# Gardlin/PCR-CG

Measured on AMD Instinct MI355X. Metric: fragment-pairs/s KPFCNN+GCN fwd, 30k-pt pairs, higher is better.
Workload: dtype f32

## Files before the change

include/pcrcg.h:

```cpp
#ifndef PCRCG_H
#define PCRCG_H

#include <stddef.h>
#include <stdint.h>

#ifdef __cplusplus
extern "C" {
#endif

#define PCRCG_OK 0
#define PCRCG_EBADARG (-1)
#define PCRCG_EWORKSPACE (-2)
#define PCRCG_ELAUNCH (-3)
#define PCRCG_ECAPACITY (-4)

#define PCRCG_KPOINTS 15

const char* pcrcg_last_error(void);
#define PCRCG_ABI_VERSION 4
int pcrcg_abi_version(void);

int pcrcg_debug_set(const char* spec);
int pcrcg_debug_release(void);

// ... 111 lines not shown
                             float* const* out, int count, int c, int ld_x, int ld_out, void* stream);
size_t pcrcg_instnorm_ws_bytes(int c);
int pcrcg_instnorm_stats_from_partials(const void* partials, int chunks, int c, double count, float eps,
                                       float* stats, void* stream);
int pcrcg_instnorm_stats(const float* x, int n, int c, int ldx, float eps, float* stats, void* ws,
                         size_t ws_bytes, void* stream);
int pcrcg_instnorm_apply(const float* x, int n, int c, int ldx, const float* stats, const float* res,
                         int ldr, const float* res_stats, float slope, float* y, int ldy, void* stream);
int pcrcg_instnorm_colsums(const float* x, int n, int c, int ldx, void* sums, void* stream);
int pcrcg_instnorm_apply_sums(const float* x, int n, int c, int ldx, const void* sums, double count, float eps,
                              const float* res, int ldr, const void* res_sums, float slope, float* y, int ldy,
                              void* stream);

int pcrcg_fill2d(float* dst, int ld, int rows, int cols, float value, void* stream);
int pcrcg_inject_image_features(const float* fmap, int c, int h, int w, const float* valid, const int64_t* inds2d,
                                const int64_t* inds3d, int n, long row_offset, long n_rows, float* x, int ldx,
                                void* stream);

typedef struct pcrcg_image_frame {
    const float* fmap;
    const float* depth;
    const float* valid;
    float world2camera[16];
    float intrinsics[16];
    float thresh;
    int h, w;
    int depth_h, depth_w;
    int target;
} pcrcg_image_frame;

size_t pcrcg_project_depth_ws_bytes(int n);
int pcrcg_project_depth(const float* points, int n, const float* depth, int h, int w, const float* h_world2camera,
                        const float* h_intrinsics, float thresh, int64_t* inds2d, int64_t* inds3d, int* k, void* ws,
                        size_t ws_bytes, void* stream);
int pcrcg_inject_frames(const float* points, long n_points, long len_src, const pcrcg_image_frame* h_frames, int n_frames,
                        int c, float* x, int ldx, void* stream);
int pcrcg_superglue_valid_maps(const float* keypoints0, int n0, const float* keypoints1, int n1, const int64_t* matches,
                               const float* confidence, int window, int map_w, int map_h, float* src_valid, float* tgt_valid,
                               void* stream);

int pcrcg_knn(const float* coords, int n, int k, int* idx, void* stream);
size_t pcrcg_edgeconv_ws_bytes(int c);
int pcrcg_edgeconv_reduce(const float* ctr, int ld_ctr, const float* nbr, int ld_nbr, const int* idx,
                          int n, int k, int c, float eps, float* emax, int ld_emax, float* stats,
                          void* ws, size_t ws_bytes, void* stream);
int pcrcg_edgeconv_reduce_sums(const float* ctr, int ld_ctr, const float* nbr, int ld_nbr, const int* idx, int n, int k,
                               int c, float* emax, int ld_emax, void* sums, void* stream);
int pcrcg_softmax_rows(float* x, int rows, int cols, int ld, float scale, void* stream);
int pcrcg_attention_supported(int d);
int pcrcg_attention(const float* q, int ldq, const float* k, int ldk, const float* v, int ldv, float* out, int ldo, int n,
                    int ms, int heads, int d, float scale, void* stream);
int pcrcg_softmax_matvec(const float* x, int rows, int cols, int ld, float scale, const float* vec, int ldv, float* y,
                         int ldy, void* stream);

int pcrcg_check_status(const int* status, void* stream);

int pcrcg_copy2d(const float* src, int ld_src, float* dst, int ld_dst, int rows, int cols, void* stream);
int pcrcg_add(const float* a, const float* b, float* dst, long n, void* stream);
int pcrcg_l2norm_rows(const float* src, int ld_src, float* dst, int ld_dst, int rows, int cols, void* stream);
int pcrcg_sigmoid_scores(const float* src, int ld_src, float* dst, int rows, void* stream);

#define PCRCG_MAX_LEVELS 8
#define PCRCG_MAX_BLOCKS 32
#define PCRCG_MAX_GNN 8

enum { PCRCG_BLK_SIMPLE = 0, PCRCG_BLK_RESNETB = 1, PCRCG_BLK_UNARY = 2, PCRCG_BLK_LAST_UNARY = 3,
       PCRCG_BLK_UPSAMPLE = 4 };

typedef struct pcrcg_block {
    int type;
    int layer;
    int strided;
    int in_dim, out_dim;
    int mid_dim;
    float extent;
    const float* kp;
    const float* kp_w;
    const float* kp_wt;
    const float* kp_w_pad;
    int cin_pad;
    const float* unary1;
    const float* unary2;
    const float* shortcut;
    const float* mlp;
    int mlp_ld;
    const float* mlp_skip;
    int mlp_skip_ld, skip_dim;
} pcrcg_block;

typedef struct pcrcg_gnn_layer {
    int cross;
    const float* edge1;
    const float* edge2;
    const float* conv3;
    const float *wq, *bq, *wk, *bk, *wv, *bv;
    const float *wm, *bm;
    const float *w0, *b0;
    const float *w3, *b3;
} pcrcg_gnn_layer;

typedef struct pcrcg_model {
    int n_enc, n_dec, n_gnn;
    pcrcg_block enc[PCRCG_MAX_BLOCKS];
    pcrcg_block dec[PCRCG_MAX_BLOCKS];
    pcrcg_gnn_layer gnn[PCRCG_MAX_GNN];
    int enc_skip[PCRCG_MAX_BLOCKS];
    int dec_concat[PCRCG_MAX_BLOCKS];
    int enc_out_dim, gnn_dim, heads, knn_k, final_dim;
    const float *bottle_w, *bottle_b;
    const float *proj_gnn_w, *proj_gnn_b;
    const float *proj_score_w, *proj_score_b;
    float temperature;
    int feature_bf16;
// ... 143 lines not shown
```

pcrcg_amd/_lib.py:

```python
import ctypes
import os

_HERE = os.path.dirname(os.path.abspath(__file__))
LIB_PATH = os.path.join(_HERE, "libpcrcg_hip.so")


def lib_identity():
    import hashlib
    with open(LIB_PATH, "rb") as f:
        return LIB_PATH, hashlib.sha256(f.read()).hexdigest()[:16]

ABI_VERSION = 4

c_int, c_float, c_void_p, c_size_t = ctypes.c_int, ctypes.c_float, ctypes.c_void_p, ctypes.c_size_t

SIGNATURES = {
    "pcrcg_last_error": (ctypes.c_char_p, []),
    "pcrcg_abi_version": (c_int, []),
    "pcrcg_debug_set": (c_int, [ctypes.c_char_p]),
    "pcrcg_check_status": (c_int, [c_void_p, c_void_p]),
    "pcrcg_grid_subsample_ws_bytes": (c_size_t, [c_int, c_int]),
    "pcrcg_grid_subsample_batch": (c_int, [c_void_p, c_int, c_void_p, c_int, c_float, c_int, c_void_p, c_void_p,
                                           c_void_p, c_void_p, c_size_t, c_void_p]),
    "pcrcg_grid_subsample_ex_ws_bytes": (c_size_t, [c_int, c_int, c_int, c_int]),
# ... 36 lines not shown
    "pcrcg_kpconv_aggregate_walk": (c_int, [c_void_p, c_int, c_void_p, c_int, c_void_p, c_int, c_int, c_void_p, c_int,
                                            c_void_p, c_float, c_void_p, c_void_p, c_void_p, c_size_t, c_void_p, c_void_p]),
    "pcrcg_kpconv_aggregate_bf16_walk": (c_int, [c_void_p, c_int, c_void_p, c_int, c_void_p, c_int, c_int, c_void_p, c_int,
                                                 c_void_p, c_float, c_void_p, c_void_p, c_void_p, c_void_p, c_size_t,
                                                 c_void_p, c_void_p]),
    "pcrcg_gather_max_walk": (c_int, [c_void_p, c_int, c_int, c_void_p, c_int, c_int, c_int, c_void_p, c_void_p, c_void_p]),
    "pcrcg_profile_kpconv": (None, [c_int]),
    "pcrcg_profile_kpconv_read": (c_int, [c_void_p, c_void_p, c_void_p, c_void_p, c_void_p, c_void_p, c_int]),
    "pcrcg_gemm_f32": (c_int, [c_void_p, c_int, c_void_p, c_int, c_int, c_void_p, c_int, c_int, c_int, c_int,
                               c_void_p, c_void_p, c_void_p]),
    "pcrcg_gemm_colstats_bytes": (c_size_t, [c_int, c_int]),
    "pcrcg_gemm_f32_colstats": (c_int, [c_void_p, c_int, c_void_p, c_int, c_int, c_void_p, c_int, c_int, c_int, c_int,
                                        c_void_p, c_void_p, c_void_p, c_size_t, c_void_p, c_void_p]),
    "pcrcg_gemm_bf16a_f32_colstats": (c_int, [c_void_p, c_int, c_void_p, c_int, c_void_p, c_int, c_int, c_int, c_int,
                                              c_void_p, c_void_p, c_void_p, c_size_t, c_void_p, c_void_p]),
    "pcrcg_gemm_f32_fused": (c_int, [c_void_p, c_int, c_void_p, c_int, c_int, c_void_p, c_void_p, ctypes.c_double, c_float,
                                     c_float, c_void_p, c_int, c_void_p, c_void_p, c_int, c_int, c_int, c_int, c_int, c_void_p]),
    "pcrcg_gemm_set_mode": (None, [c_int]),
    "pcrcg_gemm_get_mode": (c_int, []),
    "pcrcg_gemm_redo_counts": (c_int, [c_void_p, c_int]),
    "pcrcg_instnorm_stats_from_partials": (c_int, [c_void_p, c_int, c_int, ctypes.c_double, c_float, c_void_p,
                                                   c_void_p]),
    "pcrcg_gather_max": (c_int, [c_void_p, c_int, c_int, c_void_p, c_int, c_int, c_int, c_void_p, c_void_p]),
    "pcrcg_gather_first": (c_int, [c_void_p, c_int, c_int, c_void_p, c_int, c_int, c_void_p, c_int, c_void_p]),
    "pcrcg_gather_first_multi": (c_int, [c_void_p, c_void_p, c_void_p, c_void_p, c_void_p, c_void_p, c_int, c_int, c_int, c_int,
                                         c_void_p]),
    "pcrcg_instnorm_ws_bytes": (c_size_t, [c_int]),
    "pcrcg_instnorm_stats": (c_int, [c_void_p, c_int, c_int, c_int, c_float, c_void_p, c_void_p, c_size_t, c_void_p]),
    "pcrcg_instnorm_apply": (c_int, [c_void_p, c_int, c_int, c_int, c_void_p, c_void_p, c_int, c_void_p, c_float,
                                     c_void_p, c_int, c_void_p]),
    "pcrcg_instnorm_colsums": (c_int, [c_void_p, c_int, c_int, c_int, c_void_p, c_void_p]),
    "pcrcg_instnorm_apply_sums": (c_int, [c_void_p, c_int, c_int, c_int, c_void_p, ctypes.c_double, c_float, c_void_p, c_int,
                                          c_void_p, c_float, c_void_p, c_int, c_void_p]),
    "pcrcg_fill2d": (c_int, [c_void_p, c_int, c_int, c_int, c_float, c_void_p]),
    "pcrcg_inject_image_features": (c_int, [c_void_p, c_int, c_int, c_int, c_void_p, c_void_p, c_void_p, c_int, ctypes.c_long,
                                            ctypes.c_long, c_void_p, c_int, c_void_p]),
    "pcrcg_project_depth_ws_bytes": (c_size_t, [c_int]),
    "pcrcg_project_depth": (c_int, [c_void_p, c_int, c_void_p, c_int, c_int, c_void_p, c_void_p, c_float, c_void_p, c_void_p,
                                    c_void_p, c_void_p, c_size_t, c_void_p]),
    "pcrcg_inject_frames": (c_int, [c_void_p, ctypes.c_long, ctypes.c_long, c_void_p, c_int, c_int, c_void_p, c_int, c_void_p]),
    "pcrcg_superglue_valid_maps": (c_int, [c_void_p, c_int, c_void_p, c_int, c_void_p, c_void_p, c_int, c_int, c_int, c_void_p,
                                           c_void_p, c_void_p]),
    "pcrcg_knn": (c_int, [c_void_p, c_int, c_int, c_void_p, c_void_p]),
    "pcrcg_edgeconv_ws_bytes": (c_size_t, [c_int]),
    "pcrcg_edgeconv_reduce": (c_int, [c_void_p, c_int, c_void_p, c_int, c_void_p, c_int, c_int, c_int, c_float,
                                      c_void_p, c_int, c_void_p, c_void_p, c_size_t, c_void_p]),
    "pcrcg_edgeconv_reduce_sums": (c_int, [c_void_p, c_int, c_void_p, c_int, c_void_p, c_int, c_int, c_int, c_void_p, c_int,
                                           c_void_p, c_void_p]),
    "pcrcg_softmax_rows": (c_int, [c_void_p, c_int, c_int, c_int, c_float, c_void_p]),
    "pcrcg_attention_supported": (c_int, [c_int]),
    "pcrcg_attention": (c_int, [c_void_p, c_int, c_void_p, c_int, c_void_p, c_int, c_void_p, c_int, c_int, c_int, c_int,
                                c_int, c_float, c_void_p]),
    "pcrcg_softmax_matvec": (c_int, [c_void_p, c_int, c_int, c_int, c_float, c_void_p, c_int, c_void_p, c_int, c_void_p]),
    "pcrcg_copy2d": (c_int, [c_void_p, c_int, c_void_p, c_int, c_int, c_int, c_void_p]),
    "pcrcg_add": (c_int, [c_void_p, c_void_p, c_void_p, ctypes.c_long, c_void_p]),
    "pcrcg_l2norm_rows": (c_int, [c_void_p, c_int, c_void_p, c_int, c_int, c_int, c_void_p]),
    "pcrcg_sigmoid_scores": (c_int, [c_void_p, c_int, c_void_p, c_int, c_void_p]),
    "pcrcg_kpfcnn_ws_bytes": (c_size_t, [c_void_p, c_void_p]),
    "pcrcg_kpfcnn_group_ws_bytes": (c_size_t, [c_void_p, c_void_p, c_int]),
    "pcrcg_kpfcnn_forward_group": (c_int, [c_void_p, c_void_p, c_void_p, c_int, c_void_p, c_size_t, c_void_p]),
    "pcrcg_kpfcnn_forward": (c_int, [c_void_p, c_void_p, c_void_p, c_void_p, c_size_t, c_void_p]),
    "pcrcg_pyramid_ws_bytes": (c_size_t, [c_int, c_int, c_void_p]),
    "pcrcg_pyramid_build": (c_int, [c_void_p, c_int, c_void_p, c_int, c_void_p, c_void_p, c_size_t, c_void_p, c_void_p,
                                    c_void_p, c_void_p, c_void_p, c_void_p]),
    "pcrcg_pyramid_build_parts": (c_int, [c_void_p, c_void_p, c_void_p, c_void_p, c_int, c_void_p, c_void_p, c_size_t, c_void_p,
                                          c_void_p, c_void_p, c_void_p, c_void_p, c_void_p]),
    "pcrcg_pyramid_restore_run": (c_int, [c_void_p, c_void_p, c_void_p]),
    "pcrcg_debug_release": (c_int, []),
    "pcrcg_stream_pipe_classes": (c_int, [c_void_p, c_int, c_void_p, c_void_p]),
    "pcrcg_thread_shares_gpu": (None, [c_int]),
    "pcrcg_stream_create": (c_int, [c_void_p, c_int]),
    "pcrcg_stream_destroy": (c_int, [c_void_p]),
    "pcrcg_ransac_ws_bytes": (c_size_t, [c_int, c_int, c_int, c_int]),
    "pcrcg_feature_match": (c_int, [c_void_p, c_int, c_int, c_void_p, c_int, c_int, c_int, c_int, c_void_p, c_void_p,
                                    c_void_p, c_size_t, c_void_p]),
    "pcrcg_ransac": (c_int, [c_void_p, c_int, c_void_p, c_int, c_void_p, c_void_p, c_int, c_void_p, c_int, ctypes.c_double,
                             ctypes.c_double, c_int, c_int, c_int, ctypes.c_uint64, c_void_p, c_void_p, c_void_p, c_void_p,
                             c_size_t, c_void_p]),
    "pcrcg_ransac_batch_ws_bytes": (c_size_t, [c_int, c_int, c_int, c_int, c_int]),
    "pcrcg_feature_match_batch": (c_int, [c_void_p, c_int, c_void_p, c_int, c_int, c_void_p, c_int, c_void_p, c_int, c_int,
                                          c_int, c_int, c_void_p, c_void_p, c_void_p, c_size_t, c_void_p]),
    "pcrcg_ransac_batch": (c_int, [c_void_p, c_void_p, c_void_p, c_void_p, c_int, c_void_p, c_void_p, c_void_p, c_int, c_int,
                                   ctypes.c_double, ctypes.c_double, c_int, c_int, c_int, c_void_p, c_void_p, c_void_p,
                                   c_void_p, c_size_t, c_void_p]),
    "pcrcg_inlier_stats_batch_ws_bytes": (c_size_t, [c_int, c_int, c_int]),
    "pcrcg_inlier_stats_batch": (c_int, [c_void_p, c_void_p, c_int, c_void_p, c_int, c_int, c_void_p, c_void_p, c_int, c_void_p,
                                         c_int, c_int, c_int, c_int, c_void_p, c_void_p, c_int, c_void_p, c_void_p, c_void_p,
                                         c_void_p, c_void_p, c_void_p, c_void_p, c_size_t, c_void_p]),
    "pcrcg_icp_batch_ws_bytes": (c_size_t, [c_int, c_int, c_int, c_int]),
    "pcrcg_icp_batch": (c_int, [c_void_p, c_void_p, c_int, c_int, c_void_p, c_int, c_void_p, c_void_p, c_int, ctypes.c_double,
                                c_int, ctypes.c_double, ctypes.c_double, c_void_p, c_void_p, c_void_p, c_void_p, c_size_t,
                                c_void_p]),
    "pcrcg_voxel_down_sample_ws_bytes": (c_size_t, [c_int, c_int]),
    "pcrcg_voxel_down_sample_batch": (c_int, [c_void_p, c_void_p, c_int, c_int, ctypes.c_double, c_void_p, c_void_p, c_void_p,
                                              c_void_p, c_void_p, c_size_t, c_void_p]),
    "pcrcg_weighted_sample_ws_bytes": (c_size_t, [c_int, c_int]),
    "pcrcg_weighted_sample_batch": (c_int, [c_void_p, c_void_p, c_int, c_int, c_void_p, c_void_p, c_void_p, c_void_p, c_size_t,
                                            c_void_p]),
    "pcrcg_chamfer_batch_ws_bytes": (c_size_t, [c_int, c_int, c_int, c_int]),
    "pcrcg_chamfer_batch": (c_int, [c_void_p, c_void_p, c_int, c_void_p, c_void_p, c_int, c_void_p, c_void_p, c_int, c_int,
                                    c_void_p, c_void_p, c_void_p, c_void_p, c_void_p, c_void_p, c_void_p, c_void_p, c_void_p,
                                    c_void_p, c_size_t, c_void_p]),
    "pcrcg_res50unet_arena_bytes": (c_size_t, [c_int]),
    "pcrcg_res50unet_pack": (c_int, [c_void_p, c_int, c_int, c_void_p, c_void_p]),
    "pcrcg_res50unet_ws_bytes": (c_size_t, [c_int, c_int, c_int]),
    "pcrcg_res50unet_forward": (c_int, [c_void_p, c_void_p, c_int, c_int, c_void_p, c_int, c_int, c_int, c_int, c_int,
# ... 112 lines not shown
```

pcrcg_amd/csrc/common.h:

```cpp
#pragma once
#include <hip/hip_runtime.h>

#include <cstdarg>
#include <cstdint>
#include <cstdio>
#include <map>
#include <mutex>

#include "pcrcg.h"

namespace pcrcg {

void set_error(const char* fmt, ...);

inline hipStream_t as_stream(void* s) { return reinterpret_cast<hipStream_t>(s); }

struct Carver {
    char* base;
    size_t cap;
    size_t off = 0;
    Carver(void* ws, size_t bytes) : base(static_cast<char*>(ws)), cap(bytes) {}
    template <typename T>
    T* take(size_t count) {
        size_t bytes = (count * sizeof(T) + 255) & ~size_t(255);
        T* p = reinterpret_cast<T*>(base + off);
        off += bytes;
        return p;
    }
    bool ok() const { return off <= cap; }
};
inline size_t carve_bytes(size_t count, size_t elem) { return (count * elem + 255) & ~size_t(255); }

size_t scan_ws_bytes(int n);
int exclusive_scan_i32(const int* in, int* out, int n, int* total, void* ws, hipStream_t stream);

constexpr int kWave = 64;

bool instnorm_pack_ok(int c, int ldx, int ldy);
int instnorm_apply_pack(const float* x, int n, int c, int ldx, const float* stats, const double* sums, double count, float eps,
                        float slope, float* y, int ldy, const float* s_pts, float4* pk, hipStream_t st);
size_t colstats_ws_bytes(int c);
int colstats_finalize(const double* partial, int nchunks, int c, double count, float eps, float* stats,
                      hipStream_t st);
int colstats_chunks();

class StreamScratch {
public:
    explicit StreamScratch(bool cleared = false);
    void* get(hipStream_t st, size_t bytes, size_t slack = 0);
    void release();
private:
    struct Buf { void* p = nullptr; size_t bytes = 0; };
    const bool cleared_;
    std::mutex mu_;
    std::map<hipStream_t, Buf> bufs_;
};

int query_walk_multi(const float* const* pts, const int* n, int* const* walk, int* const* key, int count, hipStream_t st);

struct NormJob {
    const float* x; const double* sums; const float* res; const double* res_sums; float* y;
    const float* s_pts; float4* pk;
    int n; double count;
    float* stats_out = nullptr;
};
int instnorm_apply_sums_multi(const NormJob* jobs, int count, int c, int ldx, float eps, int ldr, float slope, int ldy, bool pack,
                              hipStream_t st);
bool instnorm_sums_ok(int c, int ldx, int ldy, int ldr = 0);

struct GatherJob { const float* x; const int64_t* idx; float* out; int ns, nq, h, ld_idx; const int* walk = nullptr; };
int gather_max_multi(const GatherJob* jobs, int count, int c, hipStream_t st);
struct FirstJob { const float* x; const int64_t* idx; float* out; int ns, nq, ld_idx; };
int gather_first_multi(const FirstJob* jobs, int count, int c, int ld_x, int ld_out, hipStream_t st);
int heads_multi(const float* const* x, const int* rows, int count, int ld, int fd, float* const* feats, float* const* s_ov,
                float* const* s_sal, hipStream_t st);
int copy2d_multi(const float* const* src, float* const* dst, const int* rows, int count, int ld_src, int ld_dst, int cols,
                 hipStream_t st);
int instnorm_colsums_multi(const float* const* x, double* const* sums, const int* n, int count, int c, int ldx, hipStream_t st);

struct EdgeCloud {
    const float* ctr; const float* nbr; const int* idx; float* emax; double* sums; int n, k;
};
bool edgeconv_rows_ok(const EdgeCloud* cl, int count, int ld_ctr, int ld_nbr, int ld_emax, int c);
int edgeconv_rows_multi(const EdgeCloud* cl, int count, int ld_ctr, int ld_nbr, int ld_emax, int c, bool atomic, int* nchunks_out,
                        hipStream_t st);

struct AttnCloud { const float* q; const float* k; const float* v; float* out; int n, ms; };
bool attention_mfma_ok(const AttnCloud* cl, int count, int ldq, int ldk, int ldv, int d);
int attention_mfma_multi(const AttnCloud* cl, int count, int ldq, int ldk, int ldv, int ldo, int heads, int d, float scale,
                         hipStream_t st);
bool attention_bwd_mfma_ok(int n, int ms, int d, int ldq, int ldk, int ldv, int ld_do);
int attention_bwd_mfma(const float* q, int ldq, const float* k, int ldk, const float* v, int ldv, const float* o, int ldo,
                       const float* d_o, int ld_do, float* dq, int ld_dq, float* dk, int ld_dk, float* dv, int ld_dv, int n, int ms,
                       int heads, int d, float scale, hipStream_t st);

struct DebugOpts {
    int stat_sums = 1;
    int stat_sums_rows = 1 << 30;
    int att_mfma = 1;
    int radius_blocks = 0;
    int kd_blocks = 0;
    int att_tq = 16;
    int kd_spin_limit = 0;
    int gemm_log = 0;
    int x6_tile = -1, x6_splitk = 0, x6_t1 = 1, x6_t2 = 1, x6_order = -1, x6_big = 0, x6_h2 = 1;
    int train_side_stream = 1;
    int gemm_tile = -1, gemm_splitk = 0, gemm_split_target = 768;
    int deterministic = 0;
    int bwd_mfma = 1;
    int walk = 1;
};
const DebugOpts& debug_opts();

struct KpProfScope {
    hipStream_t st;
    hipEvent_t a, b;
    int nq, h, cin, cout, kind;
    bool on;
    KpProfScope(hipStream_t s, int nq, int h, int cin, int cout, int kind);
    ~KpProfScope();
};

}

#define PCRCG_CHECK_ARG(cond)                                                        \
    do {                                                                             \
        if (!(cond)) {                                                               \
            pcrcg::set_error("%s: bad argument: %s", __func__, #cond);               \
            return PCRCG_EBADARG;                                                    \
        }                                                                            \
    } while (0)
// ... 44 lines not shown
```

pcrcg_amd/csrc/elementwise.hip:

```cpp
#include "common.h"
#include "pcrcg_train.h"

namespace pcrcg {
namespace {

struct CopyMulti { const float* src[4]; float* dst[4]; int rows[4]; };
__global__ void __launch_bounds__(256) k_copy2d(CopyMulti mm, int ld_src, int ld_dst, int cols) {
    const float* __restrict__ src = mm.src[blockIdx.y];
    float* __restrict__ dst = mm.dst[blockIdx.y];
    const int rows = mm.rows[blockIdx.y];
    const long e = (long)blockIdx.x * blockDim.x + threadIdx.x;
    if (e >= (long)rows * cols) return;
    const long r = e / cols;
    const int c = (int)(e - r * cols);
    dst[r * ld_dst + c] = src[r * ld_src + c];
}

__global__ void __launch_bounds__(256) k_add(const float* __restrict__ a, const float* __restrict__ b,
                                              float* __restrict__ dst, long n) {
    const long e = (long)blockIdx.x * blockDim.x + threadIdx.x;
    if (e < n) dst[e] = a[e] + b[e];
}

__global__ void __launch_bounds__(256) k_l2norm_rows(const float* __restrict__ src, int ld_src, float* __restrict__ dst,
                                                      int ld_dst, int rows, int cols) {
    const int lane = threadIdx.x & 63;
    const int r = blockIdx.x * 4 + (threadIdx.x >> 6);
    if (r >= rows) return;
    float s = 0.f;
    for (int c = lane; c < cols; c += 64) {
        const float v = src[(long)r * ld_src + c];
        s += v * v;
    }
#pragma unroll
    for (int d = 32; d >= 1; d >>= 1) s += __shfl_xor(s, d, 64);
    const float inv = 1.0f / fmaxf(sqrtf(s), 1e-12f);
    for (int c = lane; c < cols; c += 64) dst[(long)r * ld_dst + c] = src[(long)r * ld_src + c] * inv;
}

__global__ void __launch_bounds__(256) k_sigmoid_scores(const float* __restrict__ src, int ld_src,
                                                         float* __restrict__ dst, int rows) {
    const int r = blockIdx.x * blockDim.x + threadIdx.x;
    if (r >= rows) return;
    float v = 1.0f / (1.0f + expf(-src[(long)r * ld_src]));
    v = fminf(fmaxf(v, 0.0f), 1.0f);
    if (isnan(v) || isinf(v)) v = 0.0f;
    dst[r] = v;
}

struct HeadsMulti { const float* x[4]; float* feats[4]; float* s_ov[4]; float* s_sal[4]; int rows[4]; };
__global__ void __launch_bounds__(256) k_heads(HeadsMulti mm, int ld, int fd) {
    const int g = blockIdx.y, lane = threadIdx.x & 63;
    const int r = blockIdx.x * 4 + (threadIdx.x >> 6);
    if (r >= mm.rows[g]) return;
    const float* src = mm.x[g] + (long)r * ld;
    float s = 0.f;
    for (int c = lane; c < fd; c += 64) {
        const float v = src[c];
        s += v * v;
    }
#pragma unroll
    for (int d = 32; d >= 1; d >>= 1) s += __shfl_xor(s, d, 64);
    const float inv = 1.0f / fmaxf(sqrtf(s), 1e-12f);
    float* dst = mm.feats[g] + (long)r * fd;
    for (int c = lane; c < fd; c += 64) dst[c] = src[c] * inv;
    if (lane < 2) {
        float v = 1.0f / (1.0f + expf(-src[fd + lane]));
        v = fminf(fmaxf(v, 0.0f), 1.0f);
        if (isnan(v) || isinf(v)) v = 0.0f;
        (lane == 0 ? mm.s_ov[g] : mm.s_sal[g])[r] = v;
    }
}

__global__ void __launch_bounds__(256) k_fill2d(float* __restrict__ dst, int ld, int rows, int cols, float v) {
    const long e = (long)blockIdx.x * blockDim.x + threadIdx.x;
    if (e >= (long)rows * cols) return;
    const long r = e / cols;
    dst[r * ld + (int)(e - r * cols)] = v;
}

__global__ void __launch_bounds__(256) k_inject_image(const float* __restrict__ fmap, int c, int h, int w,
                                                       const float* __restrict__ valid, const long long* __restrict__ inds2d,
                                                       const long long* __restrict__ inds3d, int n, long row_offset,
                                                       long n_rows, float* __restrict__ x, int ldx) {
    const int lane = threadIdx.x & 63;
    const int j = blockIdx.x * 4 + (threadIdx.x >> 6);
    if (j >= n) return;
    const long px = inds2d[2 * (long)j], py = inds2d[2 * (long)j + 1], row = inds3d[j] + row_offset;
    if (px < 0 || px >= w || py < 0 || py >= h || row < 0 || row >= n_rows) return;
    const float m = valid ? valid[px * h + py] : 1.0f;
    float* dst = x + row * ldx;
    for (int ch = lane; ch < c; ch += 64) dst[ch] = fmap[((long)ch * h + py) * w + px] * m;
    if (lane == 0) dst[c] = 1.0f;
}

}

int heads_multi(const float* const* x, const int* rows, int count, int ld, int fd, float* const* feats, float* const* s_ov,
                float* const* s_sal, hipStream_t st) {
    PCRCG_CHECK_ARG(count >= 1 && count <= 4 && fd >= 1 && ld >= fd + 2);
    HeadsMulti mm;
    int rmax = 0;
    for (int g = 0; g < 4; ++g) {
        const int k = g < count ? g : 0;
        PCRCG_CHECK_ARG(x[k] && feats[k] && s_ov[k] && s_sal[k] && rows[k] >= 0);
        mm.x[g] = x[k]; mm.feats[g] = feats[k]; mm.s_ov[g] = s_ov[k]; mm.s_sal[g] = s_sal[k]; mm.rows[g] = g < count ? rows[k] : 0;
        if (g < count) rmax = rows[k] > rmax ? rows[k] : rmax;
    }
    if (rmax == 0) return PCRCG_OK;
    hipLaunchKernelGGL(k_heads, dim3((rmax + 3) / 4, count), dim3(256), 0, st, mm, ld, fd);
    PCRCG_CHECK_LAUNCH();
    return PCRCG_OK;
}

int copy2d_multi(const float* const* src, float* const* dst, const int* rows, int count, int ld_src, int ld_dst, int cols,
                 hipStream_t st) {
    PCRCG_CHECK_ARG(count >= 1 && count <= 4 && cols >= 0 && ld_src >= cols && ld_dst >= cols);
    CopyMulti mm;
    int rmax = 0;
    for (int g = 0; g < 4; ++g) {
        const int k = g < count ? g : 0;
        mm.src[g] = src[k]; mm.dst[g] = dst[k]; mm.rows[g] = g < count ? rows[k] : 0;
        if (g < count) {
            PCRCG_CHECK_ARG(rows[k] >= 0 && (rows[k] == 0 || (src[k] && dst[k])));
            rmax = rows[k] > rmax ? rows[k] : rmax;
        }
    }
    if (rmax == 0 || cols == 0) return PCRCG_OK;
    const long total = (long)rmax * cols;
    hipLaunchKernelGGL(k_copy2d, dim3((unsigned)((total + 255) / 256), count), dim3(256), 0, st, mm, ld_src, ld_dst, cols);
    PCRCG_CHECK_LAUNCH();
    return PCRCG_OK;
}
struct GatherJobs { const float* src; float* dst; const int* m1; const int* m2; int n; float s2; int accumulate; int cols; };
__global__ void __launch_bounds__(256) k_gather_jobs(const GatherJobs* __restrict__ jobs) {
    const GatherJobs jb = jobs[blockIdx.y];
    if (!jb.m1) {
        __shared__ float tile[32][33];
        const int cols = jb.cols, rows = jb.n / cols;
        const int tx = (cols + 31) / 32, ty = (rows + 31) / 32;
        const int lx = threadIdx.x & 31, ly = threadIdx.x >> 5;
        for (int t = blockIdx.x; t < tx * ty; t += gridDim.x) {
            const int r0 = (t / tx) * 32, c0 = (t % tx) * 32;
            __syncthreads();
#pragma unroll
            for (int u = 0; u < 4; ++u) {
                const int r = r0 + ly + 8 * u, c = c0 + lx;
                tile[ly + 8 * u][lx] = (r < rows && c < cols) ? jb.src[(long)r * cols + c] : 0.f;
            }
            __syncthreads();
#pragma unroll
            for (int u = 0; u < 4; ++u) {
                const int c = c0 + ly + 8 * u, r = r0 + lx;
                if (c < cols && r < rows) {
                    float* d = jb.dst + (long)c * rows + r;
                    *d = jb.accumulate ? *d + tile[lx][ly + 8 * u] : tile[lx][ly + 8 * u];
                }
            }
        }
        return;
    }
    auto one = [&](long i) {
        const int a = jb.m1[i];
        float v = a >= 0 ? jb.src[a] : 0.f;
        if (jb.m2) {
            const int b = jb.m2[i];
            if (b >= 0) v += jb.s2 * jb.src[b];
        }
        jb.dst[i] = jb.accumulate ? jb.dst[i] + v : v;
    };
    const bool vec = ((reinterpret_cast<uintptr_t>(jb.dst) | reinterpret_cast<uintptr_t>(jb.m1) | reinterpret_cast<uintptr_t>(jb.m2)) & 15) == 0;
    if (!vec) {
        for (long i = (long)blockIdx.x * 256 + threadIdx.x; i < jb.n; i += (long)gridDim.x * 256) one(i);
        return;
    }
    const long n4 = jb.n & ~3;
    for (long i = ((long)blockIdx.x * 256 + threadIdx.x) * 4; i < n4; i += (long)gridDim.x * 1024) {
        const int4 a = *reinterpret_cast<const int4*>(jb.m1 + i);
        int4 b = make_int4(-1, -1, -1, -1);
        if (jb.m2) b = *reinterpret_cast<const int4*>(jb.m2 + i);
        float4 v = make_float4(a.x >= 0 ? jb.src[a.x] : 0.f, a.y >= 0 ? jb.src[a.y] : 0.f, a.z >= 0 ? jb.src[a.z] : 0.f,
                               a.w >= 0 ? jb.src[a.w] : 0.f);
        if (b.x >= 0) v.x += jb.s2 * jb.src[b.x];
// ... 8 lines not shown
}
}

using namespace pcrcg;

extern "C" {

int pcrcg_fill2d(float* dst, int ld, int rows, int cols, float value, void* stream) {
    PCRCG_CHECK_ARG(rows >= 0 && cols >= 0 && ld >= cols);
    if (rows == 0 || cols == 0) return PCRCG_OK;
    PCRCG_CHECK_ARG(dst != nullptr);
    const long total = (long)rows * cols;
    hipLaunchKernelGGL(k_fill2d, dim3((unsigned)((total + 255) / 256)), dim3(256), 0, as_stream(stream), dst, ld, rows,
                       cols, value);
    PCRCG_CHECK_LAUNCH();
    return PCRCG_OK;
}

int pcrcg_inject_image_features(const float* fmap, int c, int h, int w, const float* valid, const int64_t* inds2d,
                                const int64_t* inds3d, int n, long row_offset, long n_rows, float* x, int ldx,
                                void* stream) {
    PCRCG_CHECK_ARG(c >= 1 && h >= 1 && w >= 1 && n >= 0 && n_rows >= 0 && ldx >= c + 1);
    if (n == 0) return PCRCG_OK;
    PCRCG_CHECK_ARG(fmap && inds2d && inds3d && x);
    hipLaunchKernelGGL(k_inject_image, dim3((n + 3) / 4), dim3(256), 0, as_stream(stream), fmap, c, h, w, valid,
                       reinterpret_cast<const long long*>(inds2d), reinterpret_cast<const long long*>(inds3d), n, row_offset,
                       n_rows, x, ldx);
    PCRCG_CHECK_LAUNCH();
    return PCRCG_OK;
}

int pcrcg_copy2d(const float* src, int ld_src, float* dst, int ld_dst, int rows, int cols, void* stream) {
    PCRCG_CHECK_ARG(rows >= 0 && cols >= 0 && ld_src >= cols && ld_dst >= cols);
    if (rows == 0 || cols == 0) return PCRCG_OK;
    PCRCG_CHECK_ARG(src && dst);
    return pcrcg::copy2d_multi(&src, &dst, &rows, 1, ld_src, ld_dst, cols, as_stream(stream));
}

int pcrcg_gather_jobs(const void* jobs, int n_jobs, int max_n, void* stream) {
    static_assert(sizeof(GatherJobs) == sizeof(pcrcg_gather_job), "pcrcg_gather_job layout");
    PCRCG_CHECK_ARG(n_jobs >= 0 && max_n >= 0);
    if (n_jobs == 0 || max_n == 0) return PCRCG_OK;
    PCRCG_CHECK_ARG(jobs != nullptr);
    const int gx = (max_n + 1023) / 1024 < 1024 ? (max_n + 1023) / 1024 : 1024;
    hipLaunchKernelGGL(k_gather_jobs, dim3(gx, n_jobs), dim3(256), 0, as_stream(stream), static_cast<const GatherJobs*>(jobs));
    PCRCG_CHECK_LAUNCH();
    return PCRCG_OK;
}

int pcrcg_add(const float* a, const float* b, float* dst, long n, void* stream) {
    PCRCG_CHECK_ARG(n >= 0);
    if (n == 0) return PCRCG_OK;
    PCRCG_CHECK_ARG(a && b && dst);
    hipLaunchKernelGGL(k_add, dim3((unsigned)((n + 255) / 256)), dim3(256), 0, as_stream(stream), a, b, dst, n);
    PCRCG_CHECK_LAUNCH();
    return PCRCG_OK;
}

int pcrcg_l2norm_rows(const float* src, int ld_src, float* dst, int ld_dst, int rows, int cols, void* stream) {
    PCRCG_CHECK_ARG(rows >= 0 && cols >= 1 && ld_src >= cols && ld_dst >= cols);
    if (rows == 0) return PCRCG_OK;
    PCRCG_CHECK_ARG(src && dst);
    hipLaunchKernelGGL(k_l2norm_rows, dim3((rows + 3) / 4), dim3(256), 0, as_stream(stream), src, ld_src, dst, ld_dst,
                       rows, cols);
    PCRCG_CHECK_LAUNCH();
    return PCRCG_OK;
}

int pcrcg_sigmoid_scores(const float* src, int ld_src, float* dst, int rows, void* stream) {
    PCRCG_CHECK_ARG(rows >= 0 && ld_src >= 1);
    if (rows == 0) return PCRCG_OK;
    PCRCG_CHECK_ARG(src && dst);
    hipLaunchKernelGGL(k_sigmoid_scores, dim3((rows + 255) / 256), dim3(256), 0, as_stream(stream), src, ld_src, dst,
                       rows);
    PCRCG_CHECK_LAUNCH();
    return PCRCG_OK;
}
}
```

pcrcg_amd/csrc/gnn.hip:

```cpp
#include "common.h"
#include "pcrcg_train.h"

namespace pcrcg {
namespace {

typedef unsigned long long u64;

__device__ __forceinline__ float knn_sq(float x, float y, float z) {
#pragma clang fp contract(off)
    return (x * x + y * y) + z * z;
}
__device__ __forceinline__ float knn_dist(float ax, float ay, float az, float sa, float bx, float by, float bz) {
#pragma clang fp contract(off)
    const float dot = __builtin_fmaf(az, bz, __builtin_fmaf(ay, by, ax * bx));
    const float sb = (bx * bx + by * by) + bz * bz;
    const float d = (-2.0f * dot + sa) + sb;
    return fmaxf(d, 1e-12f);
}

#define KNN_RB_MAX 704
#define KNN_K_MAX 10
__device__ __forceinline__ bool kless(u64 x, u64 y) { return (x >> 32) < (y >> 32); }

__device__ void rp_adjust_heap(u64* a, int hole, int len, u64 value) {
// ... 79 lines not shown
    auto key_of = [&](int j) -> u64 {
        const float d = knn_dist(ax, ay, az, sa, coords[3 * (long)j], coords[3 * (long)j + 1], coords[3 * (long)j + 2]);
        return ((u64)__float_as_uint(d) << 32) | (unsigned)j;
    };
    if (K * 64 <= n) {
        if (lane < K) a[lane] = key_of(lane);
        rp_make_heap(a, K);
        for (int base = K; base < n; base += 64) {
            const int j = base + lane;
            const u64 kj = j < n ? key_of(j) : ~0ull;
            u64 m = __ballot(kless(kj, a[0]));
            while (m) {
                const int l = __ffsll((long long)m) - 1;
                const u64 value = __shfl(kj, l, 64);
                rp_adjust_heap(a, 0, K, value);
                m = __ballot(kless(kj, a[0])) & ~((2ull << l) - 1ull);
            }
        }
        rp_sort_heap(a, K);
    } else {
        for (int j = lane; j < n; j += 64) a[j] = key_of(j);
        int first = 0, last = n;
        const int nth = K - 1;
        int depth = 2 * (31 - __clz(n));
        bool done = false;
        while (last - first > 3) {
            if (depth == 0) {
                u64* h = a + first;
                const int hl = nth + 1 - first;
                rp_make_heap(h, hl);
                for (int j = nth + 1; j < last; ++j)
                    if (kless(a[j], h[0])) {
                        const u64 value = a[j];
                        a[j] = h[0];
                        rp_adjust_heap(h, 0, hl, value);
                    }
                const u64 t = a[first];
                a[first] = a[nth];
                a[nth] = t;
                done = true;
                break;
            }
            --depth;
            const int cut = rp_partition_pivot(a, first, last);
            if (cut <= nth) first = cut;
            else last = cut;
        }
        if (!done) rp_insertion_sort(a, first, last);
        rp_insertion_sort(a, 0, K - 1);
    }
    if (lane >= 1 && lane < K) out[lane - 1] = (int)(a[lane] & 0xFFFFFFFFull);
}

__global__ void __launch_bounds__(256) k_knn(const float* __restrict__ coords, int n, int k, int* __restrict__ idx) {
    const int lane = threadIdx.x & 63;
    const int i = blockIdx.x * 4 + (threadIdx.x >> 6);
    if (i >= n) return;
    const float ax = coords[3 * (long)i], ay = coords[3 * (long)i + 1], az = coords[3 * (long)i + 2];
    const float sa = knn_sq(ax, ay, az);
    __shared__ u64 s_q[4][KNN_RB_MAX];
    u64 last = 0;
    bool have_last = false;
    bool tie = false;
    for (int round = 0; round <= k + 1; ++round) {
        u64 best = ~0ull;
        for (int j = lane; j < n; j += 64) {
            const float bx = coords[3 * (long)j], by = coords[3 * (long)j + 1], bz = coords[3 * (long)j + 2];
            float d = knn_dist(ax, ay, az, sa, bx, by, bz);
            const u64 key = ((u64)__float_as_uint(d) << 32) | (unsigned)j;
            if ((!have_last || key > last) && key < best) best = key;
        }
#pragma unroll
        for (int s = 32; s >= 1; s >>= 1) {
            const u64 o = __shfl_xor(best, s, 64);
            best = o < best ? o : best;
        }
        tie |= have_last && best != ~0ull && (best >> 32) == (last >> 32);
        last = best;
        have_last = true;
        if (round >= 1 && round <= k && lane == 0)
            idx[(long)i * k + (round - 1)] = best == ~0ull ? i : (int)(best & 0xFFFFFFFFull);
    }
    if (tie && n > k && k <= KNN_K_MAX) knn_replay_row(coords, n, i, k, s_q[threadIdx.x >> 6], idx + (long)i * k);
}

template <int PER>
__global__ void __launch_bounds__(256) k_knn_reg(const float* __restrict__ coords, int n, int k, int* __restrict__ idx) {
    const int lane = threadIdx.x & 63;
    const int i = blockIdx.x * 4 + (threadIdx.x >> 6);
    if (i >= n) return;
    const float ax = coords[3 * (long)i], ay = coords[3 * (long)i + 1], az = coords[3 * (long)i + 2];
    const float sa = knn_sq(ax, ay, az);
    u64 key[PER];
#pragma unroll
    for (int t = 0; t < PER; ++t) {
        const int j = lane + 64 * t;
        const int jc = j < n ? j : n - 1;
        const float bx = coords[3 * (long)jc], by = coords[3 * (long)jc + 1], bz = coords[3 * (long)jc + 2];
        float d = knn_dist(ax, ay, az, sa, bx, by, bz);
        key[t] = j < n ? (((u64)__float_as_uint(d) << 32) | (unsigned)j) : ~0ull;
    }
    __shared__ u64 s_q[4][KNN_RB_MAX];
    u64 last = 0;
    bool tie = false;
    for (int round = 0; round <= k + 1; ++round) {
        u64 best = ~0ull;
#pragma unroll
        for (int t = 0; t < PER; ++t)
            if ((round == 0 || key[t] > last) && key[t] < best) best = key[t];
#pragma unroll
        for (int s = 32; s >= 1; s >>= 1) {
            const u64 o = __shfl_xor(best, s, 64);
            best = o < best ? o : best;
        }
        tie |= round > 0 && best != ~0ull && (best >> 32) == (last >> 32);
        last = best;
        if (round >= 1 && round <= k && lane == 0)
            idx[(long)i * k + (round - 1)] = best == ~0ull ? i : (int)(best & 0xFFFFFFFFull);
    }
    if (tie && n > k && k <= KNN_K_MAX) knn_replay_row(coords, n, i, k, s_q[threadIdx.x >> 6], idx + (long)i * k);
}

struct AttCloud { const float* q; const float* k; const float* v; float* out; int n, ms; };
struct AttMulti { AttCloud cl[4]; int ldq, ldk, ldv, ldo; float scale; int chunk_blocks; };

typedef float attf16 __attribute__((ext_vector_type(16)));

template <int D>
__global__ void __launch_bounds__(256) k_attention_mfma(AttMulti a) {
    constexpr int DH = D / 2, NT = D / 32;
    extern __shared__ __attribute__((aligned(16))) float att2_lds[];
    const AttCloud cl = a.cl[blockIdx.z];
    const int n = cl.n, ms = cl.ms;
    const int q0 = blockIdx.x * 32;
    if (q0 >= n) return;
    const int head = blockIdx.y;
    const int lane = threadIdx.x & 63, wave = __builtin_amdgcn_readfirstlane((int)(threadIdx.x >> 6));
    const int l31 = lane & 31, half = lane >> 5;
    const int sld = a.chunk_blocks * 32 + 1;
    float* const S = att2_lds;
    float* const m_run = S + 32 * sld;
    float* const l_run = m_run + 32;
    float* const alpha = l_run + 32;
    float* const red = alpha + 32;
    const int nkb = (ms + 31) / 32;
    if (threadIdx.x < 32) { m_run[threadIdx.x] = -INFINITY; l_run[threadIdx.x] = 0.f; }
    float qr[DH];
    {
        const float* qrow = cl.q + (long)min(q0 + l31, n - 1) * a.ldq + head * D + half * DH;
#pragma unroll
        for (int c = 0; c < DH / 4; ++c) {
            const float4 t = *reinterpret_cast<const float4*>(qrow + 4 * c);
            qr[4 * c] = t.x; qr[4 * c + 1] = t.y; qr[4 * c + 2] = t.z; qr[4 * c + 3] = t.w;
        }
    }
    attf16 o[NT];
#pragma unroll
    for (int t = 0; t < NT; ++t)
#pragma unroll
        for (int r = 0; r < 16; ++r) o[t][r] = 0.f;
    for (int kb_lo = 0; kb_lo < nkb; kb_lo += a.chunk_blocks) {
        const int kb_hi = min(nkb, kb_lo + a.chunk_blocks), cb = kb_hi - kb_lo;
        __syncthreads();
        for (int kb = kb_lo + wave; kb < kb_hi; kb += 4) {
            const int key = kb * 32 + l31;
            const float* krow = cl.k + (long)min(key, ms - 1) * a.ldk + head * D + half * DH;
            float kr[DH];
#pragma unroll
            for (int c = 0; c < DH / 4; ++c) {
                const float4 t = *reinterpret_cast<const float4*>(krow + 4 * c);
                kr[4 * c] = t.x; kr[4 * c + 1] = t.y; kr[4 * c + 2] = t.z; kr[4 * c + 3] = t.w;
            }
            attf16 acc;
#pragma unroll
            for (int r = 0; r < 16; ++r) acc[r] = 0.f;
#pragma unroll
            for (int kk = 0; kk < DH; ++kk) acc = __builtin_amdgcn_mfma_f32_32x32x2f32(qr[kk], kr[kk], acc, 0, 0, 0);
// ... 217 lines not shown
            attf16 acc;
#pragma unroll
            for (int r = 0; r < 16; ++r) acc[r] = 0.f;
#pragma unroll
            for (int s = 0; s < 16; ++s) {
                const int qi = 2 * s + half;
                const long ro = (long)min(q0 + qi, n - 1);
                const float av = dS[qi * sld + key_lo + l31];
                const float bv = a.q[ro * a.ldq + head * D + 32 * t + l31];
                acc = __builtin_amdgcn_mfma_f32_32x32x2f32(av, bv, acc, 0, 0, 0);
            }
#pragma unroll
            for (int r = 0; r < 16; ++r) {
                const int key = key_lo + (r & 3) + 8 * (r >> 2) + 4 * half;
                if (key < ms) atomicAdd(a.dk + (long)key * a.ld_dk + head * D + 32 * t + l31, acc[r]);
            }
        }
    }
    {
        attf16 o[NT];
#pragma unroll
        for (int t = 0; t < NT; ++t)
#pragma unroll
            for (int r = 0; r < 16; ++r) o[t][r] = 0.f;
        const int per = (nkb + NW - 1) / NW;
        const int b0 = min(wave * per, nkb), b1 = min(b0 + per, nkb);
        for (int bi = b0; bi < b1; ++bi) {
            float pv[16], kv[NT][16];
#pragma unroll
            for (int j = 0; j < 16; ++j) {
                const int key = bi * 32 + 16 * half + j;
                pv[j] = dS[l31 * sld + key];
                const float* krow = a.k + (long)min(key, ms - 1) * a.ldk + head * D;
#pragma unroll
                for (int t = 0; t < NT; ++t) kv[t][j] = key < ms ? krow[t * 32 + l31] : 0.f;
            }
#pragma unroll
            for (int j = 0; j < 16; ++j)
#pragma unroll
                for (int t = 0; t < NT; ++t) o[t] = __builtin_amdgcn_mfma_f32_32x32x2f32(pv[j], kv[t][j], o[t], 0, 0, 0);
        }
        if (b1 > b0) {
#pragma unroll
            for (int t = 0; t < NT; ++t)
#pragma unroll
                for (int r = 0; r < 16; ++r) {
                    const int row = (r & 3) + 8 * (r >> 2) + 4 * half;
                    if (q0 + row < n) atomicAdd(a.dq + (long)(q0 + row) * a.ld_dq + head * D + t * 32 + l31, o[t][r]);
                }
        }
    }
}

struct EdgeMulti { EdgeCloud cl[4]; int ld_ctr, ld_nbr, ld_emax, c, rows_per_block, nchunks; };

template <bool ATOMIC>
__global__ void __launch_bounds__(256) k_edgeconv_rows(EdgeMulti a) {
    __shared__ double s_sum[4][256], s_sq[4][256];
    const EdgeCloud cl = a.cl[blockIdx.z];
    const int lane = threadIdx.x & 63, wave = __builtin_amdgcn_readfirstlane((int)(threadIdx.x >> 6));
    const int c0 = blockIdx.y * 256 + lane * 4;
    const bool cok = c0 < a.c;
    const int r0 = blockIdx.x * a.rows_per_block, r1 = min(cl.n, r0 + a.rows_per_block);
    double s[4] = {0.0, 0.0, 0.0, 0.0}, sq[4] = {0.0, 0.0, 0.0, 0.0};
    for (int r = r0 + wave; r < r1; r += 4) {
        const int mine = lane < cl.k ? cl.idx[(long)r * cl.k + lane] : 0;
        float4 q = make_float4(0.f, 0.f, 0.f, 0.f), m = q;
        if (cok) q = *reinterpret_cast<const float4*>(cl.ctr + (long)r * a.ld_ctr + c0);
        for (int j0 = 0; j0 < cl.k; j0 += 8) {
            float4 v[8];
#pragma unroll
            for (int u = 0; u < 8; ++u) {
                const int nb = __builtin_amdgcn_readlane(mine, min(j0 + u, cl.k - 1));
                v[u] = cok ? *reinterpret_cast<const float4*>(cl.nbr + (long)nb * a.ld_nbr + c0) : make_float4(0.f, 0.f, 0.f, 0.f);
            }
#pragma unroll
            for (int u = 0; u < 8; ++u) {
                if (j0 + u >= cl.k) continue;
                const float e[4] = {q.x + v[u].x, q.y + v[u].y, q.z + v[u].z, q.w + v[u].w};
                if (j0 + u == 0) m = make_float4(e[0], e[1], e[2], e[3]);
                else { m.x = fmaxf(m.x, e[0]); m.y = fmaxf(m.y, e[1]); m.z = fmaxf(m.z, e[2]); m.w = fmaxf(m.w, e[3]); }
#pragma unroll
                for (int t = 0; t < 4; ++t) { s[t] += (double)e[t]; sq[t] += (double)e[t] * (double)e[t]; }
            }
        }
        if (cok) *reinterpret_cast<float4*>(cl.emax + (long)r * a.ld_emax + c0) = m;
    }
#pragma unroll
    for (int t = 0; t < 4; ++t) { s_sum[wave][lane * 4 + t] = s[t]; s_sq[wave][lane * 4 + t] = sq[t]; }
    __syncthreads();
    const int ch = blockIdx.y * 256 + threadIdx.x;
    if (ch < a.c && r0 < r1) {
        const int t = threadIdx.x;
        const double ss = (s_sum[0][t] + s_sum[1][t]) + (s_sum[2][t] + s_sum[3][t]);
        const double qq = (s_sq[0][t] + s_sq[1][t]) + (s_sq[2][t] + s_sq[3][t]);
        if (ATOMIC) {
            unsafeAtomicAdd(&cl.sums[ch], ss);
            unsafeAtomicAdd(&cl.sums[(long)a.c + ch], qq);
        } else {
            cl.sums[(long)ch * a.nchunks + blockIdx.x] = ss;
            cl.sums[((long)a.c + ch) * a.nchunks + blockIdx.x] = qq;
        }
    } else if (!ATOMIC && ch < a.c) {
        cl.sums[(long)ch * a.nchunks + blockIdx.x] = 0.0;
        cl.sums[((long)a.c + ch) * a.nchunks + blockIdx.x] = 0.0;
    }
}
// ... 100 lines not shown
        for (int t = 0; t < KT; ++t) {
            const int key = j + G * t;
            const float* kr = Ks + key * KS;
            float acc = 0.f;
#pragma unroll
            for (int c = 0; c < D4; ++c) {
                const float4 kv = *reinterpret_cast<const float4*>(kr + 4 * c);
                acc = fmaf(qr[c].x, kv.x, acc);
                acc = fmaf(qr[c].y, kv.y, acc);
                acc = fmaf(qr[c].z, kv.z, acc);
                acc = fmaf(qr[c].w, kv.w, acc);
            }
            sc[t] = kc0 + key < ms ? acc * scale : -INFINITY;
            mx = fmaxf(mx, sc[t]);
        }
#pragma unroll
        for (int s = G / 2; s >= 1; s >>= 1) mx = fmaxf(mx, __shfl_xor(mx, s, 64));
        const float m_new = fmaxf(m, mx);
        const float alpha = expf(m - m_new);
        float psum = 0.f;
#pragma unroll
        for (int t = 0; t < KT; ++t) {
            const float pe = expf(sc[t] - m_new);
            Ps[qi * KC + j + G * t] = pe;
            psum += pe;
        }
#pragma unroll
        for (int s = G / 2; s >= 1; s >>= 1) psum += __shfl_xor(psum, s, 64);
        l = l * alpha + psum;
        m = m_new;
        __syncthreads();
#pragma unroll
        for (int i = 0; i < DV; ++i) o[i] *= alpha;
#pragma unroll 4
        for (int k4 = 0; k4 < KC / 4; ++k4) {
            const float4 pp = *reinterpret_cast<const float4*>(Ps + qi * KC + 4 * k4);
            const float pv[4] = {pp.x, pp.y, pp.z, pp.w};
#pragma unroll
            for (int u = 0; u < 4; ++u) {
                const float* vr = Vs + (4 * k4 + u) * D + j * DV;
#pragma unroll
                for (int i = 0; i < DV; ++i) o[i] = fmaf(pv[u], vr[i], o[i]);
            }
        }
    }
    if (row < n) {
        const float inv = 1.0f / l;
        float* orow = out + (long)row * ldo + head * D + j * DV;
#pragma unroll
        for (int i = 0; i < DV; ++i) orow[i] = o[i] * inv;
    }
}

__global__ void __launch_bounds__(256) k_softmax_matvec(const float* __restrict__ x, int rows, int cols, int ld, float scale,
                                                        const float* __restrict__ vec, int ldv, float* __restrict__ y,
                                                        int ldy) {
    const int lane = threadIdx.x & 63;
    const int r = blockIdx.x * 4 + (threadIdx.x >> 6);
    if (r >= rows) return;
    const float* row = x + (long)r * ld;
    float m = -INFINITY;
    for (int j = lane; j < cols; j += 64) m = fmaxf(m, row[j] * scale);
#pragma unroll
    for (int s = 32; s >= 1; s >>= 1) m = fmaxf(m, __shfl_xor(m, s, 64));
    float sum = 0.f, dot = 0.f;
    for (int j = lane; j < cols; j += 64) {
        const float e = expf(row[j] * scale - m);
        sum += e;
        dot = fmaf(e, vec[(long)j * ldv], dot);
    }
#pragma unroll
    for (int s = 32; s >= 1; s >>= 1) {
        sum += __shfl_xor(sum, s, 64);
        dot += __shfl_xor(dot, s, 64);
    }
    if (lane == 0) y[(long)r * ldy] = dot / sum;
}

}

bool edgeconv_rows_ok(const EdgeCloud* cl, int count, int ld_ctr, int ld_nbr, int ld_emax, int c) {
    if (count < 1 || count > 4 || c % 4 != 0 || ld_ctr % 4 != 0 || ld_nbr % 4 != 0 || ld_emax % 4 != 0) return false;
    for (int i = 0; i < count; ++i) {
        if (cl[i].k < 1 || cl[i].k > 64 || cl[i].n < 1) return false;
        if ((reinterpret_cast<uintptr_t>(cl[i].ctr) | reinterpret_cast<uintptr_t>(cl[i].nbr) | reinterpret_cast<uintptr_t>(cl[i].emax)) & 15)
            return false;
    }
    return true;
}
int edgeconv_rows_multi(const EdgeCloud* cl, int count, int ld_ctr, int ld_nbr, int ld_emax, int c, bool atomic, int* nchunks_out,
                        hipStream_t st) {
    EdgeMulti a;
    int nmax = 0;
    for (int i = 0; i < count; ++i) { a.cl[i] = cl[i]; nmax = cl[i].n > nmax ? cl[i].n : nmax; }
    for (int i = count; i < 4; ++i) a.cl[i] = cl[0];
    a.ld_ctr = ld_ctr; a.ld_nbr = ld_nbr; a.ld_emax = ld_emax; a.c = c;
    int rpb = 8;
    while ((nmax + rpb - 1) / rpb > colstats_chunks()) rpb += 4;
    a.rows_per_block = rpb;
    a.nchunks = (nmax + rpb - 1) / rpb;
    if (nchunks_out) *nchunks_out = a.nchunks;
    const dim3 grid(a.nchunks, (c + 255) / 256, count);
    if (atomic) hipLaunchKernelGGL(k_edgeconv_rows<true>, grid, dim3(256), 0, st, a);
    else hipLaunchKernelGGL(k_edgeconv_rows<false>, grid, dim3(256), 0, st, a);
    PCRCG_CHECK_LAUNCH();
    return PCRCG_OK;
}
static int attention_chunk_blocks(int d) {
    const size_t fixed = sizeof(float) * (96 + (size_t)96 * d);
    const size_t budget = 156 * 1024 - fixed;
    return (int)((budget / (32 * sizeof(float)) - 1) / 32);
}
bool attention_mfma_ok(const AttnCloud* cl, int count, int ldq, int ldk, int ldv, int d) {
    if (!debug_opts().att_mfma || count < 1 || count > 4 || (d != 32 && d != 64 && d != 128)) return false;
    if (ldq % 4 != 0 || ldk % 4 != 0 || ldv % 4 != 0) return false;
    for (int i = 0; i < count; ++i) {
        if (cl[i].n < 1 || cl[i].ms < 1) return false;
        if ((reinterpret_cast<uintptr_t>(cl[i].q) | reinterpret_cast<uintptr_t>(cl[i].k)) & 15) return false;
    }
    return true;
}
int attention_mfma_multi(const AttnCloud* cl, int count, int ldq, int ldk, int ldv, int ldo, int heads, int d, float scale,
                         hipStream_t st) {
    AttMulti a;
    int nmax = 0, msmax = 0;
    for (int i = 0; i < 4; ++i) {
        const AttnCloud& c = cl[i < count ? i : 0];
        a.cl[i] = AttCloud{c.q, c.k, c.v, c.out, c.n, c.ms};
        if (i < count) { nmax = c.n > nmax ? c.n : nmax; msmax = c.ms > msmax ? c.ms : msmax; }
    }
    a.ldq = ldq; a.ldk = ldk; a.ldv = ldv; a.ldo = ldo; a.scale = scale;
    const int nkb = (msmax + 31) / 32, cap = attention_chunk_blocks(d);
    a.chunk_blocks = nkb < cap ? nkb : cap;
    const size_t sld = (size_t)a.chunk_blocks * 32 + 1;
    const size_t lds = sizeof(float) * (32 * sld + 96 + (size_t)3 * 32 * d);
    const dim3 grid((nmax + 31) / 32, heads, count);
#define ATT2(DD)                                                                                                          \
    do {                                                                                                                  \
        PCRCG_GRANT_LDS((k_attention_mfma<DD>));                                                            \
        hipLaunchKernelGGL((k_attention_mfma<DD>), grid, dim3(256), lds, st, a);                                          \
    } while (0)
    if (d == 128) ATT2(128);
    else if (d == 64) ATT2(64);
    else ATT2(32);
#undef ATT2
    PCRCG_CHECK_LAUNCH();
    return PCRCG_OK;
}
bool attention_bwd_mfma_ok(int n, int ms, int d, int ldq, int ldk, int ldv, int ld_do) {
    if (!debug_opts().att_mfma || debug_opts().deterministic || n < 1 || ms < 1 || (d != 32 && d != 64 && d != 128)) return false;
    if (ldq % 4 != 0 || ldk % 4 != 0 || ldv % 4 != 0 || ld_do % 4 != 0) return false;
    const size_t sld = (size_t)((ms + 31) / 32) * 32 + 1;
    return sizeof(float) * (32 * sld + 32) <= 156 * 1024;
}
int attention_bwd_mfma(const float* q, int ldq, const float* k, int ldk, const float* v, int ldv, const float* o, int ldo,
                       const float* d_o, int ld_do, float* dq, int ld_dq, float* dk, int ld_dk, float* dv, int ld_dv, int n, int ms,
                       int heads, int d, float scale, hipStream_t st) {
    PCRCG_CHECK_ARG(attention_bwd_mfma_ok(n, ms, d, ldq, ldk, ldv, ld_do) && q && k && v && o && d_o && dq && dk && dv);
    PCRCG_CHECK_ARG(((reinterpret_cast<uintptr_t>(q) | reinterpret_cast<uintptr_t>(k) | reinterpret_cast<uintptr_t>(v) |
                      reinterpret_cast<uintptr_t>(d_o)) & 15) == 0);
    AttBwd a{q, k, v, o, d_o, dq, dk, dv, n, ms, ldq, ldk, ldv, ldo, ld_do, ld_dq, ld_dk, ld_dv, scale};
    const size_t sld = (size_t)((ms + 31) / 32) * 32 + 1;
    const size_t lds = sizeof(float) * (32 * sld + 32);
    const dim3 grid((n + 31) / 32, heads);
#define ATTB(DD)                                                                                                          \
    do {                                                                                                                  \
        PCRCG_GRANT_LDS((k_attention_bwd_mfma<DD>));                                                            \
        hipLaunchKernelGGL((k_attention_bwd_mfma<DD>), grid, dim3(512), lds, st, a);                                      \
    } while (0)
    if (d == 128) ATTB(128);
    else if (d == 64) ATTB(64);
    else ATTB(32);
#undef ATTB
    PCRCG_CHECK_LAUNCH();
    return PCRCG_OK;
}
}

using namespace pcrcg;

extern "C" {

int pcrcg_knn(const float* coords, int n, int k, int* idx, void* stream) {
    PCRCG_CHECK_ARG(n >= 0 && k >= 1);
    if (n == 0) return PCRCG_OK;
    PCRCG_CHECK_ARG(coords && idx);
    if (n <= 64 * 8)
        hipLaunchKernelGGL(k_knn_reg<8>, dim3((n + 3) / 4), dim3(256), 0, as_stream(stream), coords, n, k, idx);
    else if (n <= 64 * 16)
        hipLaunchKernelGGL(k_knn_reg<16>, dim3((n + 3) / 4), dim3(256), 0, as_stream(stream), coords, n, k, idx);
    else
        hipLaunchKernelGGL(k_knn, dim3((n + 3) / 4), dim3(256), 0, as_stream(stream), coords, n, k, idx);
    PCRCG_CHECK_LAUNCH();
    return PCRCG_OK;
}

size_t pcrcg_edgeconv_ws_bytes(int c) { return colstats_ws_bytes(c); }

int pcrcg_edgeconv_reduce(const float* ctr, int ld_ctr, const float* nbr, int ld_nbr, const int* idx,
                          int n, int k, int c, float eps, float* emax, int ld_emax, float* stats,
                          void* ws, size_t ws_bytes, void* stream) {
    PCRCG_CHECK_ARG(n >= 1 && k >= 1 && c >= 1 && ld_ctr >= c && ld_nbr >= c && ld_emax >= c);
    PCRCG_CHECK_ARG(ctr && nbr && idx && emax && stats && ws);
    const int chunks = colstats_chunks();
    Carver cv(ws, ws_bytes);
    double* partial = cv.take<double>((size_t)chunks * 2 * c);
    PCRCG_CHECK_WS(cv);
    hipStream_t st = as_stream(stream);
    {
        const EdgeCloud one = {ctr, nbr, idx, emax, partial, n, k};
        if (edgeconv_rows_ok(&one, 1, ld_ctr, ld_nbr, ld_emax, c)) {
            int nchunks = 0;
            PCRCG_PROPAGATE(edgeconv_rows_multi(&one, 1, ld_ctr, ld_nbr, ld_emax, c, false, &nchunks, st));
            return colstats_finalize(partial, nchunks, c, (double)n * (double)k, eps, stats, st);
        }
    }
    hipLaunchKernelGGL(k_edgeconv_reduce<false>, dim3(chunks, (c + 63) / 64), dim3(256), 0, st, ctr, ld_ctr, nbr, ld_nbr,
                       idx, n, k, c, emax, ld_emax, partial);
    return colstats_finalize(partial, chunks, c, (double)n * (double)k, eps, stats, st);
}

int pcrcg_edgeconv_reduce_sums(const float* ctr, int ld_ctr, const float* nbr, int ld_nbr, const int* idx, int n, int k,
                               int c, float* emax, int ld_emax, void* sums, void* stream) {
    PCRCG_CHECK_ARG(n >= 1 && k >= 1 && c >= 1 && ld_ctr >= c && ld_nbr >= c && ld_emax >= c);
    PCRCG_CHECK_ARG(ctr && nbr && idx && emax && sums);
    {
        const EdgeCloud one = {ctr, nbr, idx, emax, static_cast<double*>(sums), n, k};
        if (edgeconv_rows_ok(&one, 1, ld_ctr, ld_nbr, ld_emax, c))
            return edgeconv_rows_multi(&one, 1, ld_ctr, ld_nbr, ld_emax, c, true, nullptr, as_stream(stream));
    }
    int chunks = (n + 15) / 16;
    if (chunks > colstats_chunks()) chunks = colstats_chunks();
    hipLaunchKernelGGL(k_edgeconv_reduce<true>, dim3(chunks, (c + 63) / 64), dim3(256), 0, as_stream(stream), ctr, ld_ctr,
                       nbr, ld_nbr, idx, n, k, c, emax, ld_emax, static_cast<double*>(sums));
    PCRCG_CHECK_LAUNCH();
    return PCRCG_OK;
}

int pcrcg_attention_backward_supported(int n, int ms, int d, int ldq, int ldk, int ldv, int ld_do) {
    return attention_bwd_mfma_ok(n, ms, d, ldq, ldk, ldv, ld_do) ? 1 : 0;
}
int pcrcg_attention_backward(const float* q, int ldq, const float* k, int ldk, const float* v, int ldv, const float* out, int ldo,
                             const float* d_out, int ld_do, float* dq, int ld_dq, float* dk, int ld_dk, float* dv, int ld_dv,
                             int n, int ms, int heads, int d, float scale, void* stream) {
    PCRCG_CHECK_ARG(n >= 0 && ms >= 1 && heads >= 1);
    if (n == 0) return PCRCG_OK;
    PCRCG_CHECK_ARG(ldq >= heads * d && ldk >= heads * d && ldv >= heads * d && ldo >= heads * d && ld_do >= heads * d &&
                    ld_dq >= heads * d && ld_dk >= heads * d && ld_dv >= heads * d);
    return attention_bwd_mfma(q, ldq, k, ldk, v, ldv, out, ldo, d_out, ld_do, dq, ld_dq, dk, ld_dk, dv, ld_dv, n, ms, heads, d, scale,
                              as_stream(stream));
}

int pcrcg_attention_supported(int d) { return d == 16 || d == 32 || d == 48 || d == 64 || d == 128; }

int pcrcg_attention(const float* q, int ldq, const float* k, int ldk, const float* v, int ldv, float* out, int ldo, int n,
                    int ms, int heads, int d, float scale, void* stream) {
    PCRCG_CHECK_ARG(n >= 0 && ms >= 1 && heads >= 1 && pcrcg_attention_supported(d));
    PCRCG_CHECK_ARG(ldq >= heads * d && ldk >= heads * d && ldv >= heads * d && ldo >= heads * d);
    PCRCG_CHECK_ARG(ldq % 4 == 0 && ldk % 4 == 0 && ldv % 4 == 0);
    if (n == 0) return PCRCG_OK;
    PCRCG_CHECK_ARG(q && k && v && out);
    PCRCG_CHECK_ARG(((reinterpret_cast<uintptr_t>(q) | reinterpret_cast<uintptr_t>(k) | reinterpret_cast<uintptr_t>(v)) & 15) == 0);
    hipStream_t st = as_stream(stream);
    {
        const AttnCloud one = {q, k, v, out, n, ms};
        if (attention_mfma_ok(&one, 1, ldq, ldk, ldv, d)) return attention_mfma_multi(&one, 1, ldq, ldk, ldv, ldo, heads, d, scale, st);
    }
#define ATT(DD, TQ)                                                                                                  \
    do {                                                                                                             \
        constexpr size_t lds = sizeof(float) * (64 * (DD + 4) + 64 * DD + TQ * 64);                                  \
        if (lds > 64 * 1024) PCRCG_GRANT_LDS((k_attention<DD, TQ>));                              \
        hipLaunchKernelGGL((k_attention<DD, TQ>), dim3((n + TQ - 1) / TQ, heads), dim3(256), lds, st, q, ldq, k, ldk, v, \
                           ldv, out, ldo, n, ms, scale);                                                             \
    } while (0)
    const int att_tq = debug_opts().att_tq;
    if (d == 128 && att_tq == 8) ATT(128, 8);
    else if (d == 128) ATT(128, 16);
    else if (d == 64) ATT(64, 8);
    else if (d == 48) ATT(48, 16);
    else if (d == 32) ATT(32, 16);
    else ATT(16, 16);
#undef ATT
    PCRCG_CHECK_LAUNCH();
    return PCRCG_OK;
}

int pcrcg_softmax_matvec(const float* x, int rows, int cols, int ld, float scale, const float* vec, int ldv, float* y,
                         int ldy, void* stream) {
    PCRCG_CHECK_ARG(rows >= 0 && cols >= 1 && ld >= cols && ldv >= 1 && ldy >= 1);
    if (rows == 0) return PCRCG_OK;
    PCRCG_CHECK_ARG(x && vec && y);
    hipLaunchKernelGGL(k_softmax_matvec, dim3((rows + 3) / 4), dim3(256), 0, as_stream(stream), x, rows, cols, ld, scale, vec,
                       ldv, y, ldy);
    PCRCG_CHECK_LAUNCH();
    return PCRCG_OK;
}

int pcrcg_softmax_rows(float* x, int rows, int cols, int ld, float scale, void* stream) {
    PCRCG_CHECK_ARG(rows >= 0 && cols >= 1 && ld >= cols);
    if (rows == 0) return PCRCG_OK;
    PCRCG_CHECK_ARG(x != nullptr);
    hipLaunchKernelGGL(k_softmax_rows, dim3((rows + 3) / 4), dim3(256), 0, as_stream(stream), x, rows, cols, ld, scale);
    PCRCG_CHECK_LAUNCH();
    return PCRCG_OK;
}
}
```

pcrcg_amd/csrc/pointops.hip:

```cpp
#include "common.h"

namespace pcrcg {
namespace {

constexpr int kWavesPerBlock = 4;

struct GatherMulti { const float* x[4]; const long long* idx[4]; float* out[4]; int ns[4], nq[4], h[4], ld_idx[4]; const int* walk[4]; };
template <bool VEC4>
__global__ void __launch_bounds__(kWavesPerBlock * 64) k_gather_max(GatherMulti mm, int c, int nchunk) {
    const int g = blockIdx.y;
    const float* __restrict__ x = mm.x[g];
    const long long* __restrict__ idx = mm.idx[g];
    float* __restrict__ out = mm.out[g];
    const int ns = mm.ns[g], nq = mm.nq[g], h = mm.h[g], ld_idx = mm.ld_idx[g];
    const int lane = threadIdx.x & 63;
    const int* __restrict__ walk = mm.walk[g];
    const int wave = __builtin_amdgcn_readfirstlane((int)(threadIdx.x >> 6));
    long item = (long)blockIdx.x * kWavesPerBlock + wave, items = (long)nq * nchunk;
    int pos0 = 0;
    if (walk) {
        const int xcd = blockIdx.x & 7, slot = blockIdx.x >> 3;
        const int xq = nq >> 3, xr = nq & 7;
        pos0 = xcd < xr ? xcd * (xq + 1) : xr * (xq + 1) + (xcd - xr) * xq;
        item = (long)slot * kWavesPerBlock + wave;
// ... 21 lines not shown
            else { m.x = fmaxf(m.x, v.x); m.y = fmaxf(m.y, v.y); m.z = fmaxf(m.z, v.z); m.w = fmaxf(m.w, v.w); }
        }
        reinterpret_cast<float4*>(out + (long)q * c)[cb] = m;
    } else {
        const int cc = chunk * 64 + lane;
        if (cc >= c) return;
        float m = 0.f;
        bool any = false;
#pragma unroll 4
        for (int j = 0; j < h; ++j) {
            const long long i = row[j];
            const float v = (i >= 0 && i < ns) ? x[i * c + cc] : 0.f;
            m = any ? fmaxf(m, v) : v;
            any = true;
        }
        out[(long)q * c + cc] = m;
    }
}

__global__ void __launch_bounds__(256) k_gather_first(const float* __restrict__ x, int ns, int c,
                                                       const long long* __restrict__ idx, int nq, int ld_idx,
                                                       float* __restrict__ out, int ld_out) {
    const int lane = threadIdx.x & 63;
    const int q = blockIdx.x * 4 + __builtin_amdgcn_readfirstlane((int)(threadIdx.x >> 6));
    if (q >= nq) return;
    const long long i = idx[(long)q * ld_idx];
    const bool real = i >= 0 && i < ns;
    for (int cc = lane; cc < c; cc += 64) out[(long)q * ld_out + cc] = real ? x[i * c + cc] : 0.f;
}

struct FirstMulti { const float* x[4]; const long long* idx[4]; float* out[4]; int ns[4], nq[4], ld_idx[4]; };
template <bool VEC>
__global__ void __launch_bounds__(256) k_gather_first_multi(FirstMulti mm, int c, int ld_x, int ld_out) {
    const int g = blockIdx.y;
    const int segs = (c + 3) >> 2;
    const long t = (long)blockIdx.x * 256 + threadIdx.x;
    const long q = t / segs;
    if (q >= mm.nq[g]) return;
    const int c0 = (int)(t - q * segs) * 4;
    const long long i = mm.idx[g][q * mm.ld_idx[g]];
    const bool real = i >= 0 && i < mm.ns[g];
    const float* __restrict__ src = mm.x[g] + (real ? i : 0) * ld_x + c0;
    float* __restrict__ dst = mm.out[g] + q * ld_out + c0;
    if (VEC && c0 + 4 <= c) {
        *reinterpret_cast<float4*>(dst) = real ? *reinterpret_cast<const float4*>(src) : make_float4(0.f, 0.f, 0.f, 0.f);
    } else {
        const int n = c - c0 < 4 ? c - c0 : 4;
        for (int k = 0; k < n; ++k) dst[k] = real ? src[k] : 0.f;
    }
}

constexpr int kStatChunks = 128;

struct ColsMulti { const float* x[4]; double* partial[4]; int n[4]; };
template <bool ATOMIC>
__global__ void __launch_bounds__(256) k_colstats_partial(ColsMulti mm, int c, int ldx) {
    const float* __restrict__ x = mm.x[blockIdx.z];
    double* __restrict__ partial = mm.partial[blockIdx.z];
    const int n = mm.n[blockIdx.z];
    __shared__ double s_sum[4][64], s_sq[4][64];
    const int lane = threadIdx.x & 63, rl = threadIdx.x >> 6;
    const int ch = blockIdx.y * 64 + lane;
    const int chunk = blockIdx.x, nchunks = gridDim.x;
    const long rows_per = ((long)n + nchunks - 1) / nchunks;
    const long r0 = chunk * rows_per, r1 = min((long)n, r0 + rows_per);
    double s = 0.0, sq = 0.0;
    if (ch < c) {
        long r = r0 + rl;
        for (; r + 12 < r1; r += 16) {
            const float v0 = x[r * ldx + ch], v1 = x[(r + 4) * ldx + ch], v2 = x[(r + 8) * ldx + ch],
                        v3 = x[(r + 12) * ldx + ch];
            s += ((double)v0 + (double)v1) + ((double)v2 + (double)v3);
            sq += ((double)v0 * v0 + (double)v1 * v1) + ((double)v2 * v2 + (double)v3 * v3);
        }
        for (; r < r1; r += 4) {
            const double v = (double)x[r * ldx + ch];
            s += v;
            sq += v * v;
        }
    }
    s_sum[rl][lane] = s;
    s_sq[rl][lane] = sq;
    __syncthreads();
    if (rl == 0 && ch < c) {
        s = (s_sum[0][lane] + s_sum[1][lane]) + (s_sum[2][lane] + s_sum[3][lane]);
        sq = (s_sq[0][lane] + s_sq[1][lane]) + (s_sq[2][lane] + s_sq[3][lane]);
        if (ATOMIC) {
            if (r0 < r1) {
                unsafeAtomicAdd(&partial[ch], s);
                unsafeAtomicAdd(&partial[(long)c + ch], sq);
            }
        } else {
            partial[(long)ch * nchunks + chunk] = s;
            partial[((long)c + ch) * nchunks + chunk] = sq;
        }
    }
}

__global__ void __launch_bounds__(256) k_colstats_final(const double* __restrict__ partial, int nchunks, int c,
                                                         double count, float eps, float* __restrict__ stats) {
    const int lane = threadIdx.x & 63;
    const int ch = blockIdx.x * (blockDim.x >> 6) + (threadIdx.x >> 6);
    if (ch >= c) return;
    double s = 0.0, sq = 0.0;
    for (int k = lane; k < nchunks; k += 64) {
        s += partial[(long)ch * nchunks + k];
        sq += partial[((long)c + ch) * nchunks + k];
// ... 21 lines not shown
    const int ch = (int)(e - r * c);
    float v = (x[r * ldx + ch] - stats[2 * ch]) * stats[2 * ch + 1];
    if (res) {
        float rv = res[r * ldr + ch];
        if (res_stats) rv = (rv - res_stats[2 * ch]) * res_stats[2 * ch + 1];
        v += rv;
    }
    y[r * ldy + ch] = v >= 0.f ? v : v * slope;
}

__global__ void __launch_bounds__(256) k_instnorm_apply4(const float* __restrict__ x, int n, int c4, int ldx,
                                                          const float* __restrict__ stats, const float* __restrict__ res,
                                                          int ldr, const float* __restrict__ res_stats, float slope,
                                                          float* __restrict__ y, int ldy) {
    const long e = (long)blockIdx.x * blockDim.x + threadIdx.x;
    if (e >= (long)n * c4) return;
    const long r = e / c4;
    const int q = (int)(e - r * c4);
    const float4 xv = *reinterpret_cast<const float4*>(x + r * ldx + 4 * q);
    const float4 s0 = *reinterpret_cast<const float4*>(stats + 8 * q), s1 = *reinterpret_cast<const float4*>(stats + 8 * q + 4);
    float4 v = make_float4((xv.x - s0.x) * s0.y, (xv.y - s0.z) * s0.w, (xv.z - s1.x) * s1.y, (xv.w - s1.z) * s1.w);
    if (res) {
        float4 rv = *reinterpret_cast<const float4*>(res + r * ldr + 4 * q);
        if (res_stats) {
            const float4 t0 = *reinterpret_cast<const float4*>(res_stats + 8 * q),
                         t1 = *reinterpret_cast<const float4*>(res_stats + 8 * q + 4);
            rv = make_float4((rv.x - t0.x) * t0.y, (rv.y - t0.z) * t0.w, (rv.z - t1.x) * t1.y, (rv.w - t1.z) * t1.w);
        }
        v.x += rv.x; v.y += rv.y; v.z += rv.z; v.w += rv.w;
    }
    v.x = v.x >= 0.f ? v.x : v.x * slope;
    v.y = v.y >= 0.f ? v.y : v.y * slope;
    v.z = v.z >= 0.f ? v.z : v.z * slope;
    v.w = v.w >= 0.f ? v.w : v.w * slope;
    *reinterpret_cast<float4*>(y + r * ldy + 4 * q) = v;
}

__device__ __forceinline__ void stats4_from_sums(const double* __restrict__ sums, int c, int ch, double count, float eps,
                                                 float4& mean, float4& rstd) {
    float m[4], r[4];
#pragma unroll
    for (int i = 0; i < 4; ++i) {
        const double mu = sums[ch + i] / count;
        double var = sums[c + ch + i] / count - mu * mu;
        if (var < 0.0) var = 0.0;
        m[i] = (float)mu;
        r[i] = (float)(1.0 / sqrt(var + (double)eps));
    }
    mean = make_float4(m[0], m[1], m[2], m[3]);
    rstd = make_float4(r[0], r[1], r[2], r[3]);
}

struct NormMulti {
    const float* x[4]; const double* sums[4]; const float* res[4]; const double* res_sums[4]; float* y[4];
    const float* s_pts[4]; float4* pk[4];
    int n[4]; double count[4];
    float* stats_out[4];
};
template <int RES>
__global__ void __launch_bounds__(256) k_instnorm_apply4_sums(NormMulti mm, int c4, int ldx, float eps, int ldr, float slope, int ldy,
                                                               int rows_per_block) {
    const int g = blockIdx.y;
    const float* __restrict__ x = mm.x[g];
    const double* __restrict__ sums = mm.sums[g];
    const float* __restrict__ res = mm.res[g];
    const double* __restrict__ res_sums = mm.res_sums[g];
    float* __restrict__ y = mm.y[g];
    const int n = mm.n[g];
    const double count = mm.count[g];
    if ((long)blockIdx.x * rows_per_block >= n) return;
    const int cb = c4 < 256 ? c4 : 256;
    const int rp = 256 / cb;
    const int r_lo = blockIdx.x * rows_per_block, r_hi = min(n, r_lo + rows_per_block);
    for (int qb = 0; qb < c4; qb += cb) {
        const int q = qb + (int)(threadIdx.x % cb);
        float4 m0, s0, m1 = make_float4(0.f, 0.f, 0.f, 0.f), s1 = make_float4(1.f, 1.f, 1.f, 1.f);
        stats4_from_sums(sums, 4 * c4, 4 * q, count, eps, m0, s0);
        if (RES == 2) stats4_from_sums(res_sums, 4 * c4, 4 * q, count, eps, m1, s1);
        if (blockIdx.x == 0 && threadIdx.x < cb && mm.stats_out[g]) {
            float4* so = reinterpret_cast<float4*>(mm.stats_out[g] + 8 * q);
            so[0] = make_float4(m0.x, s0.x, m0.y, s0.y);
            so[1] = make_float4(m0.z, s0.z, m0.w, s0.w);
        }
        auto finish = [&](const float4& xv, float4 rv, long r) {
            float4 v = make_float4((xv.x - m0.x) * s0.x, (xv.y - m0.y) * s0.y, (xv.z - m0.z) * s0.z, (xv.w - m0.w) * s0.w);
            if (RES) {
                if (RES == 2) rv = make_float4((rv.x - m1.x) * s1.x, (rv.y - m1.y) * s1.y, (rv.z - m1.z) * s1.z, (rv.w - m1.w) * s1.w);
                v.x += rv.x; v.y += rv.y; v.z += rv.z; v.w += rv.w;
            }
            v.x = v.x >= 0.f ? v.x : v.x * slope;
            v.y = v.y >= 0.f ? v.y : v.y * slope;
            v.z = v.z >= 0.f ? v.z : v.z * slope;
            v.w = v.w >= 0.f ? v.w : v.w * slope;
            *reinterpret_cast<float4*>(y + r * ldy + 4 * q) = v;
        };
        long r = r_lo + (int)(threadIdx.x / cb);
        for (; r + 3 * rp < r_hi; r += 4 * rp) {
            float4 xv[4], rv[4];
#pragma unroll
            for (int u = 0; u < 4; ++u) {
                xv[u] = *reinterpret_cast<const float4*>(x + (r + u * rp) * ldx + 4 * q);
                rv[u] = RES ? *reinterpret_cast<const float4*>(res + (r + u * rp) * ldr + 4 * q) : make_float4(0.f, 0.f, 0.f, 0.f);
            }
#pragma unroll
            for (int u = 0; u < 4; ++u) finish(xv[u], rv[u], r + u * rp);
        }
        for (; r < r_hi; r += rp) {
            const float4 xv = *reinterpret_cast<const float4*>(x + r * ldx + 4 * q);
            const float4 rv = RES ? *reinterpret_cast<const float4*>(res + r * ldr + 4 * q) : make_float4(0.f, 0.f, 0.f, 0.f);
            finish(xv, rv, r);
// ... 32 lines not shown
    float4* __restrict__ pk = mm.pk[g];
    const int n = mm.n[g];
    const double count = mm.count[g];
    if ((long)blockIdx.x * rows_per_block >= n) return;
    const int rp = 256 / c4;
    const int r_lo = blockIdx.x * rows_per_block, r_hi = min(n, r_lo + rows_per_block);
    const int q = (int)(threadIdx.x % c4);
    float4 m0, s0;
    stats4_from_sums(sums, 4 * c4, 4 * q, count, eps, m0, s0);
    for (long r = r_lo + (int)(threadIdx.x / c4); r < r_hi; r += rp) {
        const float4 xv = *reinterpret_cast<const float4*>(x + r * ldx + 4 * q);
        float4 v = make_float4((xv.x - m0.x) * s0.x, (xv.y - m0.y) * s0.y, (xv.z - m0.z) * s0.z, (xv.w - m0.w) * s0.w);
        v.x = v.x >= 0.f ? v.x : v.x * slope;
        v.y = v.y >= 0.f ? v.y : v.y * slope;
        v.z = v.z >= 0.f ? v.z : v.z * slope;
        v.w = v.w >= 0.f ? v.w : v.w * slope;
        *reinterpret_cast<float4*>(y + r * ldy + 4 * q) = v;
        float part = (v.x + v.y) + (v.z + v.w);
        for (int sh = c4 >> 1; sh >= 1; sh >>= 1) part += __shfl_xor(part, sh, 64);
        if (q == 0) pk[r] = make_float4(s_pts[3 * r], s_pts[3 * r + 1], s_pts[3 * r + 2], part > 0.0f ? 1.f : 0.f);
    }
}

}

bool instnorm_pack_ok(int c, int ldx, int ldy) {
    const int c4 = c / 4;
    return c % 4 == 0 && c4 >= 1 && c4 <= 64 && (c4 & (c4 - 1)) == 0 && ldx % 4 == 0 && ldy % 4 == 0;
}
int instnorm_apply_pack(const float* x, int n, int c, int ldx, const float* stats, const double* sums, double count, float eps,
                        float slope, float* y, int ldy, const float* s_pts, float4* pk, hipStream_t st) {
    PCRCG_CHECK_ARG(n >= 0 && instnorm_pack_ok(c, ldx, ldy) && ldx >= c && ldy >= c && (stats != nullptr) != (sums != nullptr));
    if (n == 0) return PCRCG_OK;
    PCRCG_CHECK_ARG(x && y && s_pts && pk && ((reinterpret_cast<uintptr_t>(x) | reinterpret_cast<uintptr_t>(y)) & 15) == 0);
    const int c4 = c / 4;
    if (stats) {
        const long total = (long)n * c4;
        hipLaunchKernelGGL(k_instnorm_apply4_pack, dim3((unsigned)((total + 255) / 256)), dim3(256), 0, st, x, n, c4, ldx, stats,
                           slope, y, ldy, s_pts, pk);
    } else {
        NormJob one{x, sums, nullptr, nullptr, y, s_pts, pk, n, count};
        return instnorm_apply_sums_multi(&one, 1, c, ldx, eps, 0, slope, ldy, true, st);
    }
    PCRCG_CHECK_LAUNCH();
    return PCRCG_OK;
}

bool instnorm_sums_ok(int c, int ldx, int ldy, int ldr) {
    const int c4 = c / 4;
    return c >= 4 && c % 4 == 0 && (c4 <= 256 ? 256 % c4 == 0 : c4 % 256 == 0) && ldx % 4 == 0 && ldy % 4 == 0 && ldr % 4 == 0;
}
int instnorm_apply_sums_multi(const NormJob* jobs, int count, int c, int ldx, float eps, int ldr, float slope, int ldy, bool pack,
                              hipStream_t st) {
    PCRCG_CHECK_ARG(jobs && count >= 1 && count <= 4 && c >= 4 && c % 4 == 0);
    const int c4 = c / 4;
    NormMulti mm;
    int nmax = 0;
    for (int g = 0; g < 4; ++g) {
        const NormJob& j = jobs[g < count ? g : 0];
        mm.x[g] = j.x; mm.sums[g] = j.sums; mm.res[g] = j.res; mm.res_sums[g] = j.res_sums; mm.y[g] = j.y;
        mm.s_pts[g] = j.s_pts; mm.pk[g] = j.pk; mm.n[g] = g < count ? j.n : 0; mm.count[g] = j.count;
        mm.stats_out[g] = g < count ? j.stats_out : nullptr;
        if (g < count) {
            PCRCG_CHECK_ARG(j.n >= 0 && j.x && j.sums && j.y && j.count >= 1.0);
            PCRCG_CHECK_ARG((j.res != nullptr) == (jobs[0].res != nullptr) && (j.res_sums != nullptr) == (jobs[0].res_sums != nullptr));
            nmax = j.n > nmax ? j.n : nmax;
        }
    }
    if (nmax == 0) return PCRCG_OK;
    const int rp = 256 / (c4 < 256 ? c4 : 256);
    int rows_per_block = rp * 8;
    while (rows_per_block > rp && (long)(nmax + rows_per_block - 1) / rows_per_block * count < 256) rows_per_block -= rp;
    const dim3 grid((unsigned)((nmax + rows_per_block - 1) / rows_per_block), count);
    if (pack)
        hipLaunchKernelGGL(k_instnorm_apply4_sums_pack, grid, dim3(256), 0, st, mm, c4, ldx, eps, slope, ldy, rows_per_block);
    else if (!jobs[0].res)
        hipLaunchKernelGGL(k_instnorm_apply4_sums<0>, grid, dim3(256), 0, st, mm, c4, ldx, eps, ldr, slope, ldy, rows_per_block);
    else if (!jobs[0].res_sums)
        hipLaunchKernelGGL(k_instnorm_apply4_sums<1>, grid, dim3(256), 0, st, mm, c4, ldx, eps, ldr, slope, ldy, rows_per_block);
    else
        hipLaunchKernelGGL(k_instnorm_apply4_sums<2>, grid, dim3(256), 0, st, mm, c4, ldx, eps, ldr, slope, ldy, rows_per_block);
    PCRCG_CHECK_LAUNCH();
    return PCRCG_OK;
}

size_t colstats_ws_bytes(int c) { return carve_bytes((size_t)kStatChunks * 2 * (size_t)(c > 0 ? c : 1), sizeof(double)); }

int colstats_finalize(const double* partial, int nchunks, int c, double count, float eps, float* stats,
                      hipStream_t st) {
    hipLaunchKernelGGL(k_colstats_final, dim3((c + 3) / 4), dim3(256), 0, st, partial, nchunks, c, count, eps, stats);
    PCRCG_CHECK_LAUNCH();
    return PCRCG_OK;
}
int colstats_chunks() { return kStatChunks; }

int gather_max_multi(const GatherJob* jobs, int count, int c, hipStream_t st) {
    PCRCG_CHECK_ARG(jobs && count >= 1 && count <= 4 && c >= 1);
    GatherMulti mm;
    bool vec = c % 4 == 0;
    int nq_max = 0;
    for (int g = 0; g < 4; ++g) {
        const GatherJob& j = jobs[g < count ? g : 0];
        mm.x[g] = j.x; mm.idx[g] = reinterpret_cast<const long long*>(j.idx); mm.out[g] = j.out;
        mm.ns[g] = j.ns; mm.nq[g] = g < count ? j.nq : 0; mm.h[g] = j.h; mm.ld_idx[g] = j.ld_idx;
        mm.walk[g] = j.walk;
        if (g < count) {
            PCRCG_CHECK_ARG((j.walk != nullptr) == (jobs[0].walk != nullptr));
            PCRCG_CHECK_ARG(j.ns >= 0 && j.nq >= 0 && j.h >= 1 && j.ld_idx >= j.h && (j.nq == 0 || (j.x && j.idx && j.out)));
            vec = vec && ((reinterpret_cast<uintptr_t>(j.x) | reinterpret_cast<uintptr_t>(j.out)) & 15) == 0;
            nq_max = j.nq > nq_max ? j.nq : nq_max;
        }
    }
    if (nq_max == 0) return PCRCG_OK;
    const int per_wave = vec ? 256 : 64;
    const int nchunk = (c + per_wave - 1) / per_wave;
    const long items = jobs[0].walk ? (long)((nq_max + 7) / 8) * nchunk : (long)nq_max * nchunk;
    const dim3 grid((unsigned)((items + kWavesPerBlock - 1) / kWavesPerBlock) * (jobs[0].walk ? 8 : 1), count);
    if (vec) hipLaunchKernelGGL(k_gather_max<true>, grid, dim3(kWavesPerBlock * 64), 0, st, mm, c, nchunk);
    else hipLaunchKernelGGL(k_gather_max<false>, grid, dim3(kWavesPerBlock * 64), 0, st, mm, c, nchunk);
    PCRCG_CHECK_LAUNCH();
    return PCRCG_OK;
}

int gather_first_multi(const FirstJob* jobs, int count, int c, int ld_x, int ld_out, hipStream_t st) {
    PCRCG_CHECK_ARG(jobs && count >= 1 && count <= 4 && c >= 1 && ld_x >= c && ld_out >= c);
    FirstMulti mm;
    bool vec = ld_x % 4 == 0 && ld_out % 4 == 0;
    int nq_max = 0;
    for (int g = 0; g < 4; ++g) {
        const FirstJob& j = jobs[g < count ? g : 0];
        mm.x[g] = j.x; mm.idx[g] = reinterpret_cast<const long long*>(j.idx); mm.out[g] = j.out;
        mm.ns[g] = j.ns; mm.nq[g] = g < count ? j.nq : 0; mm.ld_idx[g] = j.ld_idx;
        if (g < count) {
            PCRCG_CHECK_ARG(j.ns >= 0 && j.nq >= 0 && j.ld_idx >= 1 && (j.nq == 0 || (j.idx && j.out && (j.x || j.ns == 0))));
            if (j.nq > 0) vec = vec && ((reinterpret_cast<uintptr_t>(j.x) | reinterpret_cast<uintptr_t>(j.out)) & 15) == 0;
            nq_max = j.nq > nq_max ? j.nq : nq_max;
        }
    }
    if (nq_max == 0) return PCRCG_OK;
    const long threads = (long)nq_max * ((c + 3) / 4);
    const dim3 grid((unsigned)((threads + 255) / 256), count);
    if (vec) hipLaunchKernelGGL(k_gather_first_multi<true>, grid, dim3(256), 0, st, mm, c, ld_x, ld_out);
    else hipLaunchKernelGGL(k_gather_first_multi<false>, grid, dim3(256), 0, st, mm, c, ld_x, ld_out);
    PCRCG_CHECK_LAUNCH();
    return PCRCG_OK;
}

int instnorm_colsums_multi(const float* const* x, double* const* sums, const int* n, int count, int c, int ldx, hipStream_t st) {
    PCRCG_CHECK_ARG(count >= 1 && count <= 4 && c >= 1 && ldx >= c);
    ColsMulti mm;
    int nmax = 0;
    for (int g = 0; g < 4; ++g) {
        const int k = g < count ? g : 0;
        PCRCG_CHECK_ARG(n[k] >= 1 && x[k] && sums[k]);
        mm.x[g] = x[k]; mm.partial[g] = sums[k]; mm.n[g] = n[k];
        if (g < count) nmax = n[k] > nmax ? n[k] : nmax;
    }
    int chunks = (nmax + 63) / 64;
    if (chunks > kStatChunks) chunks = kStatChunks;
    if (debug_opts().deterministic) chunks = 1;
    hipLaunchKernelGGL(k_colstats_partial<true>, dim3(chunks, (c + 63) / 64, count), dim3(256), 0, st, mm, c, ldx);
    PCRCG_CHECK_LAUNCH();
    return PCRCG_OK;
}

}

using namespace pcrcg;

extern "C" {

int pcrcg_gather_max(const float* x, int ns, int c, const int64_t* idx, int nq, int h, int ld_idx,
                     float* out, void* stream) {
    PCRCG_CHECK_ARG(ns >= 0 && c >= 1 && nq >= 0 && h >= 1 && ld_idx >= h);
    if (nq == 0) return PCRCG_OK;
    PCRCG_CHECK_ARG(x && idx && out);
    const GatherJob one{x, idx, out, ns, nq, h, ld_idx};
    return gather_max_multi(&one, 1, c, as_stream(stream));
}

int pcrcg_gather_first(const float* x, int ns, int c, const int64_t* idx, int nq, int ld_idx, float* out,
                       int ld_out, void* stream) {
    PCRCG_CHECK_ARG(ns >= 0 && c >= 1 && nq >= 0 && ld_idx >= 1 && ld_out >= c);
    if (nq == 0) return PCRCG_OK;
    PCRCG_CHECK_ARG(x && idx && out);
    hipLaunchKernelGGL(k_gather_first, dim3((nq + 3) / 4), dim3(256), 0, as_stream(stream), x, ns, c,
                       reinterpret_cast<const long long*>(idx), nq, ld_idx, out, ld_out);
    PCRCG_CHECK_LAUNCH();
    return PCRCG_OK;
}

int pcrcg_gather_first_multi(const float* const* x, const int* ns, const int64_t* const* idx, const int* nq, const int* ld_idx,
                             float* const* out, int count, int c, int ld_x, int ld_out, void* stream) {
    PCRCG_CHECK_ARG(x && ns && idx && nq && ld_idx && out && count >= 1 && count <= 4);
    FirstJob jobs[4];
    for (int g = 0; g < count; ++g) jobs[g] = FirstJob{x[g], idx[g], out[g], ns[g], nq[g], ld_idx[g]};
    return gather_first_multi(jobs, count, c, ld_x, ld_out, as_stream(stream));
}

size_t pcrcg_instnorm_ws_bytes(int c) { return colstats_ws_bytes(c); }

int pcrcg_instnorm_stats_from_partials(const void* partials, int chunks, int c, double count, float eps,
                                       float* stats, void* stream) {
    PCRCG_CHECK_ARG(partials && stats && chunks >= 1 && c >= 1 && count >= 1.0);
    return colstats_finalize(static_cast<const double*>(partials), chunks, c, count, eps, stats, as_stream(stream));
// ... 59 lines not shown
```

pcrcg_amd/csrc/runner.hip:

```cpp
#include <vector>

#include <cstdlib>

#include "gemm.h"
#include "kpconv.h"

namespace pcrcg {
namespace {

constexpr int GMAX = 4;
static_assert(GMAX <= 4, "instnorm_apply_sums_multi, instnorm_colsums_multi, gather_max_multi, gather_first_multi, copy2d_multi, heads_multi, "
                         "edgeconv_rows_multi and attention_mfma_multi (common.h) take up to four clouds");

struct Mat {
    float* p[GMAX] = {};
    int rows[GMAX] = {};
    int cols = 0, ld = 0;
    bool zeroed = false;
};

struct Ctx {
    char* base = nullptr;
    size_t cap = 0, off = 0, peak = 0;
    hipStream_t st = nullptr;
    bool dry = false;
    bool bf16 = false;
    int G = 1;
    int rc = PCRCG_OK;

    void* raw(size_t bytes) {
        bytes = (bytes + 255) & ~size_t(255);
        void* p = base ? base + off : nullptr;
        off += bytes;
        if (off > peak) peak = off;
        if (!dry && off > cap && rc == PCRCG_OK) {
            set_error("pcrcg_kpfcnn_forward: workspace too small (%zu needed so far, %zu given)", off, cap);
            rc = PCRCG_EWORKSPACE;
        }
        return p;
    }
    Mat mat(const int* rows, int cols, int ld = 0) {
        Mat m;
        m.cols = cols; m.ld = ld ? ld : cols;
        for (int g = 0; g < G; ++g) {
            m.rows[g] = rows[g];
            m.p[g] = static_cast<float*>(raw((size_t)(rows[g] > 0 ? rows[g] : 1) * m.ld * sizeof(float)));
        }
        return m;
    }
    char* zbase = nullptr;
    size_t zcap = 0, zoff = 0;
    void* zraw(size_t bytes) {
        bytes = (bytes + 255) & ~size_t(255);
        void* p = zbase ? zbase + zoff : nullptr;
        zoff += bytes;
        if (!dry && zoff > zcap && rc == PCRCG_OK) {
            set_error("pcrcg_kpfcnn_forward: zero arena too small (%zu needed so far, %zu reserved)", zoff, zcap);
            rc = PCRCG_EWORKSPACE;
        }
        return p;
    }
    int max_rows(const int* rows) const { int m = rows[0]; for (int g = 1; g < G; ++g) m = rows[g] > m ? rows[g] : m; return m; }
    Mat gemm_out(const int* rows, int cols, int k, int ld = 0) {
        long total = 0;
        for (int g = 0; g < G; ++g) total += rows[g];
        if (!gemm_bt_accumulates(max_rows(rows), cols, k, total)) return mat(rows, cols, ld);
        Mat m;
        m.cols = cols; m.ld = ld ? ld : cols;
        for (int g = 0; g < G; ++g) {
            m.rows[g] = rows[g];
            m.p[g] = static_cast<float*>(zraw((size_t)(rows[g] > 0 ? rows[g] : 1) * m.ld * sizeof(float)));
        }
        m.zeroed = true;
        return m;
    }
    size_t mark() const { return off; }
    void release(size_t m) { off = m; }
    bool live() const { return !dry && rc == PCRCG_OK; }
    void check(int r) { if (r != PCRCG_OK && rc == PCRCG_OK) rc = r; }
    bool paired() const { return G >= 2 && gemm_split_terms_on(); }
    template <class F> Mat twice(F&& f) { G *= 2; const Mat r = f(); G /= 2; return r; }
};

inline int pad4(int v) { return (v + 3) & ~3; }
inline Mat cols(const Mat& m, int c0, int n) {
    Mat r = m;
    for (int g = 0; g < GMAX; ++g) r.p[g] = m.p[g] ? m.p[g] + c0 : nullptr;
    r.cols = n;
    return r;
}
inline Mat rows(const Mat& m, const int* r0, const int* n) {
    Mat r = m;
    for (int g = 0; g < GMAX; ++g) {
        r.p[g] = m.p[g] ? m.p[g] + (long)r0[g] * m.ld : nullptr;
        r.rows[g] = n[g];
    }
    return r;
}
inline Mat stacked(const Mat& a, const Mat& b, int G0) {
    Mat m = a;
    for (int g = 0; g < G0; ++g) { m.p[G0 + g] = b.p[g]; m.rows[G0 + g] = b.rows[g]; }
    return m;
}
inline Mat half(const Mat& m, int which, int G0) {
    Mat r = m;
    for (int g = 0; g < GMAX; ++g) {
        r.p[g] = g < G0 ? m.p[which * G0 + g] : nullptr;
        r.rows[g] = g < G0 ? m.rows[which * G0 + g] : 0;
    }
    return r;
}

struct Stat {
    void* partials[GMAX] = {};
    size_t bytes = 0;
    int chunks[GMAX] = {};
    bool sums = false;
    static constexpr int SUMS = -1, NOTHING = 0;
    bool has_sums(int g) const { return chunks[g] == SUMS; }
    bool nothing(int g) const { return chunks[g] == NOTHING; }
};

Stat stat_buffer(Ctx& c, const int* rows, int cols) {
    Stat s;
    const int mr = c.max_rows(rows);
    if (debug_opts().stat_sums && mr <= debug_opts().stat_sums_rows && gemm_split_terms_on()) {
        s.sums = true;
        s.bytes = 2 * sizeof(double) * (size_t)cols;
        for (int g = 0; g < c.G; ++g) s.partials[g] = c.zraw(s.bytes);
        return s;
    }
    s.bytes = pcrcg_gemm_colstats_bytes(mr, cols);
    for (int g = 0; g < c.G; ++g) s.partials[g] = c.raw(s.bytes);
    return s;
}

inline bool sums_apply_ok(const Mat& x, const Mat& y, const Mat* res) {
    return instnorm_sums_ok(x.cols, x.ld, y.ld, res ? res->ld : 0);
}

void col_stats(Ctx& c, const Mat& x, int g, const Stat* s, float* stats, void* ws, size_t wsb) {
    if (s && !s->nothing(g))
        c.check(pcrcg_instnorm_stats_from_partials(s->partials[g], s->has_sums(g) ? 1 : s->chunks[g], x.cols, (double)x.rows[g], 1e-5f,
                                                   stats, c.st));
    else
        c.check(pcrcg_instnorm_stats(x.p[g], x.rows[g], x.cols, x.ld, 1e-5f, stats, ws, wsb, c.st));
}

void fill_sums(Ctx& c, const Mat& x, Stat* xs) {
    if (!c.live() || !xs || !xs->sums) return;
    {
        const float* xp[GMAX]; double* sp[GMAX]; int np[GMAX]; int idx[GMAX]; int cnt = 0;
        for (int g = 0; g < c.G; ++g)
            if (xs->nothing(g) && x.rows[g] >= 1) { xp[cnt] = x.p[g]; sp[cnt] = static_cast<double*>(xs->partials[g]); np[cnt] = x.rows[g]; idx[cnt++] = g; }
        if (cnt >= 2) {
            c.check(instnorm_colsums_multi(xp, sp, np, cnt, x.cols, x.ld, c.st));
            for (int i = 0; i < cnt; ++i) xs->chunks[idx[i]] = Stat::SUMS;
        }
    }
    for (int g = 0; g < c.G; ++g)
        if (xs->nothing(g)) {
            c.check(pcrcg_instnorm_colsums(x.p[g], x.rows[g], x.cols, x.ld, xs->partials[g], c.st));
            xs->chunks[g] = Stat::SUMS;
        }
}
inline bool all_sums(const Ctx& c, const Stat* s) {
    if (!s) return false;
    for (int g = 0; g < c.G; ++g)
        if (!s->has_sums(g)) return false;
    return true;
}

struct NormJobs {
    NormJob j[GMAX];
    bool aligned = true;
};
NormJobs norm_jobs(const Ctx& c, const Mat& x, void* const* sums, const Mat& y, const Mat* res = nullptr, void* const* res_sums = nullptr) {
    NormJobs nj;
    for (int g = 0; g < c.G; ++g) {
        const float* r = res ? res->p[g] : nullptr;
        nj.j[g] = NormJob{x.p[g], static_cast<const double*>(sums[g]), r, res_sums ? static_cast<const double*>(res_sums[g]) : nullptr,
                          y.p[g], nullptr, nullptr, x.rows[g], (double)(x.rows[g] > 0 ? x.rows[g] : 1)};
        nj.aligned = nj.aligned && ((reinterpret_cast<uintptr_t>(x.p[g]) | reinterpret_cast<uintptr_t>(y.p[g]) | reinterpret_cast<uintptr_t>(r)) & 15) == 0;
    }
    return nj;
}
void apply_sums(Ctx& c, const NormJob* jobs, bool one_launch, int cols, int ldx, int ldr, float slope, int ldy) {
    if (one_launch) {
        c.check(instnorm_apply_sums_multi(jobs, c.G, cols, ldx, 1e-5f, ldr, slope, ldy, false, c.st));
        return;
    }
    for (int g = 0; g < c.G; ++g) {
        const NormJob& j = jobs[g];
        c.check(pcrcg_instnorm_apply_sums(j.x, j.n, cols, ldx, j.sums, j.count, 1e-5f, j.res, ldr, j.res_sums, slope, j.y, ldy, c.st));
    }
}

void norm_act(Ctx& c, const Mat& x, float slope, const Mat& y, Stat* xs = nullptr, const Mat* res = nullptr,
              bool norm_res = false, Stat* rs = nullptr) {
    fill_sums(c, x, xs);
    if (res && norm_res) fill_sums(c, *res, rs);
    if (c.live() && all_sums(c, xs) && (!res || !norm_res || all_sums(c, rs)) && sums_apply_ok(x, y, res)) {
        const NormJobs nj = norm_jobs(c, x, xs->partials, y, res, (res && norm_res) ? rs->partials : nullptr);
        apply_sums(c, nj.j, nj.aligned, x.cols, x.ld, res ? res->ld : 0, slope, y.ld);
        return;
    }
    const size_t m = c.mark();
    float* stats = static_cast<float*>(c.raw(sizeof(float) * 2 * x.cols));
    float* rstats = (res && norm_res) ? static_cast<float*>(c.raw(sizeof(float) * 2 * x.cols)) : nullptr;
    const size_t wsb = pcrcg_instnorm_ws_bytes(x.cols);
    void* ws = c.raw(wsb);
    if (c.live())
        for (int g = 0; g < c.G; ++g) {
            col_stats(c, x, g, xs, stats, ws, wsb);
            if (rstats) col_stats(c, *res, g, rs, rstats, ws, wsb);
            c.check(pcrcg_instnorm_apply(x.p[g], x.rows[g], x.cols, x.ld, stats, res ? res->p[g] : nullptr, res ? res->ld : 0,
                                         rstats, slope, y.p[g], y.ld, c.st));
        }
    c.release(m);
}

void stats_into(GemmCall& call, Stat* st, int g) {
    if (!st) return;
    call.colstats = st->partials[g];
    call.colstats_bytes = st->bytes;
    call.h_chunks = &st->chunks[g];
    call.colstats_sums = st->sums;
}
struct Fold {
    Stat* sums = nullptr;
    float slope = 1.0f;
    bool accumulate = false;
};
GemmExtra extra_of(const Fold& f, const Mat& x, int g) {
    GemmExtra ex;
    if (f.sums) {
        ex.a_sums = static_cast<const double*>(f.sums->partials[g]);
        ex.a_count = (double)x.rows[g];
        ex.a_slope = f.slope;
    }
    ex.accumulate = f.accumulate;
    return ex;
}
GemmGroup group_of(const Ctx& c, const Mat& x, const Mat& y, bool c_zeroed, Stat* st, const float* const* row_scale, const Fold* f) {
    GemmGroup grp;
    grp.n = c.G - 1;
    for (int g = 1; g < c.G; ++g) {
        GemmPair& p = grp.p[g - 1];
        p.a = x.p[g];
        p.c = y.p[g];
        p.m = x.rows[g];
        p.row_scale = row_scale ? row_scale[g] : nullptr;
        p.colstats = st ? st->partials[g] : nullptr;
        p.h_chunks = st ? &st->chunks[g] : nullptr;
        p.c_zeroed = c_zeroed;
        if (f && f->sums) { p.a_sums = static_cast<const double*>(f->sums->partials[g]); p.a_count = (double)x.rows[g]; }
    }
    return grp;
}

void linear(Ctx& c, const Mat& x, const float* w, int ldw, const float* bias, const Mat& y, bool c_zeroed, Stat* st = nullptr,
            const float* const* row_scale = nullptr, const Fold* f = nullptr) {
    if (!c.live()) return;
    const bool grouped = c.paired();
    for (int g = 0; g < (grouped ? 1 : c.G); ++g) {
        GemmCall call;
        call.a = x.p[g]; call.lda = x.ld;
        call.b = w; call.ldb = ldw;
        call.c = y.p[g]; call.ldc = y.ld;
        call.m = x.rows[g]; call.n = y.cols; call.k = x.cols;
        call.row_scale = row_scale ? row_scale[g] : nullptr;
        call.bias = bias;
        call.st = c.st;
        stats_into(call, st, g);
        call.c_zeroed = c_zeroed;
        const GemmExtra ex = f ? extra_of(*f, x, g) : GemmExtra();
        const GemmGroup grp = grouped ? group_of(c, x, y, c_zeroed, st, row_scale, f) : GemmGroup();
        if (f) call.ex = &ex;
        if (grouped) call.grp = &grp;
        c.check(gemm_run(call));
    }
}
void linear(Ctx& c, const Mat& x, const float* w, int ldw, const float* bias, const Mat& y, Stat* st = nullptr,
            const float* const* row_scale = nullptr) {
    linear(c, x, w, ldw, bias, y, y.zeroed, st, row_scale);
}

bool lazy_stats_ready(Ctx& c, const Mat& x, Stat* xs) {
    if (!xs || !xs->sums || x.ld % 4 != 0 || x.cols > 4096) return false;
    fill_sums(c, x, xs);
    return true;
}
bool linear_norm(Ctx& c, const Mat& x, Stat* xs, float slope, const float* w, int ldw, const float* bias, const Mat& y,
                 Stat* st = nullptr) {
    if (!gemm_split_terms_on() || !lazy_stats_ready(c, x, xs)) return false;
    Fold f;
    f.sums = xs;
    f.slope = slope;
    linear(c, x, w, ldw, bias, y, y.zeroed, st, nullptr, &f);
    return true;
}

struct Batches { const pcrcg_batch* b[GMAX]; };

struct Walks {
    int* w[PCRCG_MAX_LEVELS][GMAX] = {};
    bool built[PCRCG_MAX_LEVELS] = {};
    int mode = 0;
};

static bool walk_pays(int mode, int ns, int cin, int nq) {
    if (mode != 1) return mode == 2;
    return (size_t)ns * (size_t)cin * sizeof(float) > (size_t)8 << 20 && nq >= 2048;
}

const int* const* level_walks(Ctx& c, const Batches& B, Walks& W, int l) {
    if (c.live() && !W.built[l]) {
        const float* pts[GMAX];
        int n[GMAX];
        for (int g = 0; g < c.G; ++g) { pts[g] = B.b[g]->points[l]; n[g] = B.b[g]->n_points[l]; }
        c.check(query_walk_multi(pts, n, W.w[l], nullptr, c.G, c.st));
        W.built[l] = true;
    }
    return W.w[l];
}

int kp_cin(const pcrcg_block& blk, const Mat& x) { return (blk.kp_w_pad && blk.cin_pad > x.cols) ? blk.cin_pad : x.cols; }
const float* kp_weight(const pcrcg_block& blk, const Mat& x) {
    return (blk.kp_w_pad && blk.cin_pad > 0 && kp_cin(blk, x) == blk.cin_pad) ? blk.kp_w_pad : blk.kp_w;
}

int kp_k(const pcrcg_block& blk, const Mat& x) {
    const int cin = kp_cin(blk, x);
    return (cin == 1 && blk.kp_wt) ? 16 : PCRCG_KPOINTS * cin;
}

void kpconv(Ctx& c, const Batches& B, Walks& W, const pcrcg_block& blk, const Mat& x, const Mat& y, Stat* st = nullptr,
            void* const* packed_ws = nullptr) {
    const int l = blk.layer;
    const size_t m = c.mark();
    Mat xin = x;
    const float* const w = kp_weight(blk, x);
    const int cin = kp_cin(blk, x);
    if (cin > x.cols) {
        xin = c.mat(x.rows, cin);
        if (c.live())
            for (int g = 0; g < c.G; ++g) {
                c.check(hipMemsetAsync(xin.p[g], 0, sizeof(float) * (size_t)x.rows[g] * cin, c.st) == hipSuccess ? PCRCG_OK
                                                                                                                   : PCRCG_ELAUNCH);
                c.check(pcrcg_copy2d(x.p[g], x.ld, xin.p[g], cin, x.rows[g], x.cols, c.st));
            }
    }
    int nq[GMAX], ns[GMAX];
    const float* q[GMAX];
    const pcrcg_table* tab[GMAX];
    float* inv_n[GMAX];
    void* ws[GMAX];
    size_t wsb[GMAX];
    for (int g = 0; g < c.G; ++g) {
        const pcrcg_batch& b = *B.b[g];
        tab[g] = blk.strided ? &b.pools[l] : &b.neighbors[l];
        q[g] = blk.strided ? b.points[l + 1] : b.points[l];
        nq[g] = blk.strided ? b.n_points[l + 1] : b.n_points[l];
        ns[g] = b.n_points[l];
        inv_n[g] = static_cast<float*>(c.raw(sizeof(float) * (nq[g] > 0 ? nq[g] : 1)));
        wsb[g] = pcrcg_kpconv_ws_bytes(ns[g]);
        ws[g] = (packed_ws && packed_ws[g]) ? packed_ws[g] : c.raw(wsb[g]);
    }
    const float* const kp_wt = blk.kp_wt;
    const int kk = kp_k(blk, x);
    const int* const* walks = (cin > 1 && walk_pays(W.mode, c.max_rows(ns), cin, c.max_rows(nq))) ? level_walks(c, B, W, blk.strided ? l + 1 : l) : nullptr;
    auto gather_call = [&](int g) {
        KpconvCall k;
        k.q_pts = q[g]; k.nq = nq[g]; k.s_pts = B.b[g]->points[l]; k.ns = ns[g];
        k.idx = tab[g]->idx; k.h = tab[g]->cols; k.ld_idx = tab[g]->ld;
        k.x = xin.p[g]; k.cin = cin; k.kp = blk.kp; k.extent = blk.extent;
        k.inv_n = inv_n[g]; k.ws = ws[g]; k.ws_bytes = wsb[g]; k.st = c.st;
        k.walk = walks ? walks[g] : nullptr;
        return k;
    };
    if (c.bf16 && kp_wt && cin % 32 == 0) {
        for (int g = 0; g < c.G; ++g) {
            void* xb = c.raw(sizeof(unsigned short) * (size_t)(ns[g] > 0 ? ns[g] : 1) * cin);
            void* wfb = c.raw(sizeof(unsigned short) * (size_t)(nq[g] > 0 ? nq[g] : 1) * kk);
            if (c.live()) {
                KpconvCall gather_bf16 = gather_call(g);
                gather_bf16.form = KpForm::bf16;
                gather_bf16.x_bf16 = static_cast<unsigned short*>(xb);
                gather_bf16.wf_bf16 = static_cast<unsigned short*>(wfb);
                c.check(kpconv_run(gather_bf16));
                GemmCall call;
                call.a = wfb; call.lda = kk; call.a_form = GemmA::row_bf16;
                call.b = kp_wt; call.ldb = kk;
                call.c = y.p[g]; call.ldc = y.ld;
                call.m = nq[g]; call.n = y.cols; call.k = kk;
                call.row_scale = inv_n[g];
                call.c_zeroed = y.zeroed;
                call.st = c.st;
                stats_into(call, st, g);
                c.check(gemm_run(call));
            }
        }
        c.release(m);
        return;
    }
    if (cin == 1 && st && st->sums && kpconv_c1_fused_ok(y.cols, kp_wt)) {
        if (c.live())
            for (int g = 0; g < c.G; ++g) {
                KpconvCall layer = gather_call(g);
                layer.form = KpForm::c1_fused;
                layer.wt = kp_wt; layer.cout = y.cols; layer.y = y.p[g]; layer.ld_y = y.ld;
                layer.sums = static_cast<double*>(st->partials[g]);
                c.check(kpconv_run(layer));
                st->chunks[g] = Stat::SUMS;
            }
        c.release(m);
        return;
    }
    Mat wf = c.mat(nq, kk);
    if (c.live()) {
        for (int g = 0; g < c.G; ++g) {
            KpconvCall gather = gather_call(g);
            gather.wf = wf.p[g];
            gather.pack = !(kk != 16 && packed_ws && packed_ws[g] && xin.p[g] == x.p[g]);
            gather.c1_ld = kk == 16 ? 16 : 0;
            c.check(kpconv_run(gather));
        }
        if (kp_wt)
            linear(c, wf, kp_wt, kk, nullptr, y, st, inv_n);
        else
            for (int g = 0; g < c.G; ++g)
                c.check(pcrcg_gemm_f32_colstats(wf.p[g], wf.ld, w, y.cols, 0, y.p[g], y.ld, nq[g], y.cols, kk, inv_n[g], nullptr,
                                                (st && !st->sums) ? st->partials[g] : nullptr, (st && !st->sums) ? st->bytes : 0,
                                                (st && !st->sums) ? &st->chunks[g] : nullptr, c.st));
    }
    c.release(m);
}

void out_rows(const Ctx& c, const Batches& B, const pcrcg_block& blk, int* rows) {
    for (int g = 0; g < GMAX; ++g)
        rows[g] = g < c.G ? (blk.strided ? B.b[g]->n_points[blk.layer + 1] : B.b[g]->n_points[blk.layer]) : 0;
}

Mat simple_block(Ctx& c, const Batches& B, Walks& W, const pcrcg_block& blk, const Mat& x) {
    int nq[GMAX];
    out_rows(c, B, blk, nq);
    Mat y = c.mat(nq, blk.mid_dim);
    const size_t m = c.mark();
    Mat t = c.gemm_out(nq, y.cols, kp_k(blk, x));
    Stat ts = stat_buffer(c, nq, t.cols);
    kpconv(c, B, W, blk, x, t, &ts);
    norm_act(c, t, 0.1f, y, &ts);
    c.release(m);
    return y;
}

bool norm_act_pack(Ctx& c, const Batches& B, int layer, const Mat& t, float slope, const Mat& u, Stat* ts, void* const* kp_ws,
                   const size_t* kp_ws_bytes) {
    if (c.bf16 || !instnorm_pack_ok(t.cols, t.ld, u.ld) || u.ld != u.cols) return false;
    const size_t m = c.mark();
    float* stats = static_cast<float*>(c.raw(sizeof(float) * 2 * t.cols));
    const size_t wsb = pcrcg_instnorm_ws_bytes(t.cols);
    void* ws = c.raw(wsb);
    fill_sums(c, t, ts);
    if (c.live() && all_sums(c, ts)) {
        NormJobs nj = norm_jobs(c, t, ts->partials, u);
        bool ok = nj.aligned;
        for (int g = 0; g < c.G; ++g) {
            nj.j[g].s_pts = B.b[g]->points[layer];
            nj.j[g].pk = kpconv_pk_ptr(kp_ws[g], kp_ws_bytes[g], t.rows[g]);
            ok = ok && nj.j[g].pk != nullptr;
        }
        if (ok) {
            c.check(instnorm_apply_sums_multi(nj.j, c.G, t.cols, t.ld, 1e-5f, 0, slope, u.ld, true, c.st));
            c.release(m);
            return true;
        }
    }
    if (c.live())
        for (int g = 0; g < c.G; ++g) {
            const float* s_pts = B.b[g]->points[layer];
            float4* pk = kpconv_pk_ptr(kp_ws[g], kp_ws_bytes[g], t.rows[g]);
            if (!pk) c.check(PCRCG_EWORKSPACE);
            else if (ts && ts->has_sums(g))
                c.check(instnorm_apply_pack(t.p[g], t.rows[g], t.cols, t.ld, nullptr, static_cast<const double*>(ts->partials[g]),
                                            (double)t.rows[g], 1e-5f, slope, u.p[g], u.ld, s_pts, pk, c.st));
            else {
                col_stats(c, t, g, ts, stats, ws, wsb);
                c.check(instnorm_apply_pack(t.p[g], t.rows[g], t.cols, t.ld, stats, nullptr, 0.0, 1e-5f, slope, u.p[g], u.ld, s_pts,
                                            pk, c.st));
            }
        }
    c.release(m);
    return true;
}

Mat resnet_block(Ctx& c, const Batches& B, Walks& W, const pcrcg_block& blk, const Mat& feats) {
    int nq[GMAX];
    out_rows(c, B, blk, nq);
    Mat y = c.mat(nq, blk.out_dim);
    const size_t m = c.mark();
    Mat x = feats;
    void* kp_ws[GMAX] = {};
    size_t kp_wsb[GMAX] = {};
    bool packed = false;
    if (blk.unary1) {
        Mat t = c.gemm_out(feats.rows, blk.mid_dim, feats.cols), u = c.mat(feats.rows, blk.mid_dim);
        Stat ts = stat_buffer(c, t.rows, t.cols);
        linear(c, feats, blk.unary1, feats.cols, nullptr, t, &ts);
        if (blk.mid_dim % 4 == 0 && !(blk.kp_w_pad && blk.cin_pad > blk.mid_dim)) {
            for (int g = 0; g < c.G; ++g) {
                kp_wsb[g] = pcrcg_kpconv_ws_bytes(feats.rows[g]);
                kp_ws[g] = c.raw(kp_wsb[g]);
            }
            packed = norm_act_pack(c, B, blk.layer, t, 0.1f, u, &ts, kp_ws, kp_wsb);
        }
        if (!packed) norm_act(c, t, 0.1f, u, &ts);
        x = u;
    }
    Mat k = c.gemm_out(nq, blk.mid_dim, PCRCG_KPOINTS * kp_cin(blk, x)), kn = c.mat(nq, blk.mid_dim);
    Stat ks = stat_buffer(c, nq, blk.mid_dim);
    kpconv(c, B, W, blk, x, k, &ks, packed ? kp_ws : nullptr);
    Mat u2 = c.gemm_out(nq, blk.out_dim, blk.mid_dim);
    Stat u2s = stat_buffer(c, nq, blk.out_dim);
    if (!linear_norm(c, k, &ks, 0.1f, blk.unary2, blk.mid_dim, nullptr, u2, &u2s)) {
        norm_act(c, k, 0.1f, kn, &ks);
        linear(c, kn, blk.unary2, blk.mid_dim, nullptr, u2, &u2s);
    }
    Mat sc = feats;
    if (blk.strided) {
        sc = c.mat(nq, feats.cols);
        if (c.live()) {
            GatherJob jobs[GMAX];
            const int* const* walks = walk_pays(W.mode, c.max_rows(feats.rows), feats.cols, c.max_rows(nq)) ? level_walks(c, B, W, blk.layer + 1) : nullptr;
            for (int g = 0; g < c.G; ++g) {
                const pcrcg_table& t = B.b[g]->pools[blk.layer];
                jobs[g] = GatherJob{feats.p[g], t.idx, sc.p[g], feats.rows[g], nq[g], t.cols, t.ld, walks ? walks[g] : nullptr};
            }
            c.check(gather_max_multi(jobs, c.G, feats.cols, c.st));
        }
    }
    if (blk.shortcut) {
        Mat s2 = c.gemm_out(nq, blk.out_dim, sc.cols);
        Stat s2s = stat_buffer(c, nq, blk.out_dim);
        linear(c, sc, blk.shortcut, sc.cols, nullptr, s2, &s2s);
        norm_act(c, u2, 0.1f, y, &u2s, &s2, true, &s2s);
    } else {
        norm_act(c, u2, 0.1f, y, &u2s, &sc, false);
    }
    c.release(m);
    return y;
}

void edge_norm(Ctx& c, const float* cn, int ld_cn, int cw, const int* idx, int n, int k, float* emax, int ld_emax, float* out,
               int ld_out, void* sums, bool sums_ok, float* stats, void* ws, size_t wsb) {
    if (sums && sums_ok) {
        c.check(pcrcg_edgeconv_reduce_sums(cn, ld_cn, cn + cw, ld_cn, idx, n, k, cw, emax, ld_emax, sums, c.st));
        c.check(pcrcg_instnorm_apply_sums(emax, n, cw, ld_emax, sums, (double)n * (double)k, 1e-5f, nullptr, 0, nullptr, 0.2f, out,
                                          ld_out, c.st));
        return;
    }
    c.check(pcrcg_edgeconv_reduce(cn, ld_cn, cn + cw, ld_cn, idx, n, k, cw, 1e-5f, emax, ld_emax, stats, ws, wsb, c.st));
    c.check(pcrcg_instnorm_apply(emax, n, cw, ld_emax, stats, nullptr, 0, nullptr, 0.2f, out, ld_out, c.st));
}

void edge_norm_all(Ctx& c, const Mat& cn, int cw, int* const* idx, const int* n, const int* k, const Mat& e, const Mat& out,
                   void* const* sums, bool sums_ok, float* stats, void* ws, size_t wsb) {
    bool multi = sums_ok;
    EdgeCloud cl[GMAX];
    for (int g = 0; g < c.G; ++g) {
        multi = multi && sums[g] != nullptr;
        cl[g] = EdgeCloud{cn.p[g], cn.p[g] + cw, idx[g], e.p[g], static_cast<double*>(sums[g]), n[g], k[g]};
    }
    if (multi && edgeconv_rows_ok(cl, c.G, cn.ld, cn.ld, e.ld, cw)) {
        c.check(edgeconv_rows_multi(cl, c.G, cn.ld, cn.ld, e.ld, cw, true, nullptr, c.st));
        NormJobs nj = norm_jobs(c, e, sums, out);
        bool one = nj.aligned;
        for (int g = 0; g < c.G; ++g) {
            nj.j[g].count = (double)n[g] * (double)k[g];
            one = one && n[g] > 0 && k[g] > 0;
        }
        apply_sums(c, nj.j, one, cw, e.ld, 0, 0.2f, out.ld);
        return;
    }
    for (int g = 0; g < c.G; ++g)
        edge_norm(c, cn.p[g], cn.ld, cw, idx[g], n[g], k[g], e.p[g], e.ld, out.p[g], out.ld, sums[g], sums_ok, stats, ws, wsb);
}

Mat self_attention(Ctx& c, const pcrcg_model& mdl, const pcrcg_gnn_layer& gl, const float* const* coords, const Mat& f,
                   int* const* knn_given = nullptr) {
    const int ch = f.cols;
    Mat y = c.mat(f.rows, ch);
    const size_t m = c.mark();
    int kq[GMAX];
    int* idx[GMAX];
    for (int g = 0; g < c.G; ++g) {
        const int n = f.rows[g];
        kq[g] = mdl.knn_k < n - 1 ? mdl.knn_k : n - 1;
        idx[g] = knn_given ? knn_given[g] : static_cast<int*>(c.raw(sizeof(int) * (size_t)n * (kq[g] > 0 ? kq[g] : 1)));
    }
    Mat cat = c.mat(f.rows, 4 * ch);
    const size_t wsb = pcrcg_edgeconv_ws_bytes(2 * ch);
    void* ws = c.raw(wsb);
    float* stats = static_cast<float*>(c.raw(sizeof(float) * 4 * ch));
    Mat cn1 = c.gemm_out(f.rows, 2 * ch, ch), e1 = c.mat(f.rows, ch), cn2 = c.gemm_out(f.rows, 4 * ch, ch), e2 = c.mat(f.rows, 2 * ch);
    Mat x3 = c.gemm_out(f.rows, ch, 4 * ch);
    Stat x3s = stat_buffer(c, f.rows, ch);
    void *sums1[GMAX], *sums2[GMAX];
    for (int g = 0; g < c.G; ++g) {
        sums1[g] = gemm_split_terms_on() ? c.zraw(2 * sizeof(double) * (size_t)ch) : nullptr;
        sums2[g] = gemm_split_terms_on() ? c.zraw(2 * sizeof(double) * (size_t)(2 * ch)) : nullptr;
    }
    Mat cat1 = cols(cat, ch, ch), cat2 = cols(cat, 2 * ch, 2 * ch);
    const bool ok1 = sums_apply_ok(e1, cat1, nullptr), ok2 = sums_apply_ok(e2, cat2, nullptr);
    if (c.live()) {
        if (!knn_given)
            for (int g = 0; g < c.G; ++g) c.check(pcrcg_knn(coords[g], f.rows[g], kq[g], idx[g], c.st));
        c.check(copy2d_multi(f.p, cat.p, f.rows, c.G, f.ld, cat.ld, ch, c.st));
        linear(c, f, gl.edge1, ch, nullptr, cn1);
        edge_norm_all(c, cn1, ch, idx, f.rows, kq, e1, cat1, sums1, ok1, stats, ws, wsb);
        linear(c, cat1, gl.edge2, ch, nullptr, cn2);
        edge_norm_all(c, cn2, 2 * ch, idx, f.rows, kq, e2, cat2, sums2, ok2, stats, ws, wsb);
        linear(c, cat, gl.conv3, 4 * ch, nullptr, x3, &x3s);
    }
    norm_act(c, x3, 0.2f, y, &x3s);
    c.release(m);
    return y;
}

Mat cross_attention(Ctx& c, const pcrcg_model& mdl, const pcrcg_gnn_layer& gl, const Mat& x, const Mat& src, const Mat* q_given = nullptr) {
    const int ch = x.cols, h = mdl.heads, d = ch / h;
    Mat y = c.mat(x.rows, ch);
    const size_t m = c.mark();
    const bool kv_fused = gl.wv == gl.wk + (size_t)ch * ch && gl.bv == gl.bk + ch;
    Mat q = q_given ? *q_given : c.gemm_out(x.rows, ch, ch), kk, v, msg = c.mat(x.rows, ch);
    if (kv_fused) {
        Mat kv = c.gemm_out(src.rows, 2 * ch, ch);
        linear(c, src, gl.wk, ch, gl.bk, kv);
        kk = cols(kv, 0, ch);
        v = cols(kv, ch, ch);
        kk.zeroed = v.zeroed = false;
    } else {
        kk = c.gemm_out(src.rows, ch, ch);
        v = c.gemm_out(src.rows, ch, ch);
    }
    Mat sc = c.mat(x.rows, c.max_rows(src.rows));
    Mat cat = c.mat(x.rows, 2 * ch), h0 = c.gemm_out(x.rows, 2 * ch, 2 * ch), h1 = c.mat(x.rows, 2 * ch), delta = c.gemm_out(x.rows, ch, 2 * ch);
    if (!q_given) linear(c, x, gl.wq, ch, gl.bq, q);
    if (!kv_fused) {
        linear(c, src, gl.wk, ch, gl.bk, kk);
        linear(c, src, gl.wv, ch, gl.bv, v);
    }
    bool att_done = false;
    if (c.live()) {
        AttnCloud cl[GMAX];
        for (int g = 0; g < c.G; ++g) cl[g] = AttnCloud{q.p[g], kk.p[g], v.p[g], msg.p[g], x.rows[g], src.rows[g]};
        if (attention_mfma_ok(cl, c.G, q.ld, kk.ld, v.ld, d)) {
            c.check(attention_mfma_multi(cl, c.G, q.ld, kk.ld, v.ld, msg.ld, h, d, 1.0f / sqrtf((float)d), c.st));
            att_done = true;
        }
    }
    if (c.live())
        for (int g = 0; g < c.G; ++g) {
            const int n = x.rows[g], ms = src.rows[g];
            if (att_done) {
            } else if (pcrcg_attention_supported(d) && (long)n * ms <= 1000000) {
                c.check(pcrcg_attention(q.p[g], q.ld, kk.p[g], kk.ld, v.p[g], v.ld, msg.p[g], msg.ld, n, ms, h, d,
                                        1.0f / sqrtf((float)d), c.st));
            } else {
                for (int i = 0; i < h; ++i) {
                    c.check(pcrcg_gemm_f32(q.p[g] + i * d, q.ld, kk.p[g] + i * d, kk.ld, 1, sc.p[g], ms, n, ms, d, nullptr, nullptr,
                                           c.st));
                    c.check(pcrcg_softmax_rows(sc.p[g], n, ms, ms, 1.0f / sqrtf((float)d), c.st));
                    c.check(pcrcg_gemm_f32(sc.p[g], ms, v.p[g] + i * d, v.ld, 0, msg.p[g] + i * d, msg.ld, n, d, ms, nullptr, nullptr,
                                           c.st));
                }
            }
        }
    if (c.live()) c.check(copy2d_multi(x.p, cat.p, x.rows, c.G, x.ld, cat.ld, ch, c.st));
    linear(c, msg, gl.wm, ch, gl.bm, cols(cat, ch, ch));
    Stat h0s = stat_buffer(c, x.rows, 2 * ch);
    linear(c, cat, gl.w0, 2 * ch, gl.b0, h0, &h0s);
    if (!linear_norm(c, h0, &h0s, 0.0f, gl.w3, 2 * ch, gl.b3, delta)) {
        norm_act(c, h0, 0.0f, h1, &h0s);
        linear(c, h1, gl.w3, 2 * ch, gl.b3, delta);
    }
    if (c.live())
        for (int g = 0; g < c.G; ++g) c.check(pcrcg_add(x.p[g], delta.p[g], y.p[g], (long)x.rows[g] * ch, c.st));
    c.release(m);
    return y;
}

void forward(Ctx& c, const pcrcg_model& mdl, const Batches& B, const pcrcg_outputs* out) {
    const int L = B.b[0]->n_levels;
    c.bf16 = mdl.feature_bf16 != 0;
    Mat x;
    for (int g = 0; g < c.G; ++g) {
        x.p[g] = const_cast<float*>(B.b[g]->features);
        x.rows[g] = B.b[g]->n_points[0];
    }
    x.cols = x.ld = B.b[0]->feat_dim;
    std::vector<Mat> skips;
    Walks W;
    W.mode = debug_opts().walk;
    if (W.mode)
        for (int l = 0; l < L; ++l)
            for (int g = 0; g < c.G; ++g) {
                const int n = B.b[g]->n_points[l];
                W.w[l][g] = static_cast<int*>(c.raw(sizeof(int) * (size_t)(n > 0 ? n : 1)));
            }
    for (int i = 0; i < mdl.n_enc; ++i) {
        if (mdl.enc_skip[i]) skips.push_back(x);
        const pcrcg_block& blk = mdl.enc[i];
        x = blk.type == PCRCG_BLK_SIMPLE ? simple_block(c, B, W, blk, x) : resnet_block(c, B, W, blk, x);
    }
    const int gd = mdl.gnn_dim;
    int nc[GMAX] = {}, ns[GMAX] = {}, nt[GMAX] = {}, zero[GMAX] = {};
    const float *c0[GMAX], *c1[GMAX];
    for (int g = 0; g < c.G; ++g) {
        nc[g] = B.b[g]->n_points[L - 1];
        ns[g] = B.b[g]->len_src_c;
        nt[g] = nc[g] - ns[g];
        c0[g] = B.b[g]->points[L - 1];
        c1[g] = B.b[g]->points[L - 1] + 3 * (long)ns[g];
    }
    Mat fc = c.gemm_out(nc, gd, mdl.enc_out_dim);
    linear(c, x, mdl.bottle_w, mdl.enc_out_dim, mdl.bottle_b, fc);
    Mat d0 = rows(fc, zero, ns), d1 = rows(fc, ns, nt);
    int* knn0[GMAX] = {};
    int* knn1[GMAX] = {};
    int n_self = 0;
    for (int i = 0; i < mdl.n_gnn; ++i) n_self += mdl.gnn[i].cross ? 0 : 1;
    const bool knn_once = n_self >= 2;
    if (knn_once)
        for (int g = 0; g < c.G; ++g) {
            const int k0 = mdl.knn_k < ns[g] - 1 ? mdl.knn_k : ns[g] - 1, k1 = mdl.knn_k < nt[g] - 1 ? mdl.knn_k : nt[g] - 1;
            knn0[g] = static_cast<int*>(c.raw(sizeof(int) * (size_t)ns[g] * (k0 > 0 ? k0 : 1)));
            knn1[g] = static_cast<int*>(c.raw(sizeof(int) * (size_t)nt[g] * (k1 > 0 ? k1 : 1)));
            if (c.live()) {
                c.check(pcrcg_knn(c0[g], ns[g], k0, knn0[g], c.st));
                c.check(pcrcg_knn(c1[g], nt[g], k1, knn1[g], c.st));
            }
        }
    const int G0 = c.G;
    const bool stack = 2 * G0 <= GMAX && gemm_split_terms_on();
    const float* c01[GMAX] = {};
    int* knn01[GMAX] = {};
    for (int g = 0; g < G0 && stack; ++g) { c01[g] = c0[g]; c01[G0 + g] = c1[g]; knn01[g] = knn0[g]; knn01[G0 + g] = knn1[g]; }
    for (int i = 0; i < mdl.n_gnn; ++i) {
        const pcrcg_gnn_layer& gl = mdl.gnn[i];
        if (gl.cross) {
            Mat q0, q1;
            if (stack) {
                const int ch = d0.cols;
                const Mat x2 = stacked(d0, d1, G0);
                const Mat q2 = c.twice([&] { Mat q = c.gemm_out(x2.rows, ch, ch); linear(c, x2, gl.wq, ch, gl.bq, q); return q; });
                q0 = half(q2, 0, G0);
                q1 = half(q2, 1, G0);
            }
            d0 = cross_attention(c, mdl, gl, d0, d1, stack ? &q0 : nullptr);
            d1 = cross_attention(c, mdl, gl, d1, d0, stack ? &q1 : nullptr);
        } else if (stack) {
            const Mat f2 = stacked(d0, d1, G0);
            const Mat y2 = c.twice([&] { return self_attention(c, mdl, gl, c01, f2, knn_once ? knn01 : nullptr); });
            d0 = half(y2, 0, G0);
            d1 = half(y2, 1, G0);
        } else {
            d0 = self_attention(c, mdl, gl, c0, d0, knn_once ? knn0 : nullptr);
            d1 = self_attention(c, mdl, gl, c1, d1, knn_once ? knn1 : nullptr);
        }
    }
    const int wc = gd + 2;
    Mat xc = c.mat(nc, wc, pad4(wc));
    {
        const size_t m = c.mark();
        Mat gcat = c.mat(nc, gd), fn = c.mat(nc, gd);
        Mat pst = c.mat(ns, c.max_rows(nt)), pts = c.mat(nt, c.max_rows(ns));
        if (c.live())
            for (int g = 0; g < c.G; ++g) {
                c.check(pcrcg_copy2d(d0.p[g], d0.ld, gcat.p[g], gcat.ld, ns[g], gd, c.st));
                c.check(pcrcg_copy2d(d1.p[g], d1.ld, gcat.p[g] + (long)ns[g] * gcat.ld, gcat.ld, nt[g], gd, c.st));
            }
        Mat feats = cols(xc, 2, gd), score = cols(xc, 0, 1), sal = cols(xc, 1, 1);
        linear(c, gcat, mdl.proj_gnn_w, gd, mdl.proj_gnn_b, feats);
        linear(c, feats, mdl.proj_score_w, gd, mdl.proj_score_b, score);
        if (c.live())
            for (int g = 0; g < c.G; ++g) {
                c.check(pcrcg_l2norm_rows(feats.p[g], feats.ld, fn.p[g], fn.ld, nc[g], gd, c.st));
                const float inv_t = 1.0f / mdl.temperature;
                const float* fs = fn.p[g];
                const float* ft = fn.p[g] + (long)ns[g] * fn.ld;
                c.check(pcrcg_gemm_f32(fs, fn.ld, ft, fn.ld, 1, pst.p[g], nt[g], ns[g], nt[g], gd, nullptr, nullptr, c.st));
                c.check(pcrcg_softmax_matvec(pst.p[g], ns[g], nt[g], nt[g], inv_t, score.p[g] + (long)ns[g] * xc.ld, xc.ld, sal.p[g],
                                             xc.ld, c.st));
                c.check(pcrcg_gemm_f32(ft, fn.ld, fs, fn.ld, 1, pts.p[g], ns[g], nt[g], ns[g], gd, nullptr, nullptr, c.st));
                c.check(pcrcg_softmax_matvec(pts.p[g], nt[g], ns[g], ns[g], inv_t, score.p[g], xc.ld, sal.p[g] + (long)ns[g] * xc.ld,
                                             xc.ld, c.st));
            }
        c.release(m);
    }
    x = xc;
    Stat xs;
    bool lazy = false;
    auto materialise = [&]() {
        if (!lazy) return;
        Mat y = c.mat(x.rows, x.cols);
        norm_act(c, x, 0.1f, y, &xs);
        x = y;
        lazy = false;
    };
    for (int j = 0; j < mdl.n_dec; ++j) {
        const pcrcg_block& blk = mdl.dec[j];
        if (blk.type == PCRCG_BLK_UPSAMPLE) {
            const pcrcg_table* tabs[GMAX];
            int trows[GMAX] = {};
            for (int g = 0; g < c.G; ++g) { tabs[g] = &B.b[g]->upsamples[blk.layer - 1]; trows[g] = tabs[g]->rows; }
            const bool concat = j + 1 < mdl.n_dec && mdl.dec_concat[j + 1];
            const int cs = concat ? skips.back().cols : 0;
            const pcrcg_block* next = j + 1 < mdl.n_dec ? &mdl.dec[j + 1] : nullptr;
            if (concat && next && next->mlp_skip && next->skip_dim == cs && gemm_split_terms_on() &&
                (next->type == PCRCG_BLK_UNARY || next->type == PCRCG_BLK_LAST_UNARY) && x.ld % 4 == 0 &&
                skips.back().ld % 4 == 0) {
                const Mat& sk = skips.back();
                const bool last = next->type == PCRCG_BLK_LAST_UNARY;
                Mat tt = c.mat(trows, next->out_dim, pad4(next->out_dim));
                if (lazy && !(gemm_split_terms_on() && lazy_stats_ready(c, x, &xs))) materialise();
                Mat z = c.gemm_out(x.rows, next->out_dim, x.cols, pad4(next->out_dim));
                Fold up, add;
                up.sums = lazy ? &xs : nullptr;
                up.slope = 0.1f;
                add.accumulate = true;
                linear(c, x, next->mlp, next->mlp_ld, nullptr, z, z.zeroed, nullptr, nullptr, &up);
                if (c.live()) {
                    FirstJob jobs[GMAX];
                    for (int g = 0; g < c.G; ++g) jobs[g] = FirstJob{z.p[g], tabs[g]->idx, tt.p[g], z.rows[g], trows[g], tabs[g]->ld};
                    c.check(gather_first_multi(jobs, c.G, z.cols, z.ld, tt.ld, c.st));
                }
                linear(c, sk, next->mlp_skip, next->mlp_skip_ld, nullptr, tt, true, nullptr, nullptr, &add);
                skips.pop_back();
                lazy = false;
                x = tt;
                if (!last) {
                    xs = stat_buffer(c, tt.rows, tt.cols);
                    lazy = true;
                }
                ++j;
                continue;
            }
            materialise();
            Mat y = c.mat(trows, x.cols + cs, pad4(x.cols + cs));
            Mat xd = x;
            if (x.ld != x.cols) {
                xd = c.mat(x.rows, x.cols);
                if (c.live())
                    for (int g = 0; g < c.G; ++g) c.check(pcrcg_copy2d(x.p[g], x.ld, xd.p[g], xd.ld, x.rows[g], x.cols, c.st));
            }
            if (c.live())
                for (int g = 0; g < c.G; ++g) {
                    c.check(pcrcg_gather_first(xd.p[g], xd.rows[g], xd.cols, tabs[g]->idx, tabs[g]->rows, tabs[g]->ld, y.p[g], y.ld, c.st));
                    if (concat) {
                        const Mat& s = skips.back();
                        c.check(pcrcg_copy2d(s.p[g], s.ld, y.p[g] + x.cols, y.ld, s.rows[g], s.cols, c.st));
                    }
                }
            if (concat) skips.pop_back();
            x = y;
        } else if (blk.type == PCRCG_BLK_UNARY) {
            materialise();
// ... 102 lines not shown
```

pcrcg_amd/ops.py:

```python
import ctypes

import torch

from . import _lib

_F32, _I32, _I64 = torch.float32, torch.int32, torch.int64


def _stream():
    return torch.cuda.current_stream().cuda_stream


def _dev(t, dtype, name):
    if not isinstance(t, torch.Tensor) or not t.is_cuda:
        raise RuntimeError(f"pcrcg_amd: `{name}` must be a tensor on a HIP device (no CPU fallback exists)")
    if t.dtype != dtype:
        raise RuntimeError(f"pcrcg_amd: `{name}` must have dtype {dtype}, got {t.dtype}")
    return t


def _rows(t, dtype, name):
    _dev(t, dtype, name)
    if t.dim() != 2:
        raise RuntimeError(f"pcrcg_amd: `{name}` must be 2-D")
# ... 759 lines not shown

def edgeconv_reduce_sums(ctr, nbr, idx):
    L = _lib.lib()
    ctr, ld_ctr = _rows(ctr, _F32, "ctr")
    nbr, ld_nbr = _rows(nbr, _F32, "nbr")
    idx = _dev(idx, _I32, "idx").contiguous()
    n, c = ctr.shape
    emax = torch.empty((n, c), dtype=_F32, device=ctr.device)
    sums = torch.zeros((2, c), dtype=torch.float64, device=ctr.device)
    _lib.check(L.pcrcg_edgeconv_reduce_sums(ctr.data_ptr(), ld_ctr, nbr.data_ptr(), ld_nbr, idx.data_ptr(), n, idx.shape[1],
                                            c, emax.data_ptr(), c, sums.data_ptr(), _stream()), "pcrcg_edgeconv_reduce_sums")
    return emax, sums


def softmax_rows_(x, scale=1.0):
    L = _lib.lib()
    x_, ld = _rows(x, _F32, "x")
    if x_.data_ptr() != x.data_ptr():
        raise RuntimeError("pcrcg_amd.softmax_rows_: tensor must have unit inner stride")
    _lib.check(L.pcrcg_softmax_rows(x.data_ptr(), x.shape[0], x.shape[1], ld, float(scale), _stream()),
               "pcrcg_softmax_rows")
    return x


def attention(q, k, v, heads, scale=None):
    L = _lib.lib()
    q, ldq = _rows(q, _F32, "q")
    k, ldk = _rows(k, _F32, "k")
    v, ldv = _rows(v, _F32, "v")
    n, ch = q.shape
    ms = k.shape[0]
    d = ch // heads
    if d * heads != ch or k.shape[1] != ch or v.shape != k.shape or not L.pcrcg_attention_supported(d):
        raise RuntimeError(f"pcrcg_amd.attention: unsupported widths ({ch} channels, {heads} heads)")
    out = torch.empty((n, ch), dtype=_F32, device=q.device)
    _lib.check(L.pcrcg_attention(q.data_ptr(), ldq, k.data_ptr(), ldk, v.data_ptr(), ldv, out.data_ptr(), ch, n, ms, heads,
                                 d, float(d ** -0.5 if scale is None else scale), _stream()), "pcrcg_attention")
    return out


def softmax_matvec(x, vec, scale=1.0):
    L = _lib.lib()
    x, ld = _rows(x, _F32, "x")
    vec = _dev(vec, _F32, "vec")
    if vec.dim() != 1 or vec.shape[0] != x.shape[1]:
        raise RuntimeError("pcrcg_amd.softmax_matvec: vec must be 1-D with x.shape[1] entries")
    y = torch.empty(x.shape[0], dtype=_F32, device=x.device)
    _lib.check(L.pcrcg_softmax_matvec(x.data_ptr(), x.shape[0], x.shape[1], ld, float(scale), vec.data_ptr(),
                                      int(vec.stride(0)) if vec.shape[0] > 1 else 1, y.data_ptr(), 1, _stream()),
               "pcrcg_softmax_matvec")
    return y


def feature_argmax(a, b, want_best=False):
    L = _lib.lib()
    a, lda = _rows(a, _F32, "a")
    b, ldb = _rows(b, _F32, "b")
    n, c = a.shape
    m = b.shape[0]
    if b.shape[1] != c:
        raise RuntimeError("pcrcg_amd.feature_argmax: feature widths differ")
    if m == 0:
        raise RuntimeError("pcrcg_amd.feature_argmax: `b` has no rows")
    arg = torch.empty(n, dtype=_I64, device=a.device)
    best = torch.empty(n, dtype=_F32, device=a.device) if want_best else None
    nbytes = L.pcrcg_feature_argmax_ws_bytes(n)
    ws = _ws.get("feature_argmax", nbytes, a.device)
    _lib.check(L.pcrcg_feature_argmax(a.data_ptr(), lda, n, b.data_ptr(), ldb, m, c, arg.data_ptr(), _ptr(best),
                                      ws.data_ptr(), nbytes, _stream()), "pcrcg_feature_argmax")
    return (arg, best) if want_best else arg


POSE_HEAD_WIDTH = 1024
POSE_HEAD_ROWS = 64


def _pose_head_args(h, w_q, w_t, what):
    h, ld_h = _rows(h, _F32, "h")
    n, width = h.shape
    w_q, w_t = _dev(w_q, _F32, "w_q").contiguous(), _dev(w_t, _F32, "w_t").contiguous()
    if tuple(w_q.shape) != (4, width) or tuple(w_t.shape) != (3, width):
        raise RuntimeError(f"pcrcg_amd.{what}: w_q must be [4, {width}] and w_t [3, {width}]")
    nbytes = _lib.lib().pcrcg_pose_head_ws_bytes(n, width)
    if nbytes == 0:
        _lib.check(-1, "pcrcg_pose_head_ws_bytes")
    return h, ld_h, n, width, w_q, w_t, nbytes, _ws.get("pose_head", nbytes, h.device)


def pose_head(h, w_q, b_q, w_t, b_t, want_rows=False):
    L = _lib.lib()
    h, ld_h, n, width, w_q, w_t, nbytes, ws = _pose_head_args(h, w_q, w_t, "pose_head")
    b_q, b_t = _dev(b_q, _F32, "b_q").contiguous(), _dev(b_t, _F32, "b_t").contiguous()
    if b_q.numel() != 4 or b_t.numel() != 3:
        raise RuntimeError("pcrcg_amd.pose_head: b_q must have 4 entries and b_t 3")
    out = torch.empty(7, dtype=_F32, device=h.device)
    q_rows = torch.empty((n, 4), dtype=_F32, device=h.device) if want_rows else None
    _lib.check(L.pcrcg_pose_head(h.data_ptr(), ld_h, n, width, w_q.data_ptr(), b_q.data_ptr(), w_t.data_ptr(), b_t.data_ptr(),
                                 out.data_ptr(), _ptr(q_rows), ws.data_ptr(), nbytes, _stream()), "pcrcg_pose_head")
    return out[:4], out[4:], q_rows


def pose_head_backward(h, w_q, w_t, q_rows, g, dh=None):
    L = _lib.lib()
    h, ld_h, n, width, w_q, w_t, nbytes, ws = _pose_head_args(h, w_q, w_t, "pose_head_backward")
    q_rows = _dev(q_rows, _F32, "q_rows").contiguous()
    g = _dev(g, _F32, "g").contiguous()
# ... 15 lines not shown
```

Before: 623.6.

## Batch GNN stage kernels across clouds and fuse bidirectional softmax-matvec

Generalises several GNN-stage kernels (knn, add, l2norm, edgeconv, attention, copy) to take up to eight clouds per launch through a blockIdx.y pointer table, cutting per-cloud launch count. The saliency step replaces two GEMMs plus two row softmax-matvecs with a single GEMM and one pairs kernel that reads the score matrix both row-wise and column-wise (via a shared-memory column reduction), removing the transposed GEMM. The projection is also applied per fragment directly rather than through a concatenation copy. Column-wise strided reads of the score matrix may be less coalesced than the old transposed-matrix path.

Result: no change. 628.7, median of 6 (+0.8%).

```diff
diff --git a/include/pcrcg.h b/include/pcrcg.h
--- a/include/pcrcg.h
+++ b/include/pcrcg.h
@@ -187,6 +187,16 @@
                     int ms, int heads, int d, float scale, void* stream);
 int pcrcg_softmax_matvec(const float* x, int rows, int cols, int ld, float scale, const float* vec, int ldv, float* y,
                          int ldy, void* stream);
+int pcrcg_softmax_matvec_pairs(const float* const* s, const int* ns, const int* nt, const int* ld, const float* const* score_s,
+                               const float* const* score_t, float* const* s1, float* const* s2, int count, float scale, int ld_vec,
+                               void* stream);
+int pcrcg_knn_multi(const float* const* coords, const int* n, const int* k, int* const* idx, int count, void* stream);
+int pcrcg_edgeconv_reduce_sums_multi(const float* const* ctr, const float* const* nbr, const int* const* idx, const int* n,
+                                     const int* k, float* const* emax, void* const* sums, int count, int ld_ctr, int ld_nbr,
+                                     int ld_emax, int c, void* stream);
+int pcrcg_attention_multi(const float* const* q, const float* const* k, const float* const* v, float* const* out, const int* n,
+                          const int* ms, int count, int ldq, int ldk, int ldv, int ldo, int heads, int d, float scale,
+                          void* stream);
 
 int pcrcg_check_status(const int* status, void* stream);
 
@@ -194,6 +204,9 @@
 int pcrcg_add(const float* a, const float* b, float* dst, long n, void* stream);
 int pcrcg_l2norm_rows(const float* src, int ld_src, float* dst, int ld_dst, int rows, int cols, void* stream);
 int pcrcg_sigmoid_scores(const float* src, int ld_src, float* dst, int rows, void* stream);
+int pcrcg_add_multi(const float* const* a, const float* const* b, float* const* dst, const long* n, int count, void* stream);
+int pcrcg_l2norm_rows_multi(const float* const* src, float* const* dst, const int* rows, int count, int ld_src, int ld_dst,
+                            int cols, void* stream);
 
 #define PCRCG_MAX_LEVELS 8
 #define PCRCG_MAX_BLOCKS 32
diff --git a/pcrcg_amd/_lib.py b/pcrcg_amd/_lib.py
--- a/pcrcg_amd/_lib.py
+++ b/pcrcg_amd/_lib.py
@@ -112,6 +112,15 @@
     "pcrcg_attention": (c_int, [c_void_p, c_int, c_void_p, c_int, c_void_p, c_int, c_void_p, c_int, c_int, c_int, c_int,
                                 c_int, c_float, c_void_p]),
     "pcrcg_softmax_matvec": (c_int, [c_void_p, c_int, c_int, c_int, c_float, c_void_p, c_int, c_void_p, c_int, c_void_p]),
+    "pcrcg_softmax_matvec_pairs": (c_int, [c_void_p, c_void_p, c_void_p, c_void_p, c_void_p, c_void_p, c_void_p, c_void_p, c_int,
+                                           c_float, c_int, c_void_p]),
+    "pcrcg_knn_multi": (c_int, [c_void_p, c_void_p, c_void_p, c_void_p, c_int, c_void_p]),
+    "pcrcg_edgeconv_reduce_sums_multi": (c_int, [c_void_p, c_void_p, c_void_p, c_void_p, c_void_p, c_void_p, c_void_p, c_int, c_int,
+                                                 c_int, c_int, c_int, c_void_p]),
+    "pcrcg_attention_multi": (c_int, [c_void_p, c_void_p, c_void_p, c_void_p, c_void_p, c_void_p, c_int, c_int, c_int, c_int, c_int,
+                                      c_int, c_int, c_float, c_void_p]),
+    "pcrcg_add_multi": (c_int, [c_void_p, c_void_p, c_void_p, c_void_p, c_int, c_void_p]),
+    "pcrcg_l2norm_rows_multi": (c_int, [c_void_p, c_void_p, c_void_p, c_int, c_int, c_int, c_int, c_void_p]),
     "pcrcg_copy2d": (c_int, [c_void_p, c_int, c_void_p, c_int, c_int, c_int, c_void_p]),
     "pcrcg_add": (c_int, [c_void_p, c_void_p, c_void_p, ctypes.c_long, c_void_p]),
     "pcrcg_l2norm_rows": (c_int, [c_void_p, c_int, c_void_p, c_int, c_int, c_int, c_void_p]),
diff --git a/pcrcg_amd/csrc/common.h b/pcrcg_amd/csrc/common.h
--- a/pcrcg_amd/csrc/common.h
+++ b/pcrcg_amd/csrc/common.h
@@ -35,6 +35,9 @@
 int exclusive_scan_i32(const int* in, int* out, int n, int* total, void* ws, hipStream_t stream);
 
 constexpr int kWave = 64;
+
+constexpr int GMAX = 4;
+constexpr int CMAX = 2 * GMAX;
 
 bool instnorm_pack_ok(int c, int ldx, int ldy);
 int instnorm_apply_pack(const float* x, int n, int c, int ldx, const float* stats, const double* sums, double count, float eps,
@@ -77,6 +80,14 @@
 int copy2d_multi(const float* const* src, float* const* dst, const int* rows, int count, int ld_src, int ld_dst, int cols,
                  hipStream_t st);
 int instnorm_colsums_multi(const float* const* x, double* const* sums, const int* n, int count, int c, int ldx, hipStream_t st);
+int add_multi(const float* const* a, const float* const* b, float* const* dst, const long* n, int count, hipStream_t st);
+int l2norm_rows_multi(const float* const* src, float* const* dst, const int* rows, int count, int ld_src, int ld_dst, int cols,
+                      hipStream_t st);
+
+int knn_multi(const float* const* coords, const int* n, const int* k, int* const* idx, int count, hipStream_t st);
+
+struct SalPair { const float* s; const float* score_s; const float* score_t; float* s1; float* s2; int ns, nt, ld; };
+int softmax_matvec_pairs(const SalPair* pairs, int count, float scale, int ld_vec, hipStream_t st);
 
 struct EdgeCloud {
     const float* ctr; const float* nbr; const int* idx; float* emax; double* sums; int n, k;
diff --git a/pcrcg_amd/csrc/elementwise.hip b/pcrcg_amd/csrc/elementwise.hip
--- a/pcrcg_amd/csrc/elementwise.hip
+++ b/pcrcg_amd/csrc/elementwise.hip
@@ -4,7 +4,7 @@
 namespace pcrcg {
 namespace {
 
-struct CopyMulti { const float* src[4]; float* dst[4]; int rows[4]; };
+struct CopyMulti { const float* src[CMAX]; float* dst[CMAX]; int rows[CMAX]; };
 __global__ void __launch_bounds__(256) k_copy2d(CopyMulti mm, int ld_src, int ld_dst, int cols) {
     const float* __restrict__ src = mm.src[blockIdx.y];
     float* __restrict__ dst = mm.dst[blockIdx.y];
@@ -16,14 +16,19 @@
     dst[r * ld_dst + c] = src[r * ld_src + c];
 }
 
-__global__ void __launch_bounds__(256) k_add(const float* __restrict__ a, const float* __restrict__ b,
-                                              float* __restrict__ dst, long n) {
+struct AddMulti { const float* a[CMAX]; const float* b[CMAX]; float* dst[CMAX]; long n[CMAX]; };
+__global__ void __launch_bounds__(256) k_add(AddMulti mm) {
+    const float* __restrict__ a = mm.a[blockIdx.y];
+    const float* __restrict__ b = mm.b[blockIdx.y];
+    float* __restrict__ dst = mm.dst[blockIdx.y];
     const long e = (long)blockIdx.x * blockDim.x + threadIdx.x;
-    if (e < n) dst[e] = a[e] + b[e];
-}
-
-__global__ void __launch_bounds__(256) k_l2norm_rows(const float* __restrict__ src, int ld_src, float* __restrict__ dst,
-                                                      int ld_dst, int rows, int cols) {
+    if (e < mm.n[blockIdx.y]) dst[e] = a[e] + b[e];
+}
+
+__global__ void __launch_bounds__(256) k_l2norm_rows(CopyMulti mm, int ld_src, int ld_dst, int cols) {
+    const float* __restrict__ src = mm.src[blockIdx.y];
+    float* __restrict__ dst = mm.dst[blockIdx.y];
+    const int rows = mm.rows[blockIdx.y];
     const int lane = threadIdx.x & 63;
     const int r = blockIdx.x * 4 + (threadIdx.x >> 6);
     if (r >= rows) return;
@@ -115,10 +120,10 @@
 
 int copy2d_multi(const float* const* src, float* const* dst, const int* rows, int count, int ld_src, int ld_dst, int cols,
                  hipStream_t st) {
-    PCRCG_CHECK_ARG(count >= 1 && count <= 4 && cols >= 0 && ld_src >= cols && ld_dst >= cols);
+    PCRCG_CHECK_ARG(count >= 1 && count <= CMAX && cols >= 0 && ld_src >= cols && ld_dst >= cols);
     CopyMulti mm;
     int rmax = 0;
-    for (int g = 0; g < 4; ++g) {
+    for (int g = 0; g < CMAX; ++g) {
         const int k = g < count ? g : 0;
         mm.src[g] = src[k]; mm.dst[g] = dst[k]; mm.rows[g] = g < count ? rows[k] : 0;
         if (g < count) {
@@ -129,6 +134,41 @@
     if (rmax == 0 || cols == 0) return PCRCG_OK;
     const long total = (long)rmax * cols;
     hipLaunchKernelGGL(k_copy2d, dim3((unsigned)((total + 255) / 256), count), dim3(256), 0, st, mm, ld_src, ld_dst, cols);
+    PCRCG_CHECK_LAUNCH();
+    return PCRCG_OK;
+}
+int add_multi(const float* const* a, const float* const* b, float* const* dst, const long* n, int count, hipStream_t st) {
+    PCRCG_CHECK_ARG(count >= 1 && count <= CMAX);
+    AddMulti mm;
+    long nmax = 0;
+    for (int g = 0; g < CMAX; ++g) {
+        const int k = g < count ? g : 0;
+        mm.a[g] = a[k]; mm.b[g] = b[k]; mm.dst[g] = dst[k]; mm.n[g] = g < count ? n[k] : 0;
+        if (g < count) {
+            PCRCG_CHECK_ARG(n[k] >= 0 && (n[k] == 0 || (a[k] && b[k] && dst[k])));
+            nmax = n[k] > nmax ? n[k] : nmax;
+        }
+    }
+    if (nmax == 0) return PCRCG_OK;
+    hipLaunchKernelGGL(k_add, dim3((unsigned)((nmax + 255) / 256), count), dim3(256), 0, st, mm);
+    PCRCG_CHECK_LAUNCH();
+    return PCRCG_OK;
+}
+int l2norm_rows_multi(const float* const* src, float* const* dst, const int* rows, int count, int ld_src, int ld_dst, int cols,
+                      hipStream_t st) {
+    PCRCG_CHECK_ARG(count >= 1 && count <= CMAX && cols >= 1 && ld_src >= cols && ld_dst >= cols);
+    CopyMulti mm;
+    int rmax = 0;
+    for (int g = 0; g < CMAX; ++g) {
+        const int k = g < count ? g : 0;
+        mm.src[g] = src[k]; mm.dst[g] = dst[k]; mm.rows[g] = g < count ? rows[k] : 0;
+        if (g < count) {
+            PCRCG_CHECK_ARG(rows[k] >= 0 && (rows[k] == 0 || (src[k] && dst[k])));
+            rmax = rows[k] > rmax ? rows[k] : rmax;
+        }
+    }
+    if (rmax == 0) return PCRCG_OK;
+    hipLaunchKernelGGL(k_l2norm_rows, dim3((rmax + 3) / 4, count), dim3(256), 0, st, mm, ld_src, ld_dst, cols);
     PCRCG_CHECK_LAUNCH();
     return PCRCG_OK;
 }
@@ -243,19 +283,25 @@
     PCRCG_CHECK_ARG(n >= 0);
     if (n == 0) return PCRCG_OK;
     PCRCG_CHECK_ARG(a && b && dst);
-    hipLaunchKernelGGL(k_add, dim3((unsigned)((n + 255) / 256)), dim3(256), 0, as_stream(stream), a, b, dst, n);
-    PCRCG_CHECK_LAUNCH();
-    return PCRCG_OK;
+    return pcrcg::add_multi(&a, &b, &dst, &n, 1, as_stream(stream));
 }
 
 int pcrcg_l2norm_rows(const float* src, int ld_src, float* dst, int ld_dst, int rows, int cols, void* stream) {
     PCRCG_CHECK_ARG(rows >= 0 && cols >= 1 && ld_src >= cols && ld_dst >= cols);
     if (rows == 0) return PCRCG_OK;
     PCRCG_CHECK_ARG(src && dst);
-    hipLaunchKernelGGL(k_l2norm_rows, dim3((rows + 3) / 4), dim3(256), 0, as_stream(stream), src, ld_src, dst, ld_dst,
-                       rows, cols);
-    PCRCG_CHECK_LAUNCH();
-    return PCRCG_OK;
+    return pcrcg::l2norm_rows_multi(&src, &dst, &rows, 1, ld_src, ld_dst, cols, as_stream(stream));
+}
+
+int pcrcg_add_multi(const float* const* a, const float* const* b, float* const* dst, const long* n, int count, void* stream) {
+    PCRCG_CHECK_ARG(a && b && dst && n);
+    return pcrcg::add_multi(a, b, dst, n, count, as_stream(stream));
+}
+
+int pcrcg_l2norm_rows_multi(const float* const* src, float* const* dst, const int* rows, int count, int ld_src, int ld_dst,
+                            int cols, void* stream) {
+    PCRCG_CHECK_ARG(src && dst && rows);
+    return pcrcg::l2norm_rows_multi(src, dst, rows, count, ld_src, ld_dst, cols, as_stream(stream));
 }
 
 int pcrcg_sigmoid_scores(const float* src, int ld_src, float* dst, int rows, void* stream) {
diff --git a/pcrcg_amd/csrc/gnn.hip b/pcrcg_amd/csrc/gnn.hip
--- a/pcrcg_amd/csrc/gnn.hip
+++ b/pcrcg_amd/csrc/gnn.hip
@@ -155,7 +155,12 @@
     if (lane >= 1 && lane < K) out[lane - 1] = (int)(a[lane] & 0xFFFFFFFFull);
 }
 
-__global__ void __launch_bounds__(256) k_knn(const float* __restrict__ coords, int n, int k, int* __restrict__ idx) {
+struct KnnMulti { const float* coords[CMAX]; int* idx[CMAX]; int n[CMAX], k[CMAX]; };
+
+__global__ void __launch_bounds__(256) k_knn(KnnMulti mm) {
+    const float* __restrict__ coords = mm.coords[blockIdx.y];
+    int* __restrict__ idx = mm.idx[blockIdx.y];
+    const int n = mm.n[blockIdx.y], k = mm.k[blockIdx.y];
     const int lane = threadIdx.x & 63;
     const int i = blockIdx.x * 4 + (threadIdx.x >> 6);
     if (i >= n) return;
@@ -188,7 +193,10 @@
 }
 
 template <int PER>
-__global__ void __launch_bounds__(256) k_knn_reg(const float* __restrict__ coords, int n, int k, int* __restrict__ idx) {
+__global__ void __launch_bounds__(256) k_knn_reg(KnnMulti mm) {
+    const float* __restrict__ coords = mm.coords[blockIdx.y];
+    int* __restrict__ idx = mm.idx[blockIdx.y];
+    const int n = mm.n[blockIdx.y], k = mm.k[blockIdx.y];
     const int lane = threadIdx.x & 63;
     const int i = blockIdx.x * 4 + (threadIdx.x >> 6);
     if (i >= n) return;
@@ -225,7 +233,7 @@
 }
 
 struct AttCloud { const float* q; const float* k; const float* v; float* out; int n, ms; };
-struct AttMulti { AttCloud cl[4]; int ldq, ldk, ldv, ldo; float scale; int chunk_blocks; };
+struct AttMulti { AttCloud cl[CMAX]; int ldq, ldk, ldv, ldo; float scale; int chunk_blocks; };
 
 typedef float attf16 __attribute__((ext_vector_type(16)));
 
@@ -549,7 +557,7 @@
     }
 }
 
-struct EdgeMulti { EdgeCloud cl[4]; int ld_ctr, ld_nbr, ld_emax, c, rows_per_block, nchunks; };
+struct EdgeMulti { EdgeCloud cl[CMAX]; int ld_ctr, ld_nbr, ld_emax, c, rows_per_block, nchunks; };
 
 template <bool ATOMIC>
 __global__ void __launch_bounds__(256) k_edgeconv_rows(EdgeMulti a) {
@@ -756,35 +764,85 @@
     }
 }
 
+__device__ __forceinline__ float softmax_matvec_row(const float* __restrict__ row, int cols, float scale,
+                                                    const float* __restrict__ vec, int ldv, int lane) {
+    float m = -INFINITY;
+    for (int j = lane; j < cols; j += 64) m = fmaxf(m, row[j] * scale);
+#pragma unroll
+    for (int s = 32; s >= 1; s >>= 1) m = fmaxf(m, __shfl_xor(m, s, 64));
+    float sum = 0.f, dot = 0.f;
+    for (int j = lane; j < cols; j += 64) {
+        const float e = expf(row[j] * scale - m);
+        sum += e;
+        dot = fmaf(e, vec[(long)j * ldv], dot);
+    }
+#pragma unroll
+    for (int s = 32; s >= 1; s >>= 1) {
+        sum += __shfl_xor(sum, s, 64);
+        dot += __shfl_xor(dot, s, 64);
+    }
+    return dot / sum;
+}
 __global__ void __launch_bounds__(256) k_softmax_matvec(const float* __restrict__ x, int rows, int cols, int ld, float scale,
                                                         const float* __restrict__ vec, int ldv, float* __restrict__ y,
                                                         int ldy) {
     const int lane = threadIdx.x & 63;
     const int r = blockIdx.x * 4 + (threadIdx.x >> 6);
     if (r >= rows) return;
-    const float* row = x + (long)r * ld;
+    const float v = softmax_matvec_row(x + (long)r * ld, cols, scale, vec, ldv, lane);
+    if (lane == 0) y[(long)r * ldy] = v;
+}
+
+struct SalMulti { SalPair p[GMAX]; };
+__global__ void __launch_bounds__(256) k_softmax_matvec_pairs(SalMulti mm, float scale, int ld_vec, int row_blocks) {
+    const SalPair p = mm.p[blockIdx.y];
+    if ((int)blockIdx.x < row_blocks) {
+        const int lane = threadIdx.x & 63;
+        const int r = blockIdx.x * 4 + (threadIdx.x >> 6);
+        if (r >= p.ns) return;
+        const float v = softmax_matvec_row(p.s + (long)r * p.ld, p.nt, scale, p.score_t, ld_vec, lane);
+        if (lane == 0) p.s1[(long)r * ld_vec] = v;
+        return;
+    }
+    __shared__ float s_a[16][17], s_b[16][17];
+    const int c0 = ((int)blockIdx.x - row_blocks) * 16;
+    if (c0 >= p.nt) return;
+    const int c = threadIdx.x & 15, rl = threadIdx.x >> 4;
+    const bool ok = c0 + c < p.nt;
+    const float* __restrict__ col = p.s + (ok ? c0 + c : p.nt - 1);
     float m = -INFINITY;
-    for (int j = lane; j < cols; j += 64) m = fmaxf(m, row[j] * scale);
-#pragma unroll
-    for (int s = 32; s >= 1; s >>= 1) m = fmaxf(m, __shfl_xor(m, s, 64));
+    for (int i = rl; i < p.ns; i += 16) m = fmaxf(m, col[(long)i * p.ld] * scale);
+    s_a[rl][c] = m;
+    __syncthreads();
+    m = s_a[0][c];
+#pragma unroll
+    for (int t = 1; t < 16; ++t) m = fmaxf(m, s_a[t][c]);
+    __syncthreads();
     float sum = 0.f, dot = 0.f;
-    for (int j = lane; j < cols; j += 64) {
-        const float e = expf(row[j] * scale - m);
+    for (int i = rl; i < p.ns; i += 16) {
+        const float e = expf(col[(long)i * p.ld] * scale - m);
         sum += e;
-        dot = fmaf(e, vec[(long)j * ldv], dot);
-    }
-#pragma unroll
-    for (int s = 32; s >= 1; s >>= 1) {
-        sum += __shfl_xor(sum, s, 64);
-        dot += __shfl_xor(dot, s, 64);
-    }
-    if (lane == 0) y[(long)r * ldy] = dot / sum;
+        dot = fmaf(e, p.score_s[(long)i * ld_vec], dot);
+    }
+    s_a[rl][c] = sum;
+    s_b[rl][c] = dot;
+    __syncthreads();
+    if (rl == 0 && ok) {
+        float a[16], b[16];
+#pragma unroll
+        for (int t = 0; t < 16; ++t) { a[t] = s_a[t][c]; b[t] = s_b[t][c]; }
+#pragma unroll
+        for (int w = 8; w >= 1; w >>= 1)
+#pragma unroll
+            for (int t = 0; t < w; ++t) { a[t] += a[t + w]; b[t] += b[t + w]; }
+        p.s2[(long)(c0 + c) * ld_vec] = b[0] / a[0];
+    }
 }
 
 }
 
 bool edgeconv_rows_ok(const EdgeCloud* cl, int count, int ld_ctr, int ld_nbr, int ld_emax, int c) {
-    if (count < 1 || count > 4 || c % 4 != 0 || ld_ctr % 4 != 0 || ld_nbr % 4 != 0 || ld_emax % 4 != 0) return false;
+    if (count < 1 || count > CMAX || c % 4 != 0 || ld_ctr % 4 != 0 || ld_nbr % 4 != 0 || ld_emax % 4 != 0) return false;
     for (int i = 0; i < count; ++i) {
         if (cl[i].k < 1 || cl[i].k > 64 || cl[i].n < 1) return false;
         if ((reinterpret_cast<uintptr_t>(cl[i].ctr) | reinterpret_cast<uintptr_t>(cl[i].nbr) | reinterpret_cast<uintptr_t>(cl[i].emax)) & 15)
@@ -794,10 +852,11 @@
 }
 int edgeconv_rows_multi(const EdgeCloud* cl, int count, int ld_ctr, int ld_nbr, int ld_emax, int c, bool atomic, int* nchunks_out,
                         hipStream_t st) {
+    PCRCG_CHECK_ARG(cl && count >= 1 && count <= CMAX);
     EdgeMulti a;
     int nmax = 0;
     for (int i = 0; i < count; ++i) { a.cl[i] = cl[i]; nmax = cl[i].n > nmax ? cl[i].n : nmax; }
-    for (int i = count; i < 4; ++i) a.cl[i] = cl[0];
+    for (int i = count; i < CMAX; ++i) a.cl[i] = cl[0];
     a.ld_ctr = ld_ctr; a.ld_nbr = ld_nbr; a.ld_emax = ld_emax; a.c = c;
     int rpb = 8;
     while ((nmax + rpb - 1) / rpb > colstats_chunks()) rpb += 4;
@@ -816,7 +875,7 @@
     return (int)((budget / (32 * sizeof(float)) - 1) / 32);
 }
 bool attention_mfma_ok(const AttnCloud* cl, int count, int ldq, int ldk, int ldv, int d) {
-    if (!debug_opts().att_mfma || count < 1 || count > 4 || (d != 32 && d != 64 && d != 128)) return false;
+    if (!debug_opts().att_mfma || count < 1 || count > CMAX || (d != 32 && d != 64 && d != 128)) return false;
     if (ldq % 4 != 0 || ldk % 4 != 0 || ldv % 4 != 0) return false;
     for (int i = 0; i < count; ++i) {
         if (cl[i].n < 1 || cl[i].ms < 1) return false;
@@ -826,9 +885,10 @@
 }
 int attention_mfma_multi(const AttnCloud* cl, int count, int ldq, int ldk, int ldv, int ldo, int heads, int d, float scale,
                          hipStream_t st) {
+    PCRCG_CHECK_ARG(cl && count >= 1 && count <= CMAX);
     AttMulti a;
     int nmax = 0, msmax = 0;
-    for (int i = 0; i < 4; ++i) {
+    for (int i = 0; i < CMAX; ++i) {
         const AttnCloud& c = cl[i < count ? i : 0];
         a.cl[i] = AttCloud{c.q, c.k, c.v, c.out, c.n, c.ms};
         if (i < count) { nmax = c.n > nmax ? c.n : nmax; msmax = c.ms > msmax ? c.ms : msmax; }
@@ -848,6 +908,44 @@
     else if (d == 64) ATT2(64);
     else ATT2(32);
 #undef ATT2
+    PCRCG_CHECK_LAUNCH();
+    return PCRCG_OK;
+}
+int knn_multi(const float* const* coords, const int* n, const int* k, int* const* idx, int count, hipStream_t st) {
+    PCRCG_CHECK_ARG(coords && n && k && idx && count >= 1 && count <= CMAX);
+    KnnMulti mm;
+    int nmax = 0;
+    for (int g = 0; g < CMAX; ++g) {
+        const int i = g < count ? g : 0;
+        mm.coords[g] = coords[i]; mm.idx[g] = idx[i]; mm.n[g] = g < count ? n[i] : 0; mm.k[g] = k[i];
+        if (g < count) {
+            PCRCG_CHECK_ARG(n[i] >= 0 && (n[i] == 0 || (k[i] >= 1 && coords[i] && idx[i])));
+            nmax = n[i] > nmax ? n[i] : nmax;
+        }
+    }
+    if (nmax == 0) return PCRCG_OK;
+    const dim3 grid((nmax + 3) / 4, count);
+    if (nmax <= 64 * 8) hipLaunchKernelGGL(k_knn_reg<8>, grid, dim3(256), 0, st, mm);
+    else if (nmax <= 64 * 16) hipLaunchKernelGGL(k_knn_reg<16>, grid, dim3(256), 0, st, mm);
+    else hipLaunchKernelGGL(k_knn, grid, dim3(256), 0, st, mm);
+    PCRCG_CHECK_LAUNCH();
+    return PCRCG_OK;
+}
+int softmax_matvec_pairs(const SalPair* pairs, int count, float scale, int ld_vec, hipStream_t st) {
+    PCRCG_CHECK_ARG(pairs && count >= 1 && count <= GMAX && ld_vec >= 1);
+    SalMulti mm;
+    int ns_max = 0, nt_max = 0;
+    for (int g = 0; g < GMAX; ++g) {
+        mm.p[g] = pairs[g < count ? g : 0];
+        if (g >= count) { mm.p[g].ns = 0; mm.p[g].nt = 0; continue; }
+        const SalPair& p = pairs[g];
+        PCRCG_CHECK_ARG(p.ns >= 1 && p.nt >= 1 && p.ld >= p.nt && p.s && p.score_s && p.score_t && p.s1 && p.s2);
+        ns_max = p.ns > ns_max ? p.ns : ns_max;
+        nt_max = p.nt > nt_max ? p.nt : nt_max;
+    }
+    const int row_blocks = (ns_max + 3) / 4;
+    hipLaunchKernelGGL(k_softmax_matvec_pairs, dim3(row_blocks + (nt_max + 15) / 16, count), dim3(256), 0, st, mm, scale, ld_vec,
+                       row_blocks);
     PCRCG_CHECK_LAUNCH();
     return PCRCG_OK;
 }
@@ -889,14 +987,7 @@
     PCRCG_CHECK_ARG(n >= 0 && k >= 1);
     if (n == 0) return PCRCG_OK;
     PCRCG_CHECK_ARG(coords && idx);
-    if (n <= 64 * 8)
-        hipLaunchKernelGGL(k_knn_reg<8>, dim3((n + 3) / 4), dim3(256), 0, as_stream(stream), coords, n, k, idx);
-    else if (n <= 64 * 16)
-        hipLaunchKernelGGL(k_knn_reg<16>, dim3((n + 3) / 4), dim3(256), 0, as_stream(stream), coords, n, k, idx);
-    else
-        hipLaunchKernelGGL(k_knn, dim3((n + 3) / 4), dim3(256), 0, as_stream(stream), coords, n, k, idx);
-    PCRCG_CHECK_LAUNCH();
-    return PCRCG_OK;
+    return knn_multi(&coords, &n, &k, &idx, 1, as_stream(stream));
 }
 
 size_t pcrcg_edgeconv_ws_bytes(int c) { return colstats_ws_bytes(c); }
@@ -1000,6 +1091,47 @@
     return PCRCG_OK;
 }
 
+int pcrcg_softmax_matvec_pairs(const float* const* s, const int* ns, const int* nt, const int* ld, const float* const* score_s,
+                               const float* const* score_t, float* const* s1, float* const* s2, int count, float scale, int ld_vec,
+                               void* stream) {
+    PCRCG_CHECK_ARG(s && ns && nt && ld && score_s && score_t && s1 && s2 && count >= 1 && count <= GMAX);
+    SalPair p[GMAX];
+    for (int g = 0; g < count; ++g) p[g] = SalPair{s[g], score_s[g], score_t[g], s1[g], s2[g], ns[g], nt[g], ld[g]};
+    return softmax_matvec_pairs(p, count, scale, ld_vec, as_stream(stream));
+}
+
+int pcrcg_knn_multi(const float* const* coords, const int* n, const int* k, int* const* idx, int count, void* stream) {
+    return knn_multi(coords, n, k, idx, count, as_stream(stream));
+}
+
+int pcrcg_edgeconv_reduce_sums_multi(const float* const* ctr, const float* const* nbr, const int* const* idx, const int* n,
+                                     const int* k, float* const* emax, void* const* sums, int count, int ld_ctr, int ld_nbr,
+                                     int ld_emax, int c, void* stream) {
+    PCRCG_CHECK_ARG(ctr && nbr && idx && n && k && emax && sums && count >= 1 && count <= CMAX);
+    PCRCG_CHECK_ARG(c >= 1 && ld_ctr >= c && ld_nbr >= c && ld_emax >= c);
+    EdgeCloud cl[CMAX];
+    for (int g = 0; g < count; ++g) {
+        PCRCG_CHECK_ARG(ctr[g] && nbr[g] && idx[g] && emax[g] && sums[g]);
+        cl[g] = EdgeCloud{ctr[g], nbr[g], idx[g], emax[g], static_cast<double*>(sums[g]), n[g], k[g]};
+    }
+    PCRCG_CHECK_ARG(edgeconv_rows_ok(cl, count, ld_ctr, ld_nbr, ld_emax, c));
+    return edgeconv_rows_multi(cl, count, ld_ctr, ld_nbr, ld_emax, c, true, nullptr, as_stream(stream));
+}
+
+int pcrcg_attention_multi(const float* const* q, const float* const* k, const float* const* v, float* const* out, const int* n,
+                          const int* ms, int count, int ldq, int ldk, int ldv, int ldo, int heads, int d, float scale,
+                          void* stream) {
+    PCRCG_CHECK_ARG(q && k && v && out && n && ms && count >= 1 && count <= CMAX && heads >= 1);
+    PCRCG_CHECK_ARG(ldq >= heads * d && ldk >= heads * d && ldv >= heads * d && ldo >= heads * d);
+    AttnCloud cl[CMAX];
+    for (int g = 0; g < count; ++g) {
+        PCRCG_CHECK_ARG(q[g] && k[g] && v[g] && out[g] && (reinterpret_cast<uintptr_t>(v[g]) & 15) == 0);
+        cl[g] = AttnCloud{q[g], k[g], v[g], out[g], n[g], ms[g]};
+    }
+    PCRCG_CHECK_ARG(attention_mfma_ok(cl, count, ldq, ldk, ldv, d));
+    return attention_mfma_multi(cl, count, ldq, ldk, ldv, ldo, heads, d, scale, as_stream(stream));
+}
+
 int pcrcg_softmax_rows(float* x, int rows, int cols, int ld, float scale, void* stream) {
     PCRCG_CHECK_ARG(rows >= 0 && cols >= 1 && ld >= cols);
     if (rows == 0) return PCRCG_OK;
diff --git a/pcrcg_amd/csrc/pointops.hip b/pcrcg_amd/csrc/pointops.hip
--- a/pcrcg_amd/csrc/pointops.hip
+++ b/pcrcg_amd/csrc/pointops.hip
@@ -97,7 +97,7 @@
 
 constexpr int kStatChunks = 128;
 
-struct ColsMulti { const float* x[4]; double* partial[4]; int n[4]; };
+struct ColsMulti { const float* x[CMAX]; double* partial[CMAX]; int n[CMAX]; };
 template <bool ATOMIC>
 __global__ void __launch_bounds__(256) k_colstats_partial(ColsMulti mm, int c, int ldx) {
     const float* __restrict__ x = mm.x[blockIdx.z];
@@ -225,10 +225,10 @@
 }
 
 struct NormMulti {
-    const float* x[4]; const double* sums[4]; const float* res[4]; const double* res_sums[4]; float* y[4];
-    const float* s_pts[4]; float4* pk[4];
-    int n[4]; double count[4];
-    float* stats_out[4];
+    const float* x[CMAX]; const double* sums[CMAX]; const float* res[CMAX]; const double* res_sums[CMAX]; float* y[CMAX];
+    const float* s_pts[CMAX]; float4* pk[CMAX];
+    int n[CMAX]; double count[CMAX];
+    float* stats_out[CMAX];
 };
 template <int RES>
 __global__ void __launch_bounds__(256) k_instnorm_apply4_sums(NormMulti mm, int c4, int ldx, float eps, int ldr, float slope, int ldy,
@@ -367,11 +367,11 @@
 }
 int instnorm_apply_sums_multi(const NormJob* jobs, int count, int c, int ldx, float eps, int ldr, float slope, int ldy, bool pack,
                               hipStream_t st) {
-    PCRCG_CHECK_ARG(jobs && count >= 1 && count <= 4 && c >= 4 && c % 4 == 0);
+    PCRCG_CHECK_ARG(jobs && count >= 1 && count <= CMAX && c >= 4 && c % 4 == 0);
     const int c4 = c / 4;
     NormMulti mm;
     int nmax = 0;
-    for (int g = 0; g < 4; ++g) {
+    for (int g = 0; g < CMAX; ++g) {
         const NormJob& j = jobs[g < count ? g : 0];
         mm.x[g] = j.x; mm.sums[g] = j.sums; mm.res[g] = j.res; mm.res_sums[g] = j.res_sums; mm.y[g] = j.y;
         mm.s_pts[g] = j.s_pts; mm.pk[g] = j.pk; mm.n[g] = g < count ? j.n : 0; mm.count[g] = j.count;
@@ -462,10 +462,10 @@
 }
 
 int instnorm_colsums_multi(const float* const* x, double* const* sums, const int* n, int count, int c, int ldx, hipStream_t st) {
-    PCRCG_CHECK_ARG(count >= 1 && count <= 4 && c >= 1 && ldx >= c);
+    PCRCG_CHECK_ARG(count >= 1 && count <= CMAX && c >= 1 && ldx >= c);
     ColsMulti mm;
     int nmax = 0;
-    for (int g = 0; g < 4; ++g) {
+    for (int g = 0; g < CMAX; ++g) {
         const int k = g < count ? g : 0;
         PCRCG_CHECK_ARG(n[k] >= 1 && x[k] && sums[k]);
         mm.x[g] = x[k]; mm.partial[g] = sums[k]; mm.n[g] = n[k];
diff --git a/pcrcg_amd/csrc/runner.hip b/pcrcg_amd/csrc/runner.hip
--- a/pcrcg_amd/csrc/runner.hip
+++ b/pcrcg_amd/csrc/runner.hip
@@ -8,16 +8,17 @@
 namespace pcrcg {
 namespace {
 
-constexpr int GMAX = 4;
-static_assert(GMAX <= 4, "instnorm_apply_sums_multi, instnorm_colsums_multi, gather_max_multi, gather_first_multi, copy2d_multi, heads_multi, "
-                         "edgeconv_rows_multi and attention_mfma_multi (common.h) take up to four clouds");
+static_assert(CMAX == 2 * GMAX && GMAX == 4, "forward() stacks the two clouds of up to GMAX pairs: 2 * GMAX clouds per multi-cloud launch, "
+                                             "and linear() splits them into launches of four products (GemmGroup)");
 
 struct Mat {
-    float* p[GMAX] = {};
-    int rows[GMAX] = {};
+    float* p[CMAX] = {};
+    int rows[CMAX] = {};
     int cols = 0, ld = 0;
     bool zeroed = false;
 };
+
+constexpr int kGemmClouds = 4;
 
 struct Ctx {
     char* base = nullptr;
@@ -62,9 +63,14 @@
     }
     int max_rows(const int* rows) const { int m = rows[0]; for (int g = 1; g < G; ++g) m = rows[g] > m ? rows[g] : m; return m; }
     Mat gemm_out(const int* rows, int cols, int k, int ld = 0) {
-        long total = 0;
-        for (int g = 0; g < G; ++g) total += rows[g];
-        if (!gemm_bt_accumulates(max_rows(rows), cols, k, total)) return mat(rows, cols, ld);
+        bool acc = false;
+        for (int g0 = 0; g0 < G; g0 += kGemmClouds) {
+            long total = 0;
+            int mr = 0;
+            for (int g = g0; g < G && g < g0 + kGemmClouds; ++g) { total += rows[g]; mr = rows[g] > mr ? rows[g] : mr; }
+            acc = acc || gemm_bt_accumulates(mr, cols, k, total);
+        }
+        if (!acc) return mat(rows, cols, ld);
         Mat m;
         m.cols = cols; m.ld = ld ? ld : cols;
         for (int g = 0; g < G; ++g) {
@@ -85,13 +91,13 @@
 inline int pad4(int v) { return (v + 3) & ~3; }
 inline Mat cols(const Mat& m, int c0, int n) {
     Mat r = m;
-    for (int g = 0; g < GMAX; ++g) r.p[g] = m.p[g] ? m.p[g] + c0 : nullptr;
+    for (int g = 0; g < CMAX; ++g) r.p[g] = m.p[g] ? m.p[g] + c0 : nullptr;
     r.cols = n;
     return r;
 }
 inline Mat rows(const Mat& m, const int* r0, const int* n) {
     Mat r = m;
-    for (int g = 0; g < GMAX; ++g) {
+    for (int g = 0; g < CMAX; ++g) {
         r.p[g] = m.p[g] ? m.p[g] + (long)r0[g] * m.ld : nullptr;
         r.rows[g] = n[g];
     }
@@ -104,7 +110,7 @@
 }
 inline Mat half(const Mat& m, int which, int G0) {
     Mat r = m;
-    for (int g = 0; g < GMAX; ++g) {
+    for (int g = 0; g < CMAX; ++g) {
         r.p[g] = g < G0 ? m.p[which * G0 + g] : nullptr;
         r.rows[g] = g < G0 ? m.rows[which * G0 + g] : 0;
     }
@@ -112,9 +118,9 @@
 }
 
 struct Stat {
-    void* partials[GMAX] = {};
+    void* partials[CMAX] = {};
     size_t bytes = 0;
-    int chunks[GMAX] = {};
+    int chunks[CMAX] = {};
     bool sums = false;
     static constexpr int SUMS = -1, NOTHING = 0;
     bool has_sums(int g) const { return chunks[g] == SUMS; }
@@ -150,7 +156,7 @@
 void fill_sums(Ctx& c, const Mat& x, Stat* xs) {
     if (!c.live() || !xs || !xs->sums) return;
     {
-        const float* xp[GMAX]; double* sp[GMAX]; int np[GMAX]; int idx[GMAX]; int cnt = 0;
+        const float* xp[CMAX]; double* sp[CMAX]; int np[CMAX]; int idx[CMAX]; int cnt = 0;
         for (int g = 0; g < c.G; ++g)
             if (xs->nothing(g) && x.rows[g] >= 1) { xp[cnt] = x.p[g]; sp[cnt] = static_cast<double*>(xs->partials[g]); np[cnt] = x.rows[g]; idx[cnt++] = g; }
         if (cnt >= 2) {
@@ -172,7 +178,7 @@
 }
 
 struct NormJobs {
-    NormJob j[GMAX];
+    NormJob j[CMAX];
     bool aligned = true;
 };
 NormJobs norm_jobs(const Ctx& c, const Mat& x, void* const* sums, const Mat& y, const Mat* res = nullptr, void* const* res_sums = nullptr) {
@@ -242,11 +248,11 @@
     ex.accumulate = f.accumulate;
     return ex;
 }
-GemmGroup group_of(const Ctx& c, const Mat& x, const Mat& y, bool c_zeroed, Stat* st, const float* const* row_scale, const Fold* f) {
+GemmGroup group_of(const Mat& x, const Mat& y, int g0, int g1, bool c_zeroed, Stat* st, const float* const* row_scale, const Fold* f) {
     GemmGroup grp;
-    grp.n = c.G - 1;
-    for (int g = 1; g < c.G; ++g) {
-        GemmPair& p = grp.p[g - 1];
+    grp.n = g1 - g0 - 1;
+    for (int g = g0 + 1; g < g1; ++g) {
+        GemmPair& p = grp.p[g - g0 - 1];
         p.a = x.p[g];
         p.c = y.p[g];
         p.m = x.rows[g];
@@ -263,7 +269,9 @@
             const float* const* row_scale = nullptr, const Fold* f = nullptr) {
     if (!c.live()) return;
     const bool grouped = c.paired();
-    for (int g = 0; g < (grouped ? 1 : c.G); ++g) {
+    const int per = grouped ? kGemmClouds : 1;
+    for (int g = 0; g < c.G; g += per) {
+        const int g1 = g + per < c.G ? g + per : c.G;
         GemmCall call;
         call.a = x.p[g]; call.lda = x.ld;
         call.b = w; call.ldb = ldw;
@@ -275,7 +283,7 @@
         stats_into(call, st, g);
         call.c_zeroed = c_zeroed;
         const GemmExtra ex = f ? extra_of(*f, x, g) : GemmExtra();
-        const GemmGroup grp = grouped ? group_of(c, x, y, c_zeroed, st, row_scale, f) : GemmGroup();
+        const GemmGroup grp = grouped ? group_of(x, y, g, g1, c_zeroed, st, row_scale, f) : GemmGroup();
         if (f) call.ex = &ex;
         if (grouped) call.grp = &grp;
         c.check(gemm_run(call));
@@ -304,7 +312,7 @@
 struct Batches { const pcrcg_batch* b[GMAX]; };
 
 struct Walks {
-    int* w[PCRCG_MAX_LEVELS][GMAX] = {};
+    int* w[PCRCG_MAX_LEVELS][CMAX] = {};
     bool built[PCRCG_MAX_LEVELS] = {};
     int mode = 0;
 };
@@ -316,8 +324,8 @@
 
 const int* const* level_walks(Ctx& c, const Batches& B, Walks& W, int l) {
     if (c.live() && !W.built[l]) {
-        const float* pts[GMAX];
-        int n[GMAX];
+        const float* pts[CMAX];
+        int n[CMAX];
         for (int g = 0; g < c.G; ++g) { pts[g] = B.b[g]->points[l]; n[g] = B.b[g]->n_points[l]; }
         c.check(query_walk_multi(pts, n, W.w[l], nullptr, c.G, c.st));
         W.built[l] = true;
@@ -351,12 +359,12 @@
                 c.check(pcrcg_copy2d(x.p[g], x.ld, xin.p[g], cin, x.rows[g], x.cols, c.st));
             }
     }
-    int nq[GMAX], ns[GMAX];
-    const float* q[GMAX];
-    const pcrcg_table* tab[GMAX];
-    float* inv_n[GMAX];
-    void* ws[GMAX];
-    size_t wsb[GMAX];
+    int nq[CMAX], ns[CMAX];
+    const float* q[CMAX];
+    const pcrcg_table* tab[CMAX];
+    float* inv_n[CMAX];
+    void* ws[CMAX];
+    size_t wsb[CMAX];
     for (int g = 0; g < c.G; ++g) {
         const pcrcg_batch& b = *B.b[g];
         tab[g] = blk.strided ? &b.pools[l] : &b.neighbors[l];
@@ -438,12 +446,12 @@
 }
 
 void out_rows(const Ctx& c, const Batches& B, const pcrcg_block& blk, int* rows) {
-    for (int g = 0; g < GMAX; ++g)
+    for (int g = 0; g < CMAX; ++g)
         rows[g] = g < c.G ? (blk.strided ? B.b[g]->n_points[blk.layer + 1] : B.b[g]->n_points[blk.layer]) : 0;
 }
 
 Mat simple_block(Ctx& c, const Batches& B, Walks& W, const pcrcg_block& blk, const Mat& x) {
-    int nq[GMAX];
+    int nq[CMAX];
     out_rows(c, B, blk, nq);
     Mat y = c.mat(nq, blk.mid_dim);
     const size_t m = c.mark();
@@ -496,13 +504,13 @@
 }
 
 Mat resnet_block(Ctx& c, const Batches& B, Walks& W, const pcrcg_block& blk, const Mat& feats) {
-    int nq[GMAX];
+    int nq[CMAX];
     out_rows(c, B, blk, nq);
     Mat y = c.mat(nq, blk.out_dim);
     const size_t m = c.mark();
     Mat x = feats;
-    void* kp_ws[GMAX] = {};
-    size_t kp_wsb[GMAX] = {};
+    void* kp_ws[CMAX] = {};
+    size_t kp_wsb[CMAX] = {};
     bool packed = false;
     if (blk.unary1) {
         Mat t = c.gemm_out(feats.rows, blk.mid_dim, feats.cols), u = c.mat(feats.rows, blk.mid_dim);
@@ -567,7 +575,7 @@
 void edge_norm_all(Ctx& c, const Mat& cn, int cw, int* const* idx, const int* n, const int* k, const Mat& e, const Mat& out,
                    void* const* sums, bool sums_ok, float* stats, void* ws, size_t wsb) {
     bool multi = sums_ok;
-    EdgeCloud cl[GMAX];
+    EdgeCloud cl[CMAX];
     for (int g = 0; g < c.G; ++g) {
         multi = multi && sums[g] != nullptr;
         cl[g] = EdgeCloud{cn.p[g], cn.p[g] + cw, idx[g], e.p[g], static_cast<double*>(sums[g]), n[g], k[g]};
@@ -592,8 +600,8 @@
     const int ch = f.cols;
     Mat y = c.mat(f.rows, ch);
     const size_t m = c.mark();
-    int kq[GMAX];
-    int* idx[GMAX];
+    int kq[CMAX];
+    int* idx[CMAX];
     for (int g = 0; g < c.G; ++g) {
         const int n = f.rows[g];
         kq[g] = mdl.knn_k < n - 1 ? mdl.knn_k : n - 1;
@@ -606,7 +614,7 @@
     Mat cn1 = c.gemm_out(f.rows, 2 * ch, ch), e1 = c.mat(f.rows, ch), cn2 = c.gemm_out(f.rows, 4 * ch, ch), e2 = c.mat(f.rows, 2 * ch);
     Mat x3 = c.gemm_out(f.rows, ch, 4 * ch);
     Stat x3s = stat_buffer(c, f.rows, ch);
-    void *sums1[GMAX], *sums2[GMAX];
+    void *sums1[CMAX], *sums2[CMAX];
     for (int g = 0; g < c.G; ++g) {
         sums1[g] = gemm_split_terms_on() ? c.zraw(2 * sizeof(double) * (size_t)ch) : nullptr;
         sums2[g] = gemm_split_terms_on() ? c.zraw(2 * sizeof(double) * (size_t)(2 * ch)) : nullptr;
@@ -614,8 +622,7 @@
     Mat cat1 = cols(cat, ch, ch), cat2 = cols(cat, 2 * ch, 2 * ch);
     const bool ok1 = sums_apply_ok(e1, cat1, nullptr), ok2 = sums_apply_ok(e2, cat2, nullptr);
     if (c.live()) {
-        if (!knn_given)
-            for (int g = 0; g < c.G; ++g) c.check(pcrcg_knn(coords[g], f.rows[g], kq[g], idx[g], c.st));
+        if (!knn_given) c.check(knn_multi(coords, f.rows, kq, idx, c.G, c.st));
         c.check(copy2d_multi(f.p, cat.p, f.rows, c.G, f.ld, cat.ld, ch, c.st));
         linear(c, f, gl.edge1, ch, nullptr, cn1);
         edge_norm_all(c, cn1, ch, idx, f.rows, kq, e1, cat1, sums1, ok1, stats, ws, wsb);
@@ -653,7 +660,7 @@
     }
     bool att_done = false;
     if (c.live()) {
-        AttnCloud cl[GMAX];
+        AttnCloud cl[CMAX];
         for (int g = 0; g < c.G; ++g) cl[g] = AttnCloud{q.p[g], kk.p[g], v.p[g], msg.p[g], x.rows[g], src.rows[g]};
         if (attention_mfma_ok(cl, c.G, q.ld, kk.ld, v.ld, d)) {
             c.check(attention_mfma_multi(cl, c.G, q.ld, kk.ld, v.ld, msg.ld, h, d, 1.0f / sqrtf((float)d), c.st));
@@ -685,8 +692,11 @@
         norm_act(c, h0, 0.0f, h1, &h0s);
         linear(c, h1, gl.w3, 2 * ch, gl.b3, delta);
     }
-    if (c.live())
-        for (int g = 0; g < c.G; ++g) c.check(pcrcg_add(x.p[g], delta.p[g], y.p[g], (long)x.rows[g] * ch, c.st));
+    if (c.live()) {
+        long cnt[CMAX];
+        for (int g = 0; g < c.G; ++g) cnt[g] = (long)x.rows[g] * ch;
+        c.check(add_multi(x.p, delta.p, y.p, cnt, c.G, c.st));
+    }
     c.release(m);
     return y;
 }
@@ -715,8 +725,8 @@
         x = blk.type == PCRCG_BLK_SIMPLE ? simple_block(c, B, W, blk, x) : resnet_block(c, B, W, blk, x);
     }
     const int gd = mdl.gnn_dim;
-    int nc[GMAX] = {}, ns[GMAX] = {}, nt[GMAX] = {}, zero[GMAX] = {};
-    const float *c0[GMAX], *c1[GMAX];
+    int nc[CMAX] = {}, ns[CMAX] = {}, nt[CMAX] = {}, zero[CMAX] = {};
+    const float *c0[CMAX], *c1[CMAX];
     for (int g = 0; g < c.G; ++g) {
         nc[g] = B.b[g]->n_points[L - 1];
         ns[g] = B.b[g]->len_src_c;
@@ -727,25 +737,28 @@
     Mat fc = c.gemm_out(nc, gd, mdl.enc_out_dim);
     linear(c, x, mdl.bottle_w, mdl.enc_out_dim, mdl.bottle_b, fc);
     Mat d0 = rows(fc, zero, ns), d1 = rows(fc, ns, nt);
-    int* knn0[GMAX] = {};
-    int* knn1[GMAX] = {};
+    int* knn0[CMAX] = {};
+    int* knn1[CMAX] = {};
     int n_self = 0;
     for (int i = 0; i < mdl.n_gnn; ++i) n_self += mdl.gnn[i].cross ? 0 : 1;
     const bool knn_once = n_self >= 2;
-    if (knn_once)
-        for (int g = 0; g < c.G; ++g) {
+    const int G0 = c.G;
+    if (knn_once) {
+        const float* pts[CMAX];
+        int n01[CMAX], k01[CMAX];
+        int* tab[CMAX];
+        for (int g = 0; g < G0; ++g) {
             const int k0 = mdl.knn_k < ns[g] - 1 ? mdl.knn_k : ns[g] - 1, k1 = mdl.knn_k < nt[g] - 1 ? mdl.knn_k : nt[g] - 1;
             knn0[g] = static_cast<int*>(c.raw(sizeof(int) * (size_t)ns[g] * (k0 > 0 ? k0 : 1)));
             knn1[g] = static_cast<int*>(c.raw(sizeof(int) * (size_t)nt[g] * (k1 > 0 ? k1 : 1)));
-            if (c.live()) {
-                c.check(pcrcg_knn(c0[g], ns[g], k0, knn0[g], c.st));
-                c.check(pcrcg_knn(c1[g], nt[g], k1, knn1[g], c.st));
-            }
-        }
-    const int G0 = c.G;
-    const bool stack = 2 * G0 <= GMAX && gemm_split_terms_on();
-    const float* c01[GMAX] = {};
-    int* knn01[GMAX] = {};
+            pts[g] = c0[g]; n01[g] = ns[g]; k01[g] = k0; tab[g] = knn0[g];
+            pts[G0 + g] = c1[g]; n01[G0 + g] = nt[g]; k01[G0 + g] = k1; tab[G0 + g] = knn1[g];
+        }
+        if (c.live()) c.check(knn_multi(pts, n01, k01, tab, 2 * G0, c.st));
+    }
+    const bool stack = 2 * G0 <= CMAX && gemm_split_terms_on();
+    const float* c01[CMAX] = {};
+    int* knn01[CMAX] = {};
     for (int g = 0; g < G0 && stack; ++g) { c01[g] = c0[g]; c01[G0 + g] = c1[g]; knn01[g] = knn0[g]; knn01[G0 + g] = knn1[g]; }
     for (int i = 0; i < mdl.n_gnn; ++i) {
         const pcrcg_gnn_layer& gl = mdl.gnn[i];
@@ -774,29 +787,30 @@
     Mat xc = c.mat(nc, wc, pad4(wc));
     {
         const size_t m = c.mark();
-        Mat gcat = c.mat(nc, gd), fn = c.mat(nc, gd);
-        Mat pst = c.mat(ns, c.max_rows(nt)), pts = c.mat(nt, c.max_rows(ns));
-        if (c.live())
+        Mat fn = c.mat(nc, gd);
+        Mat pst = c.mat(ns, c.max_rows(nt));
+        Mat feats = cols(xc, 2, gd), score = cols(xc, 0, 1), sal = cols(xc, 1, 1);
+        const Mat f0 = rows(feats, zero, ns), f1 = rows(feats, ns, nt);
+        if (stack) {
+            const Mat x2 = stacked(d0, d1, G0), y2 = stacked(f0, f1, G0);
+            c.twice([&] { linear(c, x2, mdl.proj_gnn_w, gd, mdl.proj_gnn_b, y2); return y2; });
+        } else {
+            linear(c, d0, mdl.proj_gnn_w, gd, mdl.proj_gnn_b, f0);
+            linear(c, d1, mdl.proj_gnn_w, gd, mdl.proj_gnn_b, f1);
+        }
+        linear(c, feats, mdl.proj_score_w, gd, mdl.proj_score_b, score);
+        if (c.live()) {
+            c.check(l2norm_rows_multi(feats.p, fn.p, nc, c.G, feats.ld, fn.ld, gd, c.st));
+            SalPair sp[GMAX];
             for (int g = 0; g < c.G; ++g) {
-                c.check(pcrcg_copy2d(d0.p[g], d0.ld, gcat.p[g], gcat.ld, ns[g], gd, c.st));
-                c.check(pcrcg_copy2d(d1.p[g], d1.ld, gcat.p[g] + (long)ns[g] * gcat.ld, gcat.ld, nt[g], gd, c.st));
-            }
-        Mat feats = cols(xc, 2, gd), score = cols(xc, 0, 1), sal = cols(xc, 1, 1);
-        linear(c, gcat, mdl.proj_gnn_w, gd, mdl.proj_gnn_b, feats);
-        linear(c, feats, mdl.proj_score_w, gd, mdl.proj_score_b, score);
-        if (c.live())
-            for (int g = 0; g < c.G; ++g) {
-                c.check(pcrcg_l2norm_rows(feats.p[g], feats.ld, fn.p[g], fn.ld, nc[g], gd, c.st));
-                const float inv_t = 1.0f / mdl.temperature;
                 const float* fs = fn.p[g];
                 const float* ft = fn.p[g] + (long)ns[g] * fn.ld;
                 c.check(pcrcg_gemm_f32(fs, fn.ld, ft, fn.ld, 1, pst.p[g], nt[g], ns[g], nt[g], gd, nullptr, nullptr, c.st));
-                c.check(pcrcg_softmax_matvec(pst.p[g], ns[g], nt[g], nt[g], inv_t, score.p[g] + (long)ns[g] * xc.ld, xc.ld, sal.p[g],
-                                             xc.ld, c.st));
-                c.check(pcrcg_gemm_f32(ft, fn.ld, fs, fn.ld, 1, pts.p[g], ns[g], nt[g], ns[g], gd, nullptr, nullptr, c.st));
-                c.check(pcrcg_softmax_matvec(pts.p[g], nt[g], ns[g], ns[g], inv_t, score.p[g], xc.ld, sal.p[g] + (long)ns[g] * xc.ld,
-                                             xc.ld, c.st));
-            }
+                sp[g] = SalPair{pst.p[g], score.p[g], score.p[g] + (long)ns[g] * xc.ld, sal.p[g], sal.p[g] + (long)ns[g] * xc.ld,
+                                ns[g], nt[g], nt[g]};
+            }
+            c.check(softmax_matvec_pairs(sp, c.G, 1.0f / mdl.temperature, xc.ld, c.st));
+        }
         c.release(m);
     }
     x = xc;
@@ -812,8 +826,8 @@
     for (int j = 0; j < mdl.n_dec; ++j) {
         const pcrcg_block& blk = mdl.dec[j];
         if (blk.type == PCRCG_BLK_UPSAMPLE) {
-            const pcrcg_table* tabs[GMAX];
-            int trows[GMAX] = {};
+            const pcrcg_table* tabs[CMAX];
+            int trows[CMAX] = {};
             for (int g = 0; g < c.G; ++g) { tabs[g] = &B.b[g]->upsamples[blk.layer - 1]; trows[g] = tabs[g]->rows; }
             const bool concat = j + 1 < mdl.n_dec && mdl.dec_concat[j + 1];
             const int cs = concat ? skips.back().cols : 0;
diff --git a/pcrcg_amd/ops.py b/pcrcg_amd/ops.py
--- a/pcrcg_amd/ops.py
+++ b/pcrcg_amd/ops.py
@@ -835,6 +835,103 @@
     return y
 
 
+def _ptr_array(ts):
+    return (ctypes.c_void_p * len(ts))(*[t.data_ptr() for t in ts])
+
+
+def _int_array(vs, ctype=ctypes.c_int):
+    return (ctype * len(vs))(*[int(v) for v in vs])
+
+
+def _one_ld(lds, rows, what):
+    many = {l for l, r in zip(lds, rows) if r > 1} or {max(lds)}
+    if len(many) != 1:
+        raise RuntimeError(f"pcrcg_amd.{what}: the clouds must share their leading dimensions")
+    return many.pop()
+
+
+def softmax_matvec_pairs(ss, scores_s, scores_t, scale=1.0):
+    L = _lib.lib()
+    n = len(ss)
+    if not (1 <= n <= 4 and len(scores_s) == n and len(scores_t) == n):
+        raise RuntimeError("pcrcg_amd.softmax_matvec_pairs: one to four pairs")
+    ss, ld = zip(*[_rows(s, _F32, "s") for s in ss])
+    scores_s = [_dev(v, _F32, "score_s").contiguous() for v in scores_s]
+    scores_t = [_dev(v, _F32, "score_t").contiguous() for v in scores_t]
+    for s, a, b in zip(ss, scores_s, scores_t):
+        if a.dim() != 1 or b.dim() != 1 or a.shape[0] != s.shape[0] or b.shape[0] != s.shape[1]:
+            raise RuntimeError("pcrcg_amd.softmax_matvec_pairs: scores_s[p] [ns_p] and scores_t[p] [nt_p] for ss[p] [ns_p, nt_p]")
+    s1 = [torch.empty(s.shape[0], dtype=_F32, device=s.device) for s in ss]
+    s2 = [torch.empty(s.shape[1], dtype=_F32, device=s.device) for s in ss]
+    _lib.check(L.pcrcg_softmax_matvec_pairs(_ptr_array(ss), _int_array([s.shape[0] for s in ss]), _int_array([s.shape[1] for s in ss]),
+                                            _int_array(ld), _ptr_array(scores_s), _ptr_array(scores_t), _ptr_array(s1),
+                                            _ptr_array(s2), n, float(scale), 1, _stream()), "pcrcg_softmax_matvec_pairs")
+    return s1, s2
+
+
+def knn_multi(coords, ks):
+    L = _lib.lib()
+    coords = [_dev(c, _F32, "coords").contiguous() for c in coords]
+    idx = [torch.empty((c.shape[0], int(k)), dtype=_I32, device=c.device) for c, k in zip(coords, ks)]
+    _lib.check(L.pcrcg_knn_multi(_ptr_array(coords), _int_array([c.shape[0] for c in coords]), _int_array(ks), _ptr_array(idx),
+                                 len(coords), _stream()), "pcrcg_knn_multi")
+    return idx
+
+
+def edgeconv_reduce_sums_multi(ctrs, nbrs, idxs):
+    L = _lib.lib()
+    ctrs, ld_ctr = zip(*[_rows(t, _F32, "ctr") for t in ctrs])
+    nbrs, ld_nbr = zip(*[_rows(t, _F32, "nbr") for t in nbrs])
+    idxs = [_dev(i, _I32, "idx").contiguous() for i in idxs]
+    c = ctrs[0].shape[1]
+    rows = [t.shape[0] for t in ctrs]
+    emax = [torch.empty((r, c), dtype=_F32, device=ctrs[0].device) for r in rows]
+    sums = [torch.zeros((2, c), dtype=torch.float64, device=ctrs[0].device) for _ in rows]
+    _lib.check(L.pcrcg_edgeconv_reduce_sums_multi(_ptr_array(ctrs), _ptr_array(nbrs), _ptr_array(idxs), _int_array(rows),
+                                                  _int_array([i.shape[1] for i in idxs]), _ptr_array(emax), _ptr_array(sums),
+                                                  len(rows), _one_ld(ld_ctr, rows, "edgeconv_reduce_sums_multi"),
+                                                  _one_ld(ld_nbr, rows, "edgeconv_reduce_sums_multi"), c, c, _stream()),
+               "pcrcg_edgeconv_reduce_sums_multi")
+    return emax, sums
+
+
+def attention_multi(qs, ks, vs, heads, scale=None):
+    L = _lib.lib()
+    qs, ldq = zip(*[_rows(t, _F32, "q") for t in qs])
+    ks, ldk = zip(*[_rows(t, _F32, "k") for t in ks])
+    vs, ldv = zip(*[_rows(t, _F32, "v") for t in vs])
+    ch = qs[0].shape[1]
+    d = ch // heads
+    n, ms = [q.shape[0] for q in qs], [k.shape[0] for k in ks]
+    outs = [torch.empty((r, ch), dtype=_F32, device=qs[0].device) for r in n]
+    _lib.check(L.pcrcg_attention_multi(_ptr_array(qs), _ptr_array(ks), _ptr_array(vs), _ptr_array(outs), _int_array(n), _int_array(ms),
+                                       len(n), _one_ld(ldq, n, "attention_multi"), _one_ld(ldk, ms, "attention_multi"),
+                                       _one_ld(ldv, ms, "attention_multi"), ch, heads, d,
+                                       float(d ** -0.5 if scale is None else scale), _stream()), "pcrcg_attention_multi")
+    return outs
+
+
+def add_multi(a, b):
+    L = _lib.lib()
+    a = [_dev(t, _F32, "a").contiguous() for t in a]
+    b = [_dev(t, _F32, "b").contiguous() for t in b]
+    out = [torch.empty_like(t) for t in a]
+    _lib.check(L.pcrcg_add_multi(_ptr_array(a), _ptr_array(b), _ptr_array(out), _int_array([t.numel() for t in a], ctypes.c_long),
+                                 len(a), _stream()), "pcrcg_add_multi")
+    return out
+
+
+def l2norm_rows_multi(xs):
+    L = _lib.lib()
+    xs, ld = zip(*[_rows(t, _F32, "x") for t in xs])
+    rows = [t.shape[0] for t in xs]
+    c = xs[0].shape[1]
+    out = [torch.empty((r, c), dtype=_F32, device=xs[0].device) for r in rows]
+    _lib.check(L.pcrcg_l2norm_rows_multi(_ptr_array(xs), _ptr_array(out), _int_array(rows), len(rows),
+                                         _one_ld(ld, rows, "l2norm_rows_multi"), c, c, _stream()), "pcrcg_l2norm_rows_multi")
+    return out
+
+
 def feature_argmax(a, b, want_best=False):
     L = _lib.lib()
     a, lda = _rows(a, _F32, "a")
```
